# naver-ai/egtr

Hardware: AMD Instinct MI355X
Metric: images/sec end-to-end SGG, 600x1000 input, N=200 queries (higher is better)
Workload: dtype f32; 1 GPU; VG inference: ResNet-50, N=200, 6 enc/6 dec, 150 classes, 50 predicates, 600x1000, bs=1/GPU fp32 (BASELINE configs[1]); hip_graph=True, gemm_tuning=True, miopen_find=True, parallelism=replicas x1 (independent images, no collective)

## Files before the change

### egtr_amd/_lib.py

```python
import ctypes
import os

import torch

_HERE = os.path.dirname(os.path.abspath(__file__))
LIB_PATH = os.environ.get("EGTR_HIP_LIBRARY") or os.path.join(_HERE, "libegtr_hip.so")

_P = ctypes.c_void_p
_I = ctypes.c_int
ABI_VERSION = 5

SIGNATURES = {
    "egtr_abi_version": [],
    "egtr_status_string": [_I],
    "egtr_last_hip_error": [],
    "egtr_msda_forward_f32": [_P, _P, _P, _P, _P, _P, _I, _I, _I, _I, _I, _I, _I, _P],
    "egtr_msda_forward_fused_vbias_f32": [_P, _P, _P, _P, _P, _P, _P, _I, _I, _I, _I, _I, _I, _I, _P, _P, _I, _I, _P, _P,
                                          _P],
    "egtr_msda_forward_fused_box_f32": [_P, _P, _P, _P, _P, _P, _P, _I, _I, _I, _I, _I, _I, _I, _P, _P, _I, _I, _P, _P,
                                        _P],
    "egtr_msda_backward_f32": [_P, _P, _P, _P, _P, _P, _P, _I, _I, _I, _I, _I, _I, _I, _P, _P, _P],
    "egtr_msda_backward_out_f32": [_P, _P, _P, _P, _P, _P, _P, _I, _I, _I, _I, _I, _I, _I, _P, _P, _P],
    "egtr_msda_forward_f64": [_P, _P, _P, _P, _P, _P, _I, _I, _I, _I, _I, _I, _I, _P],
    "egtr_msda_backward_f64": [_P, _P, _P, _P, _P, _P, _P, _I, _I, _I, _I, _I, _I, _I, _P, _P, _P],
    "egtr_msda_backward_bf16": [_P, _P, _P, _P, _P, _P, _P, _I, _I, _I, _I, _I, _I, _I, _P, _P, _P, _P],
    "egtr_msda_backward_bf16_workspace_floats": [_I, _I, _I, _I, _I, _I, _I],
    "egtr_msda_forward_bf16": [_P, _P, _P, _P, _P, _P, _I, _I, _I, _I, _I, _I, _I, _P],
    "egtr_msda_forward_fused_bf16": [_P, _P, _P, _P, _P, _P, _P, _I, _I, _I, _I, _I, _I, _I, _P, _I, _I, _P, _P],
    "egtr_self_attn_forward_f32": [_P, _P, _P, _P, _I, _I, _I, _I, _P, _P, _P, _P],
    "egtr_self_attn_forward_bf16": [_P, _P, _P, _P, _I, _I, _I, _I, _P, _P, _P],
    "egtr_self_attn_backward_f32": [_P, _P, _P, _P, _P, _P, _P, _I, _I, _I, _I, _P, _P, _P],
    "egtr_self_attn_backward_acc_f32": [_P, _P, _P, _P, _P, _P, _P, _I, _I, _I, _I, _P, _P, _P, _P, _P],
    "egtr_linear_f32": [_P, _P, _P, _P, _P, _I, _I, _I, ctypes.c_float, _I],
    "egtr_linear_grouped_f32": [_P, _I, _P, _P, _P, _P, _P, _P, _P, _P, _P, _P, _I],
    "egtr_linear_grouped_ln_f32": [_P, _I, _P, _P, _P, _P, _P, _P, _P, _P, _P, _P, _I, _P, _P, _P, _P, _P, _P, _P],
    "egtr_add_layernorm_pos_f32": [_P, _P, _P, _P, _P, _P, _I, _I, ctypes.c_float, _P, _I, _P],
    "egtr_bias_mask_rows_f32": [_P, _P, _P, _P, _I, _I, _I],
    "egtr_bias_relu_maxpool3x3s2_f32": [_P, _P, _P, _P, _I, _I, _I, _I],
    "egtr_box_decode_argmax_f32": [_P, _P, _P, _P, _I, _I, _I, _I, ctypes.c_float, _P, _P, _I, _P],
    "egtr_scale_rows_multi_f32": [_P, _I, _P, _P, _P, _P, _P],
    "egtr_bias_act_nchw_f32": [_P, _P, _P, _P, _P, _I, _I, _I, _I],
    "egtr_bias_act_nchw_bf16": [_P, _P, _P, _P, _P, _I, _I, _I, _I],
    "egtr_bias_act_nhwc_bf16": [_P, _P, _P, _P, _P, ctypes.c_longlong, _I, _I],
    "egtr_bias_act_nhwc_f32": [_P, _P, _P, _P, _P, ctypes.c_longlong, _I, _I],
    "egtr_add_layernorm_bf16": [_P, _P, _P, _P, _P, _P, _I, _I, ctypes.c_float],
    "egtr_add_layernorm_pos_bf16": [_P, _P, _P, _P, _P, _P, _I, _I, ctypes.c_float, _P, _I, _P],
    "egtr_add_layernorm_f32": [_P, _P, _P, _P, _P, _P, _I, _I, ctypes.c_float],
    "egtr_sine_pos_embed_f32": [_P, _P, _P, _P, _P, _I, _I, _I, _I, ctypes.c_float, ctypes.c_float],
    "egtr_level_geometry_f32": [_P, _P, _I, _P, _P, _P, _I, _I, _I, _I, _I, ctypes.c_float, ctypes.c_float, _P, _P, _P,
                                _P, _P],
    "egtr_level_geometry_bf16": [_P, _P, _I, _P, _P, _P, _I, _I, _I, _I, _I, ctypes.c_float, ctypes.c_float, _P, _P, _P,
                                 _P, _P],
    "egtr_input_proj_groupnorm_flatten_f32": [_P, _I, _P, _P, _P, _P, _P, _I, _I, _I, ctypes.c_float, _P, _P],
    "egtr_input_proj_groupnorm_flatten_bf16": [_P, _I, _P, _P, _P, _P, _P, _I, _I, _I, ctypes.c_float, _P, _P],
    "egtr_input_proj_groupnorm_tokens_bf16": [_P, _I, _P, _P, _P, _P, _P, _I, _I, _I, ctypes.c_float, _P, _P],
    "egtr_input_proj_groupnorm_tokens_f32": [_P, _I, _P, _P, _P, _P, _P, _I, _I, _I, ctypes.c_float, _P, _P],
    "egtr_input_proj_groupnorm_tokens_workspace_floats": [_I, _P, _I],
    "egtr_bbox_overlaps_f64": [_P, _P, _P, _I, _I, _I, _P],
    "egtr_sgg_eval_width": [_I, _I],
    "egtr_sgg_eval_f32": [_P, _P, _I, _P, _P, _P, _I, _I, _I, _I, _P, _P, ctypes.c_longlong, _P, _P, _P, ctypes.c_longlong,
                          _P, _I, ctypes.c_double, _P, _P, _P],
    "egtr_sgg_zero_shot_f64": [_P, _P, _P, _P, ctypes.c_longlong, _P, _P, ctypes.c_longlong, _I, _I, _I, _I, _P, _P, _I, _P,
                               _P],
    "egtr_sgg_eval_phrdet_f32": [_P, _P, _I, _P, _P, _P, _I, _I, _I, _I, _P, _P, ctypes.c_longlong, _P, _P, _P,
                                 ctypes.c_longlong, _P, _I, ctypes.c_double, _P, _P, _P],
    "egtr_sgg_eval_preddet_f32": [_P, _P, _P, _I, _I, _I, _P, _P, ctypes.c_longlong, _P, ctypes.c_longlong, _P, _I, _P, _P,
                                  _P, _P, _P],
    "egtr_matched_topk_workspace_bytes": [_I, _I, _I],
    "egtr_matched_topk_f32": [_P, _P, _P, _P, _P, _I, _I, _I, _I, _I, _I, _P, _P, _P, _P, _P],
    "egtr_rel_stats_i64": [_P, _P, _P, ctypes.c_longlong, _P, _P, ctypes.c_longlong, _I, _I, _I, _P, _P],
    "egtr_rel_seen_bits_i64": [_P, _P, ctypes.c_longlong, _P],
    "egtr_oi_eval_width": [_I, _I],
    "egtr_oi_select_workspace_bytes": [_I, _I, _I, _I],
    "egtr_oi_select_f32": [_P, _P, ctypes.c_longlong, ctypes.c_longlong, _P, _P, ctypes.c_longlong, _I, _I, _I, _I, _I,
                           _I, _P, _P, _P, _P],
    "egtr_oi_match_f32": [_P, _P, _P, _I, _I, _P, _P, _I, _I, _P, _P, ctypes.c_longlong, _P, _P, _P, ctypes.c_longlong,
                          _P, _I, _P, _P, _P],
    "egtr_oi_ap_f64": [_P, _P, _P, _P, ctypes.c_longlong, _I, _P, _P],
    "egtr_coco_match_f32": [_P, _P, _P, _P, _I, _I, _I, _P, _P, _P, _P, _P, ctypes.c_longlong, _P, _P, _I, _P, _P, _P,
                            _P, _P],
    "egtr_coco_accumulate_f64": [_P, _P, _P, _P, _P, ctypes.c_longlong, _I, _P, _P, _P, _P],
    "egtr_hungarian_match_f32": [_P, _P, _P, _P, _P, _P, _P, _I, _I, _I, _I, ctypes.c_float, ctypes.c_float,
                                 ctypes.c_float, _I, ctypes.c_float, ctypes.c_float, _P, _P, _P, _P, _P, _P, _P],
    "egtr_hungarian_match_scratch_doubles": [_I, _I, ctypes.c_longlong],
    "egtr_add_layernorm_backward_f32": [_P, _P, _P, _P, _P, _P, _P, _P, _I, _I, ctypes.c_float],
    "egtr_add_layernorm_backward_workspace_floats": [_I],
    "egtr_msda_geometry_forward_f32": [_P, _P, ctypes.c_longlong, _P, ctypes.c_longlong, _P, _I, _P, _P, _P, ctypes.c_longlong, _I, _I, _I],
    "egtr_msda_geometry_backward_f32": [_P, _P, _P, _P, _P, ctypes.c_longlong, _P, _I, _P, _P, ctypes.c_longlong, _P, ctypes.c_longlong, _P, ctypes.c_longlong, _I, _I, _I],
    "egtr_linear_backward_f32": [_P, _P, _P, _P, _P, ctypes.c_float, _P, _P, _P, _I, _I, _I],
    "egtr_linear_backward_acc_f32": [_P, _P, _P, _P, _P, ctypes.c_float, _P, _P, _P, _I, _I, _I, _P, _P],
    "egtr_weighted_column_sum_f32": [_P, _P, _P, _P, _P, _I, _I],
    "egtr_column_sum_f32": [_P, _P, _P, _P, _P, _P, _I, _I],
    "egtr_column_sum_workspace_floats": [_I, _I],
    "egtr_any_nonfinite_f32": [_P, _P, ctypes.c_longlong, _P],
    "egtr_clamp_if_flag_f32": [_P, _P, _P, ctypes.c_longlong, _P, ctypes.c_float, _I],
    "egtr_detection_loss_f32": [_P, _P, _P, _P, _P, _P, _P, _P, _P, _I, _I, _I, ctypes.c_float, ctypes.c_float, _P, _P,
                                _P, _P],
    "egtr_relation_loss_f32": [_P, _P, _P, _P, _P, _P, _P, _P, _I, _I, _I, ctypes.c_float, _I, _I, _P, _P, _P, _P],
    "egtr_relation_loss_workspace_bytes": [_I, _I],
    "egtr_relation_loss_bits_f32": [_P, _P, _P, _P, _P, _P, _P, _P, _I, _I, _I, ctypes.c_float, _I, _I, _P, _P, _P, _P],
    "egtr_pack_relations_u64": [_P, _P, _P, _I, _I, _I, _I, _P],
    "egtr_rel_head_forward_bf16w": [_P] * 16 + [_I] * 6 + [_P] * 3,
    "egtr_ffn_layernorm_bf16": [_P] * 7 + [ctypes.c_float, _P, _I, _P, _P, _I, _I, _I],
    "egtr_ffn_pack_weights_bf16": [_P, _P, _P, _I, _I, _P],
    "egtr_ffn_packed_weights_bytes": [_I],
    "egtr_linear_bf16": [_P, _P, _I, _P, _P, _P, _I, _I, _I, _I, _I, ctypes.c_float],
    "egtr_rel_head_forward_bf16p": [_P] * 16 + [_I] * 6 + [_P] * 3,
    "egtr_rel_head_pack_tables_bf16": [_P, _P, _I, _I, _I, _P],
    "egtr_linear_split_bf16_f32": [_P, _P, _I, _P, _P, _P, _I, _I, _I, _I, _I],
    "egtr_linear_split_bf16_wgrad_f32": [_P, _P, _I, _P, _I, _P, _P, _I, _I, _I],
    "egtr_linear_split_bf16_wgrad_workspace_floats": [_I, _I, _I],
    "egtr_gemm_split_tile_weights_f32": [_P, _P, _I, _I, _I, _I, _P],
    "egtr_gemm_split_tile_weights_pair_f32": [_P, _P, _I, _I, _I, _P],
    "egtr_gemm_split_tile_weights_multi_f32": [_P, _I, _P, _P, _P, _P, _P, _P, _P, _P],
    "egtr_linear_split_bf16_grouped_pos_f32": [_P, _I, _P, _P, _P, _P, _P, _P, _P, _P, _I, _I, _P, _P],
    "egtr_linear_split_bf16_ex_f32": [_P, _I, _P, _P, _P, _P, _P, _P, _P, _P, _I, _I, _P, _P, _P, _P, _P, _P, _P, _P, _P],
    "egtr_linear_split_bf16_wgrad_ex_f32": [_P, _P, _I, _P, _I, _P, _P, _I, _I, _I, _P, _I, _P],
    "egtr_dropout_add_layernorm_f32": [_P, _P, _P, _P, ctypes.c_float, _P, _P, _P, _I, _I, ctypes.c_float, _P],
    "egtr_dropout_add_layernorm_backward_workspace_floats": [_I],
    "egtr_dropout_add_layernorm_backward_f32": [_P, _P, _P, _P, ctypes.c_float, _P, _P, _P, _P, ctypes.c_float, _P, _P, _P,
                                                _P, _I, _I, ctypes.c_float],
    "egtr_pad_batch_f32": [_P, _P, _P, _I, _I, _I, _I, _P, _P],
    "egtr_preprocess_f32": [_P, _P, _I, _P, _P, _I, _I, _I, _I, _P, _P, _P],
    "egtr_preprocess_bf16": [_P, _P, _I, _P, _P, _I, _I, _I, _I, _P, _P, _P],
    "egtr_preprocess_augment_f32": [_P, _P, _P, _I, _P, _P, _I, _I, _I, _I, _I, _I, _I, _I, _P, _P, _P],
    "egtr_preprocess_augment_bf16": [_P, _P, _P, _I, _P, _P, _I, _I, _I, _I, _I, _I, _I, _I, _P, _P, _P],
    "egtr_conv1x1_tail_x6_f32": [_P, _P, _I, _P, _I, _P, _P, _P, _I, _I, _P, _I, _I, _I, _I, _I, _I],
    "egtr_stem_conv7x7_pool_bf16": [_P, _P, _P, _P, _P, _I, _I, _I],
    "egtr_stem_conv7x7_pool_x6_f32": [_P, _P, _P, _P, _P, _I, _I, _I],
    "egtr_conv1x1_strided_x6_f32": [_P, _P, _P, _P, _I, _I, _I, _I, _I, _I],
    "egtr_conv3x3_phase_channels": [_I, _I, _I, _I],
    "egtr_conv3x3_x6_f32": [_P, _P, _P, _P, _I, _I, _I, _I, _I, _I, _I],
    "egtr_conv3x3_x6_shift_f32": [_P, _P, _P, _P, _P, _I, _I, _I, _I, _I, _I, _I],
    "egtr_conv1x1_tail_pack_weights_bf16": [_P, _P, _I, _I, _I, _P],
    "egtr_conv1x1_tail_bf16": [_P, _P, _I, _P, _I, _P, _P, _P, _I, _I, _P, _I, _I, _I, _I],
    "egtr_ffn_x6_f32": [_P, _P, _I, _P, _P, _P, _P, _P, _P, ctypes.c_float, _P, _I, _P, _P, _I, _I, _I],
    "egtr_encoder_tail_x6_f32": [_P, _P, _I, _P, _I, _P, _P, _P, _P, ctypes.c_float, _P, _P, _P, _P, _P, _P, ctypes.c_float,
                                 _P, _I, _P, _P, _I, _I, _I],
    "egtr_proj_ln_x6_f32": [_P, _P, _I, _P, _P, _P, _I, _P, _P, ctypes.c_float, _P, _I, _P, _P, _I, _I],
    "egtr_proj_multi_x6_f32": [_P, _P, _I, _P, _P, _P, _I, _I, _I],
    "egtr_xs_bytes": [_I, _I],
    "egtr_xs_split_f32": [_P, _P, _I, _P, _I, _I, _I, _P, _P, _I],
    "egtr_rel_head_forward_bf16x6_f32": [_P] * 16 + [_I] * 6 + [_P] * 3 + [_I],
    "egtr_rel_head_forward_bf16x6_save_f32": [_P] * 16 + [_I] * 6 + [_P] * 5,
    "egtr_rel_head_streams_f32": [_P] * 4 + [_I] * 2 + [_P] * 3,
    "egtr_rel_head_forward_save_f32": [_P] * 16 + [_I] * 6 + [_P] * 5,
    "egtr_rel_head_backward_pairs_f32": [_P] * 6 + [_I] * 4 + [_P] * 5,
    "egtr_decoder_layer_f32": [_P, _P],
    "egtr_decoder_layer_workspace": [_I, _I, _P, _P, _P],
}
_RESTYPES = {"egtr_status_string": ctypes.c_char_p, "egtr_last_hip_error": ctypes.c_char_p,
             "egtr_ffn_packed_weights_bytes": ctypes.c_longlong,
             "egtr_input_proj_groupnorm_tokens_workspace_floats": ctypes.c_longlong,
             "egtr_msda_backward_bf16_workspace_floats": ctypes.c_longlong,
             "egtr_hungarian_match_scratch_doubles": ctypes.c_longlong,
             "egtr_relation_loss_workspace_bytes": ctypes.c_longlong,
             "egtr_column_sum_workspace_floats": ctypes.c_longlong,
             "egtr_add_layernorm_backward_workspace_floats": ctypes.c_longlong,
             "egtr_linear_split_bf16_wgrad_workspace_floats": ctypes.c_longlong,
             "egtr_dropout_add_layernorm_backward_workspace_floats": ctypes.c_longlong,
             "egtr_xs_bytes": ctypes.c_longlong, "egtr_sgg_eval_width": ctypes.c_longlong,
             "egtr_oi_eval_width": ctypes.c_longlong, "egtr_matched_topk_workspace_bytes": ctypes.c_longlong, "egtr_oi_select_workspace_bytes": ctypes.c_longlong}

_lib = None


class EgtrHipError(RuntimeError):
    pass


def lib():
    global _lib
    if _lib is None:
        if not os.path.exists(LIB_PATH):
            raise EgtrHipError(
                f"{LIB_PATH} not found: the HIP extension has not been built "
                "(run `make -C egtr_amd/csrc` or __graft_entry__.build()). There is no CPU fallback.")
        handle = ctypes.CDLL(LIB_PATH)
        handle.egtr_abi_version.restype = ctypes.c_int
        got = handle.egtr_abi_version()
        if got != ABI_VERSION:
            raise EgtrHipError(f"{LIB_PATH} has ABI version {got}, this package was written against {ABI_VERSION}: "
                               "rebuild it (make -C egtr_amd/csrc)")
        if os.environ.get("EGTR_HIP_LIBRARY"):
            import sys
            print(f"egtr_amd: EGTR_HIP_LIBRARY is set -- using {LIB_PATH} instead of the in-tree build", file=sys.stderr)
        for name, argtypes in SIGNATURES.items():
            fn = getattr(handle, name)
            fn.argtypes = argtypes
            fn.restype = _RESTYPES.get(name, ctypes.c_int)
        _lib = handle
    return _lib


def check(status, what):
    if status != 0:
        h = lib()
        msg = h.egtr_status_string(status).decode()
        if status == -2:
            msg += ": " + h.egtr_last_hip_error().decode()
        raise EgtrHipError(f"{what} failed: {msg} (status {status})")


def _chk(t, name, dtype=None):
    if not t.is_cuda:
        raise RuntimeError(f"{name} must be a CUDA/HIP tensor")
    if not t.is_contiguous():
        raise RuntimeError(f"{name} tensor has to be contiguous")
    if dtype is not None and t.dtype != dtype:
        raise RuntimeError(f"{name} must be {dtype}, got {t.dtype}")
    if t.data_ptr() % 16 != 0:
        raise RuntimeError(f"{name} must be 16-byte aligned")
    return t


_RAW_STREAM = getattr(torch._C, "_cuda_getCurrentRawStream", None)


def _stream():
    if _RAW_STREAM is not None:
        return _RAW_STREAM(torch.cuda.current_device())
    return torch.cuda.current_stream().cuda_stream


def launch(name, *args, what=None):
    st = getattr(lib(), name)(_stream(), *args)
    if st != 0:
        check(st, what or name)


def ptr(t):
    return None if t is None else t.data_ptr()


def row_view(t, K):
    t2 = t.reshape(-1, K)
    if t2.stride(1) != 1 or t2.stride(0) % 4 or t2.data_ptr() % 16:
        t2 = t2.contiguous()
    return t2
```

### egtr_amd/csrc/elementwise.hip

```cpp
#include <hip/hip_runtime.h>
#include <stdint.h>

#include "common.h"

namespace {

__global__ __launch_bounds__(256) void bias_act_nchw_vec4(const float* __restrict__ x, const float* __restrict__ bias,
                                                          const float* __restrict__ res, float* __restrict__ y,
                                                          long long n4, int C, int HW4, int relu) {
  for (long long i = blockIdx.x * (long long)blockDim.x + threadIdx.x; i < n4; i += (long long)gridDim.x * blockDim.x) {
    const int c = (int)((i / HW4) % C);
    const float b = bias[c];
    float4 v = reinterpret_cast<const float4*>(x)[i];
    v.x += b; v.y += b; v.z += b; v.w += b;
    if (res != nullptr) {
      const float4 r = reinterpret_cast<const float4*>(res)[i];
      v.x += r.x; v.y += r.y; v.z += r.z; v.w += r.w;
    }
    if (relu) { v.x = egtr_relu(v.x); v.y = egtr_relu(v.y); v.z = egtr_relu(v.z); v.w = egtr_relu(v.w); }
    reinterpret_cast<float4*>(y)[i] = v;
  }
}

__global__ __launch_bounds__(256) void bias_act_nchw_flat4(const float* __restrict__ x, const float* __restrict__ bias,
// ... 238 lines not shown
    }
    if (relu) {
#pragma unroll
      for (int k = 0; k < 8; ++k) v[k] = egtr_relu(v[k]);
    }
    unsigned w[4];
#pragma unroll
    for (int k = 0; k < 4; ++k) {
      bf16x2 pr;
      pr[0] = (__bf16)v[2 * k];
      pr[1] = (__bf16)v[2 * k + 1];
      w[k] = __builtin_bit_cast(unsigned, pr);
    }
    reinterpret_cast<uint4*>(y)[i] = make_uint4(w[0], w[1], w[2], w[3]);
  }
}

__global__ __launch_bounds__(256) void bias_act_nchw_scalar_bf16(const unsigned short* __restrict__ x,
                                                                 const float* __restrict__ bias,
                                                                 const unsigned short* __restrict__ res,
                                                                 unsigned short* __restrict__ y, long long n, int C,
                                                                 int HW, int relu) {
  for (long long i = blockIdx.x * (long long)blockDim.x + threadIdx.x; i < n; i += (long long)gridDim.x * blockDim.x) {
    const int c = (int)((i / HW) % C);
    float v = bf2f(x[i]) + bias[c];
    if (res != nullptr) v += bf2f(res[i]);
    if (relu) v = egtr_relu(v);
    y[i] = f2bf(v);
  }
}

__global__ __launch_bounds__(256) void bias_mask_rows(float* __restrict__ y, const float* __restrict__ bias,
                                                      const unsigned char* __restrict__ keep, long long n4, int R,
                                                      int C4) {
  for (long long i = blockIdx.x * (long long)blockDim.x + threadIdx.x; i < n4; i += (long long)gridDim.x * blockDim.x) {
    const int c4 = (int)(i % C4);
    const long long gr = i / C4;
    const int r = (int)(gr % R);
    const int g = (int)(gr / R);
    float4 v = reinterpret_cast<float4*>(y)[i];
    const float4 b = reinterpret_cast<const float4*>(bias)[(size_t)g * C4 + c4];
    const bool k = keep == nullptr || keep[r] != 0;
    v = k ? make_float4(v.x + b.x, v.y + b.y, v.z + b.z, v.w + b.w) : make_float4(0.f, 0.f, 0.f, 0.f);
    reinterpret_cast<float4*>(y)[i] = v;
  }
}

__global__ __launch_bounds__(256) void bias_relu_maxpool3x3s2(const float* __restrict__ x, const float* __restrict__ bias,
                                                              float* __restrict__ y, int C, int H, int W, int Ho,
                                                              int Wo, long long planes) {
  const int ox = blockIdx.x * 64 + (threadIdx.x & 63);
  const int oy = blockIdx.y * 4 + (threadIdx.x >> 6);
  const long long plane = blockIdx.z;
  if (ox >= Wo || oy >= Ho) return;
  const float* xp = x + plane * H * W;
  const int iy0 = 2 * oy - 1, ix0 = 2 * ox - 1;
  float m = -INFINITY;
#pragma unroll
  for (int dy = 0; dy < 3; ++dy) {
    const int iy = iy0 + dy;
    if (iy < 0 || iy >= H) continue;
    const float* row = xp + (size_t)iy * W;
#pragma unroll
    for (int dx = 0; dx < 3; ++dx) {
      const int ix = ix0 + dx;
      if (ix >= 0 && ix < W) {
        const float v = row[ix];
        m = (v > m || v != v) ? v : m;
      }
    }
  }
  const float r = m + bias[(int)(plane % C)];
  y[(plane * Ho + oy) * Wo + ox] = (r != r) ? r : fmaxf(r, 0.f);
}

__global__ __launch_bounds__(256) void box_decode(const float* __restrict__ delta, const float* __restrict__ init_ref,
                                                  const float* __restrict__ inter_ref, int B, int Ld, int N, int RD,
                                                  float eps, float* __restrict__ out,
                                                  const float* __restrict__ logits_all, int C,
                                                  long long* __restrict__ node_cls) {
  const int nb_decode = (B * Ld * N + 255) / 256;
  if ((int)blockIdx.x >= nb_decode) {
    const int row = ((int)blockIdx.x - nb_decode) * 4 + (threadIdx.x >> 6), lane = threadIdx.x & 63;
    if (row >= B * N) return;
    const int b = row / N, n = row - b * N;
    const float* lg = logits_all + (((size_t)b * Ld + (Ld - 1)) * N + n) * C;
    float best = lane < C ? lg[lane] : 0.f;
    int arg = lane < C ? lane : 0x7fffffff;
    for (int c = lane + 64; c < C; c += 64) {
      const float v = lg[c];
      if (v > best || (v != v && best == best)) { best = v; arg = c; }
    }
#pragma unroll
    for (int o = 1; o < 64; o <<= 1) {
      const float v = __shfl_xor(best, o);
      const int a = __shfl_xor(arg, o);
      const bool vn = v != v, bn = best != best;
      const bool take = a != 0x7fffffff && (arg == 0x7fffffff || (vn && !bn) || (!bn && v > best) || ((vn == bn) && (vn || v == best) && a < arg));
      if (take) { best = v; arg = a; }
    }
    if (lane == 0) node_cls[row] = arg;
    return;
  }
  const int i = blockIdx.x * 256 + threadIdx.x;
  if (i >= B * Ld * N) return;
  const int n = i % N, l = (i / N) % Ld, b = i / (N * Ld);
  const float* rp = (l == 0 || inter_ref == nullptr) ? init_ref + ((size_t)b * N + n) * RD
                                                      : inter_ref + (((size_t)b * Ld + (l - 1)) * N + n) * RD;
  const float4 d = reinterpret_cast<const float4*>(delta)[i];
  float v[4] = {d.x, d.y, d.z, d.w};
  for (int k = 0; k < RD; ++k) {
    float x = rp[k];
    x = fminf(fmaxf(x, 0.f), 1.f);
    if (rp[k] != rp[k]) x = rp[k];
    const float x1 = (x != x) ? x : fmaxf(x, eps), x2 = (x != x) ? x : fmaxf(1.f - x, eps);
    v[k] += logf(x1 / x2);
  }
  float4 o;
  o.x = 1.f / (1.f + expf(-v[0]));
  o.y = 1.f / (1.f + expf(-v[1]));
  o.z = 1.f / (1.f + expf(-v[2]));
  o.w = 1.f / (1.f + expf(-v[3]));
  reinterpret_cast<float4*>(out)[i] = o;
}

__global__ __launch_bounds__(256) void sine_pos_embed(const float* __restrict__ y_embed, const float* __restrict__ x_embed,
                                                      const float* __restrict__ dim_t, float* __restrict__ out, int B,
                                                      int H, int Wd, int E, float scale, float eps) {
  const long long n = (long long)B * E * H * Wd;
  for (long long i = blockIdx.x * (long long)blockDim.x + threadIdx.x; i < n; i += (long long)gridDim.x * blockDim.x) {
    const int x = (int)(i % Wd);
    long long t = i / Wd;
    const int y = (int)(t % H);
    t /= H;
    const int slot = (int)(t % E);
    const int b = (int)(t / E);
    const int axis = slot >= E / 2;
    const int pair = axis ? slot - E / 2 : slot;
    const size_t pix = ((size_t)b * H + y) * Wd + x;
    float e, last;
    if (axis == 0) {
      e = y_embed[pix];
      last = y_embed[((size_t)b * H + (H - 1)) * Wd + x];
    } else {
      e = x_embed[pix];
      last = x_embed[((size_t)b * H + y) * Wd + (Wd - 1)];
    }
    const float v = (e - 0.5f) / (last + eps) * scale;
    const float a0 = v / dim_t[2 * pair], a1 = v / dim_t[2 * pair + 1];
    const size_t plane = (size_t)H * Wd;
    float* o = out + ((size_t)b * 2 * E + (size_t)axis * E + 2 * pair) * plane + (size_t)y * Wd + x;
    o[0] = sinf(a0);
    o[plane] = cosf(a1);
  }
}


struct LevelDims {
  int H[4], W[4], start[4];
};

template <typename MaskT>
__global__ __launch_bounds__(256) void level_mask_resize(const MaskT* __restrict__ pixel_mask, LevelDims ld, int L, int S,
                                                         int Hin, int Win, unsigned char* __restrict__ mask_flat,
                                                         unsigned* __restrict__ mask_bits) {
  const int b = blockIdx.y;
  const int s = blockIdx.x * 256 + threadIdx.x;
  int m = 0;
  if (s < S) {
    int l = 0;
    while (l + 1 < L && s >= ld.start[l + 1]) ++l;
    const int rel = s - ld.start[l];
    const int y = rel / ld.W[l], x = rel - y * ld.W[l];
    const float sh = (float)Hin / (float)ld.H[l], sw = (float)Win / (float)ld.W[l];
    const int sy = min((int)floorf((float)y * sh), Hin - 1), sx = min((int)floorf((float)x * sw), Win - 1);
    m = pixel_mask[((size_t)b * Hin + sy) * Win + sx] != 0 ? 1 : 0;
    mask_flat[(size_t)b * S + s] = (unsigned char)m;
  }
  if (mask_bits != nullptr) {
    const unsigned long long bal = __ballot(m != 0);
    const int lane = threadIdx.x & 63, s64 = s - lane;
    const int nwords = (S + 31) >> 5;
    if (lane < 2 && s64 + 32 * lane < S && (s64 >> 5) + lane < nwords)
      mask_bits[(size_t)b * nwords + (s64 >> 5) + lane] = (unsigned)(bal >> (32 * lane));
  }
}

template <typename PosT>
__global__ __launch_bounds__(256) void level_geometry(const unsigned char* __restrict__ mask_all,
                                                      const float* __restrict__ dim_t,
                                                      const float* __restrict__ level_embed, LevelDims ld, int L, int S,
                                                      int E, float scale, float eps, PosT* __restrict__ pos_flat,
                                                      float* __restrict__ valid_ratios, float* __restrict__ ref_points) {
  constexpr int TP = 8;
  __shared__ int s_cnt[8];
  __shared__ float s_vr[8];
  __shared__ int s_pix[TP][5];
  const int tid = threadIdx.x;
  const int b = blockIdx.y;
  const int s0 = blockIdx.x * TP;
  const unsigned char* mk = mask_all + (size_t)b * S;
  if (tid < 8) s_cnt[tid] = 0;
  __syncthreads();
  for (int l = 0; l < L; ++l) {
    const unsigned char* ml = mk + ld.start[l];
    int cw = 0, ch = 0;
    for (int x = tid; x < ld.W[l]; x += 256) cw += ml[x];
    for (int y = tid; y < ld.H[l]; y += 256) ch += ml[(size_t)y * ld.W[l]];
#pragma unroll
    for (int o = 1; o < 64; o <<= 1) {
      cw += __shfl_xor(cw, o);
      ch += __shfl_xor(ch, o);
    }
    if ((tid & 63) == 0) {
      if (cw) atomicAdd(&s_cnt[2 * l], cw);
      if (ch) atomicAdd(&s_cnt[2 * l + 1], ch);
    }
  }
  {
    const int p = tid >> 5, part = tid & 31;
    const int s = s0 + p;
    int l = 0, cy = 0, toty = 0, cx = 0, totx = 0;
    if (s < S) {
      while (l + 1 < L && s >= ld.start[l + 1]) ++l;
      const unsigned char* ml = mk + ld.start[l];
      const int rel = s - ld.start[l];
      const int Wl = ld.W[l], Hl = ld.H[l];
      const int y = rel / Wl, x = rel - y * Wl;
      for (int yy = part; yy < Hl; yy += 32) {
        const int v = ml[yy * Wl + x];
        toty += v;
        cy += (yy <= y) ? v : 0;
      }
      for (int xx = part; xx < Wl; xx += 32) {
        const int v = ml[y * Wl + xx];
        totx += v;
        cx += (xx <= x) ? v : 0;
      }
    }
#pragma unroll
    for (int o = 1; o < 32; o <<= 1) {
      cy += __shfl_xor(cy, o);
      toty += __shfl_xor(toty, o);
      cx += __shfl_xor(cx, o);
      totx += __shfl_xor(totx, o);
    }
    if (part == 0) {
      s_pix[p][0] = l;
      s_pix[p][1] = cy;
      s_pix[p][2] = toty;
      s_pix[p][3] = cx;
      s_pix[p][4] = totx;
    }
  }
  __syncthreads();
  if (tid < 2 * L) {
    const int l = tid >> 1;
    const float vr = (float)s_cnt[tid] / (float)((tid & 1) ? ld.H[l] : ld.W[l]);
    s_vr[tid] = vr;
    if (blockIdx.x == 0) valid_ratios[(size_t)b * L * 2 + tid] = vr;
  }
  __syncthreads();
  if (tid < 8 * TP) {
    const int p = tid >> 3, k = tid & 7, s = s0 + p;
    if (s < S && k < 2 * L) {
      const int l = s_pix[p][0];
      const int rel = s - ld.start[l];
      const int y = rel / ld.W[l], x = rel - y * ld.W[l];
      const int lt = k >> 1, ax = k & 1;
      const float base = ax ? ((float)y + 0.5f) / (s_vr[2 * l + 1] * (float)ld.H[l])
                            : ((float)x + 0.5f) / (s_vr[2 * l] * (float)ld.W[l]);
      ref_points[(((size_t)b * S + s) * L + lt) * 2 + ax] = base * s_vr[2 * lt + ax];
    }
  }
  {
    const int npair = E;
    const int per = 256 / npair > 0 ? 256 / npair : 1;
    for (int k = tid % npair; k < npair; k += 256) {
      const int c = 2 * k;
      const int axis = c >= E, i = axis ? c - E : c;
      const float dt = dim_t[i];
      for (int p = (npair <= 256 ? tid / npair : 0); p < TP; p += per) {
        const int s = s0 + p;
        if (s >= S) break;
        const int l = s_pix[p][0];
        const float e = (float)(axis ? s_pix[p][3] : s_pix[p][1]), last = (float)(axis ? s_pix[p][4] : s_pix[p][2]);
        const float v = (e - 0.5f) / (last + eps) * scale;
        const float a = v / dt;
        float sn, cs;
        sincosf(a, &sn, &cs);
        const float2 le = *reinterpret_cast<const float2*>(level_embed + l * 2 * E + c);
        if constexpr (sizeof(PosT) == 4) {
          *reinterpret_cast<float2*>(pos_flat + ((size_t)b * S + s) * (2 * E) + c) = make_float2(sn + le.x, cs + le.y);
        } else {
          const unsigned lo = f2bf(bf2f(f2bf(sn)) + le.x), hi = f2bf(bf2f(f2bf(cs)) + le.y);
          *reinterpret_cast<unsigned*>(pos_flat + ((size_t)b * S + s) * (2 * E) + c) = lo | (hi << 16);
        }
      }
    }
  }
}


struct GnLevels {
  const void* x[4];
  const float* conv_bias[4];
  const float* gamma[4];
  const float* beta[4];
  int hw[4], start[4], tile0[4];
};

__device__ __forceinline__ float gn_load(const float* p) { return *p; }
__device__ __forceinline__ float gn_load(const unsigned short* p) { return bf2f(*p); }

template <typename T>
__global__ __launch_bounds__(1024) void gn_stats_levels(GnLevels P, int C, int G, float eps, float2* __restrict__ stats) {
  __shared__ double s_red[2][16];
  const int g = blockIdx.x, b = blockIdx.y, l = blockIdx.z;
  const int cpg = C / G, hw = P.hw[l];
  const T* x = static_cast<const T*>(P.x[l]) + ((size_t)b * C + (size_t)g * cpg) * hw;
  float s1 = 0.f, s2 = 0.f;
  for (int c = 0; c < cpg; ++c) {
    const float cb = P.conv_bias[l][g * cpg + c];
    const T* xc = x + (size_t)c * hw;
    for (int i0 = threadIdx.x; i0 < hw; i0 += 8 * 1024) {
      float v[8];
#pragma unroll
      for (int u = 0; u < 8; ++u) {
        const int i = i0 + 1024 * u;
        v[u] = i < hw ? gn_load(xc + i) : 0.f;
      }
#pragma unroll
      for (int u = 0; u < 8; ++u) {
        if (i0 + 1024 * u < hw) {
          const float t = v[u] + cb;
          s1 += t;
          s2 += t * t;
        }
      }
    }
  }
  double d1 = (double)s1, d2 = (double)s2;
#pragma unroll
  for (int o = 1; o < 64; o <<= 1) {
    d1 += __shfl_xor(d1, o);
    d2 += __shfl_xor(d2, o);
  }
  if ((threadIdx.x & 63) == 0) {
    s_red[0][threadIdx.x >> 6] = d1;
    s_red[1][threadIdx.x >> 6] = d2;
  }
  __syncthreads();
  if (threadIdx.x == 0) {
    double t1 = 0.0, t2 = 0.0;
    for (int w = 0; w < 16; ++w) {
      t1 += s_red[0][w];
      t2 += s_red[1][w];
    }
    const double n = (double)cpg * hw, mean = t1 / n;
    const double var = fmax(t2 / n - mean * mean, 0.0);
    stats[((size_t)l * gridDim.y + b) * G + g] = make_float2((float)mean, (float)(1.0 / sqrt(var + (double)eps)));
  }
}

template <typename T>
__global__ __launch_bounds__(256) void gn_apply_flatten(GnLevels P, int L, int C, int G, int S, const float2* __restrict__ stats,
                                                        T* __restrict__ out) {
  __shared__ float s_t[32][257];
  const int b = blockIdx.y;
  int l = 0;
  while (l + 1 < L && (int)blockIdx.x >= P.tile0[l + 1]) ++l;
  const int p0 = ((int)blockIdx.x - P.tile0[l]) * 32, hw = P.hw[l];
  const int cpg = C / G;
  const int px = threadIdx.x & 31, cs = threadIdx.x >> 5;
  const T* x = static_cast<const T*>(P.x[l]) + (size_t)b * C * hw;
  float xv[32];
  const bool inside = p0 + px < hw;
#pragma unroll
  for (int k = 0; k < 32; ++k) xv[k] = inside ? gn_load(x + (size_t)(cs + 8 * k) * hw + p0 + px) : 0.f;
#pragma unroll
  for (int k = 0; k < 32; ++k) {
    const int c = cs + 8 * k;
    const float2 st = stats[((size_t)l * gridDim.y + b) * G + c / cpg];
    const float v = (xv[k] + P.conv_bias[l][c] - st.x) * st.y * P.gamma[l][c] + P.beta[l][c];
    s_t[px][c] = inside ? v : 0.f;
  }
  __syncthreads();
  for (int p = 0; p < 32; ++p) {
    if (p0 + p >= hw) break;
    if constexpr (sizeof(T) == 4) out[((size_t)b * S + P.start[l] + p0 + p) * C + threadIdx.x] = s_t[p][threadIdx.x];
    else out[((size_t)b * S + P.start[l] + p0 + p) * C + threadIdx.x] = f2bf(s_t[p][threadIdx.x]);
  }
}

}

extern "C" int egtr_sine_pos_embed_f32(egtr_stream_t stream, const float* y_embed, const float* x_embed,
                                       const float* dim_t, float* out, int B, int H, int W, int E, float scale,
                                       float eps) {
  if (!y_embed || !x_embed || !dim_t || !out) return EGTR_E_ARG;
  if (B <= 0 || H <= 0 || W <= 0 || E <= 0 || (E & 1)) return EGTR_E_ARG;
  const long long n = (long long)B * E * H * W;
  const int blocks = (int)std::min<long long>((n + 255) / 256, 256 * 16);
  hipLaunchKernelGGL(sine_pos_embed, dim3(blocks), dim3(256), 0, static_cast<hipStream_t>(stream), y_embed, x_embed,
                     dim_t, out, B, H, W, E, scale, eps);
  return egtr_check_launch();
}

static int level_geometry_launch(egtr_stream_t stream, const void* pixel_mask, int mask_elem_size, const float* dim_t,
                                 const float* level_embed, const int* level_hw, int num_levels, int batch, int height,
                                 int width, int embed_dim, float scale, float eps, unsigned char* mask_flat,
                                 void* pos_flat, bool pos_bf16, float* valid_ratios, float* ref_points,
                                 unsigned* mask_bits) {
  if (!pixel_mask || !dim_t || !level_embed || !level_hw || !mask_flat || !pos_flat || !valid_ratios || !ref_points)
    return EGTR_E_ARG;
  if (num_levels < 1 || num_levels > 4 || batch <= 0 || height <= 0 || width <= 0 || embed_dim <= 0)
    return EGTR_E_ARG;
  if (mask_elem_size != 1 && mask_elem_size != 8) return EGTR_E_UNSUPPORTED;
  if (embed_dim & 1) return EGTR_E_UNSUPPORTED;
  LevelDims ld;
  int S = 0;
  for (int l = 0; l < 4; ++l) {
    const bool on = l < num_levels;
    ld.H[l] = on ? level_hw[2 * l] : 1;
    ld.W[l] = on ? level_hw[2 * l + 1] : 1;
    ld.start[l] = S;
    if (on) {
      if (ld.H[l] <= 0 || ld.W[l] <= 0) return EGTR_E_ARG;
      S += ld.H[l] * ld.W[l];
    }
  }
  hipStream_t st = static_cast<hipStream_t>(stream);
  const dim3 grid1((unsigned)((S + 255) / 256), (unsigned)batch);
  if (mask_elem_size == 8)
    hipLaunchKernelGGL(level_mask_resize<long long>, grid1, dim3(256), 0, st, static_cast<const long long*>(pixel_mask),
                       ld, num_levels, S, height, width, mask_flat, mask_bits);
  else
    hipLaunchKernelGGL(level_mask_resize<unsigned char>, grid1, dim3(256), 0, st,
                       static_cast<const unsigned char*>(pixel_mask), ld, num_levels, S, height, width, mask_flat,
                       mask_bits);
  const dim3 grid((unsigned)((S + 7) / 8), (unsigned)batch);
  if (pos_bf16)
    hipLaunchKernelGGL(level_geometry<unsigned short>, grid, dim3(256), 0, st, mask_flat, dim_t, level_embed, ld,
                       num_levels, S, embed_dim, scale, eps, static_cast<unsigned short*>(pos_flat), valid_ratios,
                       ref_points);
  else
    hipLaunchKernelGGL(level_geometry<float>, grid, dim3(256), 0, st, mask_flat, dim_t, level_embed, ld, num_levels, S,
                       embed_dim, scale, eps, static_cast<float*>(pos_flat), valid_ratios, ref_points);
  return egtr_check_launch();
}

extern "C" int egtr_level_geometry_f32(egtr_stream_t stream, const void* pixel_mask, int mask_elem_size,
                                       const float* dim_t, const float* level_embed, const int* level_hw,
                                       int num_levels, int batch, int height, int width, int embed_dim, float scale,
                                       float eps, unsigned char* mask_flat, float* pos_flat, float* valid_ratios,
                                       float* ref_points, unsigned* mask_bits) {
  return level_geometry_launch(stream, pixel_mask, mask_elem_size, dim_t, level_embed, level_hw, num_levels, batch, height,
                               width, embed_dim, scale, eps, mask_flat, pos_flat, false, valid_ratios, ref_points,
                               mask_bits);
}

extern "C" int egtr_level_geometry_bf16(egtr_stream_t stream, const void* pixel_mask, int mask_elem_size,
                                        const float* dim_t, const float* level_embed, const int* level_hw,
                                        int num_levels, int batch, int height, int width, int embed_dim, float scale,
                                        float eps, unsigned char* mask_flat, uint16_t* pos_flat, float* valid_ratios,
                                        float* ref_points, unsigned* mask_bits) {
  return level_geometry_launch(stream, pixel_mask, mask_elem_size, dim_t, level_embed, level_hw, num_levels, batch, height,
                               width, embed_dim, scale, eps, mask_flat, pos_flat, true, valid_ratios, ref_points,
                               mask_bits);
}

static int groupnorm_flatten_launch(egtr_stream_t stream, int num_levels, const void* const* x,
                                    const float* const* conv_bias, const float* const* gamma, const float* const* beta,
                                    const int* level_hw, int batch, int channels, int num_groups, float eps, float* stats,
                                    void* out, bool bf16) {
  if (!x || !conv_bias || !gamma || !beta || !level_hw || !stats || !out) return EGTR_E_ARG;
  if (num_levels < 1 || num_levels > 4 || batch <= 0 || num_groups <= 0) return EGTR_E_ARG;
  if (channels != 256 || channels % num_groups != 0) return EGTR_E_UNSUPPORTED;
  GnLevels P;
  int S = 0, tiles = 0;
  for (int l = 0; l < 4; ++l) {
    const int s = l < num_levels ? l : 0;
    if (!x[s] || !conv_bias[s] || !gamma[s] || !beta[s] || level_hw[2 * s] <= 0 || level_hw[2 * s + 1] <= 0)
      return EGTR_E_ARG;
    P.x[l] = x[s];
    P.conv_bias[l] = conv_bias[s];
    P.gamma[l] = gamma[s];
    P.beta[l] = beta[s];
    P.hw[l] = level_hw[2 * s] * level_hw[2 * s + 1];
    P.start[l] = S;
    P.tile0[l] = tiles;
    if (l < num_levels) {
      S += P.hw[l];
      tiles += (P.hw[l] + 31) / 32;
    }
  }
  hipStream_t st = static_cast<hipStream_t>(stream);
  if (bf16) {
    hipLaunchKernelGGL(gn_stats_levels<unsigned short>, dim3(num_groups, batch, num_levels), dim3(1024), 0, st, P, channels,
                       num_groups, eps, reinterpret_cast<float2*>(stats));
    hipLaunchKernelGGL(gn_apply_flatten<unsigned short>, dim3(tiles, batch), dim3(256), 0, st, P, num_levels, channels,
                       num_groups, S, reinterpret_cast<const float2*>(stats), static_cast<unsigned short*>(out));
  } else {
    hipLaunchKernelGGL(gn_stats_levels<float>, dim3(num_groups, batch, num_levels), dim3(1024), 0, st, P, channels,
                       num_groups, eps, reinterpret_cast<float2*>(stats));
    hipLaunchKernelGGL(gn_apply_flatten<float>, dim3(tiles, batch), dim3(256), 0, st, P, num_levels, channels, num_groups,
                       S, reinterpret_cast<const float2*>(stats), static_cast<float*>(out));
  }
  return egtr_check_launch();
}

struct GnTokLevels {
  const void* x[4];
  const float* conv_bias[4];
  const float* gamma[4];
  const float* beta[4];
  int hw[4], start[4];
  long long chunk0[5];
  int cchunk0[5];
};

namespace {
__device__ __forceinline__ void load_group8(const unsigned short* x, size_t idx, float (&f)[8]) {
  unpack8(reinterpret_cast<const uint4*>(x)[idx], f);
}
__device__ __forceinline__ void load_group8(const float* x, size_t idx, float (&f)[8]) {
  const float4 a = reinterpret_cast<const float4*>(x)[2 * idx], b = reinterpret_cast<const float4*>(x)[2 * idx + 1];
  f[0] = a.x; f[1] = a.y; f[2] = a.z; f[3] = a.w; f[4] = b.x; f[5] = b.y; f[6] = b.z; f[7] = b.w;
}
constexpr int kGnTokChunk = 256;
template <typename T>
__global__ __launch_bounds__(256) void gn_partial_tokens(GnTokLevels P, int L, int chunks_total, double2* __restrict__ partial) {
  __shared__ double s_red[2][32][9];
  const int b = blockIdx.y;
  int l = 0;
  while (l + 1 < L && (int)blockIdx.x >= P.cchunk0[l + 1]) ++l;
  const int t_begin = ((int)blockIdx.x - P.cchunk0[l]) * kGnTokChunk, hw = P.hw[l];
  const int g = threadIdx.x & 31, ph = threadIdx.x >> 5;
  const T* x = static_cast<const T*>(P.x[l]) + (size_t)b * hw * 256;
  const float4 ba = *reinterpret_cast<const float4*>(P.conv_bias[l] + 8 * g), bb = *reinterpret_cast<const float4*>(P.conv_bias[l] + 8 * g + 4);
  const float cb[8] = {ba.x, ba.y, ba.z, ba.w, bb.x, bb.y, bb.z, bb.w};
  float s1 = 0.f, s2 = 0.f;
#pragma unroll
  for (int u0 = 0; u0 < kGnTokChunk / 8; u0 += 8) {
    float f[8][8];
#pragma unroll
    for (int u = 0; u < 8; ++u) {
      const int t = t_begin + ph + 8 * (u0 + u);
      if (t < hw) load_group8(x, (size_t)t * 32 + g, f[u]);
    }
#pragma unroll
    for (int u = 0; u < 8; ++u) {
      const int t = t_begin + ph + 8 * (u0 + u);
      if (t < hw) {
#pragma unroll
        for (int k = 0; k < 8; ++k) {
          const float v = f[u][k] + cb[k];
          s1 += v;
          s2 += v * v;
        }
      }
    }
  }
  s_red[0][g][ph] = (double)s1;
  s_red[1][g][ph] = (double)s2;
  __syncthreads();
  if (threadIdx.x < 32) {
    double t1 = 0.0, t2 = 0.0;
    for (int w = 0; w < 8; ++w) {
      t1 += s_red[0][threadIdx.x][w];
      t2 += s_red[1][threadIdx.x][w];
    }
    partial[((size_t)b * chunks_total + blockIdx.x) * 32 + threadIdx.x] = make_double2(t1, t2);
  }
}

__global__ __launch_bounds__(256) void gn_finalize_tokens(GnTokLevels P, int chunks_total, float eps,
                                                          const double2* __restrict__ partial, float2* __restrict__ stats) {
  __shared__ double2 s_part[8][32];
  const int b = blockIdx.x, l = blockIdx.y, B = gridDim.x, g = threadIdx.x & 31, part = threadIdx.x >> 5;
  double t1 = 0.0, t2 = 0.0;
  for (int c = P.cchunk0[l] + part; c < P.cchunk0[l + 1]; c += 8) {
    const double2 p = partial[((size_t)b * chunks_total + c) * 32 + g];
    t1 += p.x;
    t2 += p.y;
  }
  s_part[part][g] = make_double2(t1, t2);
  __syncthreads();
  if (part != 0) return;
  t1 = 0.0;
  t2 = 0.0;
#pragma unroll
  for (int k = 0; k < 8; ++k) {
    t1 += s_part[k][g].x;
    t2 += s_part[k][g].y;
  }
  const double n = 8.0 * P.hw[l], mean = t1 / n;
  const double var = fmax(t2 / n - mean * mean, 0.0);
  stats[((size_t)l * B + b) * 32 + g] = make_float2((float)mean, (float)(1.0 / sqrt(var + (double)eps)));
}

template <typename T>
__global__ __launch_bounds__(256) void gn_apply_tokens(GnTokLevels P, int L, int S, const float2* __restrict__ stats,
                                                       T* __restrict__ out) {
  typedef __bf16 bf16x2 __attribute__((ext_vector_type(2)));
  const int b = blockIdx.y, B = gridDim.y;
  const long long i = (long long)blockIdx.x * 256 + threadIdx.x;
  if (i >= (long long)S * 32) return;
  int l = 0;
  while (l + 1 < L && i >= P.chunk0[l + 1]) ++l;
  const long long rel = i - P.chunk0[l];
  const int g = (int)(rel & 31);
  const float2 st = stats[((size_t)l * B + b) * 32 + g];
  float f[8];
  load_group8(static_cast<const T*>(P.x[l]) + (size_t)b * P.hw[l] * 256, (size_t)rel, f);
  const float4 ca = *reinterpret_cast<const float4*>(P.conv_bias[l] + 8 * g), cb = *reinterpret_cast<const float4*>(P.conv_bias[l] + 8 * g + 4);
  const float4 ga = *reinterpret_cast<const float4*>(P.gamma[l] + 8 * g), gb = *reinterpret_cast<const float4*>(P.gamma[l] + 8 * g + 4);
  const float4 ea = *reinterpret_cast<const float4*>(P.beta[l] + 8 * g), eb = *reinterpret_cast<const float4*>(P.beta[l] + 8 * g + 4);
  const float c8[8] = {ca.x, ca.y, ca.z, ca.w, cb.x, cb.y, cb.z, cb.w};
  const float g8[8] = {ga.x, ga.y, ga.z, ga.w, gb.x, gb.y, gb.z, gb.w};
  const float e8[8] = {ea.x, ea.y, ea.z, ea.w, eb.x, eb.y, eb.z, eb.w};
  float o[8];
#pragma unroll
  for (int k = 0; k < 8; ++k) o[k] = (f[k] + c8[k] - st.x) * st.y * g8[k] + e8[k];
  T* dst = out + ((size_t)b * S + P.start[l]) * 256;
  if constexpr (sizeof(T) == 2) {
    unsigned w[4];
#pragma unroll
    for (int k = 0; k < 4; ++k) {
      bf16x2 pr;
      pr[0] = (__bf16)o[2 * k];
      pr[1] = (__bf16)o[2 * k + 1];
      w[k] = __builtin_bit_cast(unsigned, pr);
    }
    reinterpret_cast<uint4*>(dst)[rel] = make_uint4(w[0], w[1], w[2], w[3]);
  } else {
    reinterpret_cast<float4*>(dst)[2 * rel] = make_float4(o[0], o[1], o[2], o[3]);
    reinterpret_cast<float4*>(dst)[2 * rel + 1] = make_float4(o[4], o[5], o[6], o[7]);
  }
}
}

static int gn_tokens_chunks(int num_levels, const int* level_tokens) {
  int c = 0;
  for (int l = 0; l < num_levels; ++l) c += (level_tokens[l] + kGnTokChunk - 1) / kGnTokChunk;
  return c;
}

extern "C" long long egtr_input_proj_groupnorm_tokens_workspace_floats(int num_levels, const int* level_tokens, int batch) {
  if (!level_tokens || num_levels < 1 || num_levels > 4 || batch <= 0) return 0;
  return (long long)num_levels * batch * 64 + (long long)batch * gn_tokens_chunks(num_levels, level_tokens) * 128;
}

static int groupnorm_tokens_launch(egtr_stream_t stream, int num_levels, const void* const* x, const float* const* conv_bias,
                                   const float* const* gamma, const float* const* beta, const int* level_tokens, int batch,
                                   int channels, int num_groups, float eps, float* stats, void* out, bool bf16) {
  if (!x || !conv_bias || !gamma || !beta || !level_tokens || !stats || !out) return EGTR_E_ARG;
  if (num_levels < 1 || num_levels > 4 || batch <= 0) return EGTR_E_ARG;
  if (channels != 256 || num_groups != 32) return EGTR_E_UNSUPPORTED;
  GnTokLevels P;
  int S = 0, cc = 0;
  for (int l = 0; l < 4; ++l) {
    const int s = l < num_levels ? l : 0;
    if (!x[s] || !conv_bias[s] || !gamma[s] || !beta[s] || level_tokens[s] <= 0) return EGTR_E_ARG;
    if (reinterpret_cast<uintptr_t>(x[s]) & 15) return EGTR_E_UNSUPPORTED;
    P.x[l] = x[s];
    P.conv_bias[l] = conv_bias[s];
    P.gamma[l] = gamma[s];
    P.beta[l] = beta[s];
    P.hw[l] = level_tokens[s];
    P.start[l] = S;
    P.chunk0[l] = (long long)S * 32;
    P.cchunk0[l] = cc;
    if (l < num_levels) {
      S += P.hw[l];
      cc += (P.hw[l] + kGnTokChunk - 1) / kGnTokChunk;
    }
  }
  P.chunk0[4] = (long long)S * 32;
  P.cchunk0[4] = cc;
  for (int l = num_levels; l < 4; ++l) {
    P.chunk0[l] = (long long)S * 32;
    P.cchunk0[l] = cc;
  }
  if ((reinterpret_cast<uintptr_t>(out) | reinterpret_cast<uintptr_t>(stats)) & 15) return EGTR_E_UNSUPPORTED;
  hipStream_t st = static_cast<hipStream_t>(stream);
  float2* st2 = reinterpret_cast<float2*>(stats);
  double2* partial = reinterpret_cast<double2*>(stats + (size_t)num_levels * batch * 64);
  const long long chunks = (long long)S * 32;
  const dim3 agrid((unsigned)((chunks + 255) / 256), batch);
  if (bf16) {
    hipLaunchKernelGGL(gn_partial_tokens<unsigned short>, dim3(cc, batch), dim3(256), 0, st, P, num_levels, cc, partial);
    hipLaunchKernelGGL(gn_finalize_tokens, dim3(batch, num_levels), dim3(256), 0, st, P, cc, eps, partial, st2);
    hipLaunchKernelGGL(gn_apply_tokens<unsigned short>, agrid, dim3(256), 0, st, P, num_levels, S, st2,
                       static_cast<unsigned short*>(out));
  } else {
    hipLaunchKernelGGL(gn_partial_tokens<float>, dim3(cc, batch), dim3(256), 0, st, P, num_levels, cc, partial);
    hipLaunchKernelGGL(gn_finalize_tokens, dim3(batch, num_levels), dim3(256), 0, st, P, cc, eps, partial, st2);
    hipLaunchKernelGGL(gn_apply_tokens<float>, agrid, dim3(256), 0, st, P, num_levels, S, st2, static_cast<float*>(out));
  }
  return egtr_check_launch();
}

extern "C" int egtr_input_proj_groupnorm_tokens_bf16(egtr_stream_t stream, int num_levels, const uint16_t* const* x,
                                                     const float* const* conv_bias, const float* const* gamma,
                                                     const float* const* beta, const int* level_tokens, int batch,
                                                     int channels, int num_groups, float eps, float* stats, uint16_t* out) {
  return groupnorm_tokens_launch(stream, num_levels, reinterpret_cast<const void* const*>(x), conv_bias, gamma, beta,
                                 level_tokens, batch, channels, num_groups, eps, stats, out, true);
}

extern "C" int egtr_input_proj_groupnorm_tokens_f32(egtr_stream_t stream, int num_levels, const float* const* x,
                                                    const float* const* conv_bias, const float* const* gamma,
                                                    const float* const* beta, const int* level_tokens, int batch,
                                                    int channels, int num_groups, float eps, float* stats, float* out) {
  return groupnorm_tokens_launch(stream, num_levels, reinterpret_cast<const void* const*>(x), conv_bias, gamma, beta,
                                 level_tokens, batch, channels, num_groups, eps, stats, out, false);
}

extern "C" int egtr_input_proj_groupnorm_flatten_f32(egtr_stream_t stream, int num_levels, const float* const* x,
                                                     const float* const* conv_bias, const float* const* gamma,
                                                     const float* const* beta, const int* level_hw, int batch,
                                                     int channels, int num_groups, float eps, float* stats,
                                                     float* out) {
  return groupnorm_flatten_launch(stream, num_levels, reinterpret_cast<const void* const*>(x), conv_bias, gamma, beta,
                                  level_hw, batch, channels, num_groups, eps, stats, out, false);
}

extern "C" int egtr_input_proj_groupnorm_flatten_bf16(egtr_stream_t stream, int num_levels, const uint16_t* const* x,
                                                      const float* const* conv_bias, const float* const* gamma,
                                                      const float* const* beta, const int* level_hw, int batch,
                                                      int channels, int num_groups, float eps, float* stats,
                                                      uint16_t* out) {
  return groupnorm_flatten_launch(stream, num_levels, reinterpret_cast<const void* const*>(x), conv_bias, gamma, beta,
                                  level_hw, batch, channels, num_groups, eps, stats, out, true);
}

struct ScaleRowsArgs {
  const float* w[64];
  const float* scale[64];
  float* out[64];
  int rows[64], cols[64], blk0[65];
  int n;
};

namespace {
__global__ __launch_bounds__(256) void scale_rows_multi(ScaleRowsArgs A) {
  int t = 0;
  while (t + 1 < A.n && (int)blockIdx.x >= A.blk0[t + 1]) ++t;
  const int cols = A.cols[t];
  const long long n4 = (long long)A.rows[t] * cols / 4;
  const float4* w = reinterpret_cast<const float4*>(A.w[t]);
  float4* o = reinterpret_cast<float4*>(A.out[t]);
  const float* sc = A.scale[t];
  const long long base = (long long)((int)blockIdx.x - A.blk0[t]) * 1024;
#pragma unroll
  for (int u = 0; u < 4; ++u) {
    const long long i = base + u * 256 + threadIdx.x;
    if (i < n4) {
      const float s = sc[(i * 4) / cols];
      const float4 v = w[i];
      o[i] = make_float4(v.x * s, v.y * s, v.z * s, v.w * s);
    }
  }
}
}

extern "C" int egtr_scale_rows_multi_f32(egtr_stream_t stream, int n, const float* const* w, const float* const* scale,
                                         float* const* out, const int* rows, const int* cols) {
  if (!w || !scale || !out || !rows || !cols) return EGTR_E_ARG;
  if (n <= 0 || n > 64) return EGTR_E_UNSUPPORTED;
  ScaleRowsArgs A;
  int blocks = 0;
  for (int t = 0; t < n; ++t) {
    if (!w[t] || !scale[t] || !out[t] || rows[t] <= 0 || cols[t] <= 0) return EGTR_E_ARG;
    if (cols[t] % 4 != 0) return EGTR_E_UNSUPPORTED;
    if ((reinterpret_cast<uintptr_t>(w[t]) | reinterpret_cast<uintptr_t>(out[t])) & 15) return EGTR_E_UNSUPPORTED;
    A.w[t] = w[t];
    A.scale[t] = scale[t];
    A.out[t] = out[t];
    A.rows[t] = rows[t];
    A.cols[t] = cols[t];
    A.blk0[t] = blocks;
    const long long n4 = (long long)rows[t] * cols[t] / 4;
    blocks += (int)((n4 + 1023) / 1024);
  }
  A.blk0[n] = blocks;
  A.n = n;
  hipLaunchKernelGGL(scale_rows_multi, dim3(blocks), dim3(256), 0, static_cast<hipStream_t>(stream), A);
  return egtr_check_launch();
}

extern "C" int egtr_bias_act_nchw_f32(egtr_stream_t stream, const float* x, const float* bias, const float* residual,
                                      float* y, int N, int C, int HW, int relu) {
  if (!x || !bias || !y) return EGTR_E_ARG;
  if (N <= 0 || C <= 0 || HW <= 0) return EGTR_E_ARG;
  hipStream_t st = static_cast<hipStream_t>(stream);
  const long long n = (long long)N * C * HW;
  const bool aligned = ((reinterpret_cast<uintptr_t>(x) | reinterpret_cast<uintptr_t>(y) |
                         reinterpret_cast<uintptr_t>(residual)) & 15) == 0;
  const long long cap = 256 * 8;
  if (HW % 4 == 0 && aligned) {
    const long long n4 = n / 4;
    const int blocks = (int)std::min<long long>((n4 + 255) / 256, cap);
    hipLaunchKernelGGL(bias_act_nchw_vec4, dim3(blocks), dim3(256), 0, st, x, bias, residual, y, n4, C, HW / 4, relu);
  } else if (n % 4 == 0 && aligned && HW >= 4 && n < (1ll << 25)) {
    const long long n4 = n / 4;
    const int blocks = (int)std::min<long long>((n4 + 255) / 256, cap);
    hipLaunchKernelGGL(bias_act_nchw_flat4, dim3(blocks), dim3(256), 0, st, x, bias, residual, y, n4, C, HW, relu);
  } else {
    const int blocks = (int)std::min<long long>((n + 255) / 256, cap);
    hipLaunchKernelGGL(bias_act_nchw_scalar, dim3(blocks), dim3(256), 0, st, x, bias, residual, y, n, C, HW, relu);
  }
  return egtr_check_launch();
}

extern "C" int egtr_add_layernorm_f32(egtr_stream_t stream, const float* x, const float* residual, const float* gamma,
                                      const float* beta, float* y, int rows, int dim, float eps) {
  if (!x || !gamma || !beta || !y) return EGTR_E_ARG;
  if (rows <= 0) return EGTR_E_ARG;
  if (dim != 256) return EGTR_E_UNSUPPORTED;
  hipLaunchKernelGGL(add_layernorm_256, dim3((rows + 3) / 4), dim3(256), 0, static_cast<hipStream_t>(stream), x,
                     residual, gamma, beta, y, rows, eps, (const float*)nullptr, 1, (float*)nullptr);
  return egtr_check_launch();
}

extern "C" int egtr_add_layernorm_pos_f32(egtr_stream_t stream, const float* x, const float* residual,
                                          const float* gamma, const float* beta, float* y, int rows, int dim,
                                          float eps, const float* pos, int pos_rows, float* y_plus_pos) {
  if (!x || !gamma || !beta || !y || !pos || !y_plus_pos) return EGTR_E_ARG;
  if (rows <= 0 || pos_rows <= 0) return EGTR_E_ARG;
  if (dim != 256) return EGTR_E_UNSUPPORTED;
  hipLaunchKernelGGL(add_layernorm_256, dim3((rows + 3) / 4), dim3(256), 0, static_cast<hipStream_t>(stream), x,
                     residual, gamma, beta, y, rows, eps, pos, pos_rows, y_plus_pos);
  return egtr_check_launch();
}

extern "C" int egtr_bias_relu_maxpool3x3s2_f32(egtr_stream_t stream, const float* x, const float* bias, float* y, int N,
                                               int C, int H, int W) {
  if (!x || !bias || !y) return EGTR_E_ARG;
  if (N <= 0 || C <= 0 || H <= 0 || W <= 0) return EGTR_E_ARG;
  const int Ho = (H - 1) / 2 + 1, Wo = (W - 1) / 2 + 1;
  const long long planes = (long long)N * C;
  if (planes > 65535 || (Ho + 3) / 4 > 65535) return EGTR_E_UNSUPPORTED;
  const dim3 grid((unsigned)((Wo + 63) / 64), (unsigned)((Ho + 3) / 4), (unsigned)planes);
  hipLaunchKernelGGL(bias_relu_maxpool3x3s2, grid, dim3(256), 0, static_cast<hipStream_t>(stream), x, bias, y, C, H, W, Ho,
                     Wo, planes);
  return egtr_check_launch();
}

extern "C" int egtr_box_decode_argmax_f32(egtr_stream_t stream, const float* delta, const float* init_reference,
                                          const float* inter_references, int batch, int num_levels, int num_query,
                                          int ref_dim, float eps, float* boxes, const float* logits_all,
                                          int num_classes, int64_t* node_cls) {
  if (!delta || !init_reference || !boxes) return EGTR_E_ARG;
  if (batch <= 0 || num_levels <= 0 || num_query <= 0) return EGTR_E_ARG;
  if (logits_all && (!node_cls || num_classes <= 0)) return EGTR_E_ARG;
  if (ref_dim != 2 && ref_dim != 4) return EGTR_E_UNSUPPORTED;
  const long long n = (long long)batch * num_levels * num_query;
  if (n >= (1ll << 31)) return EGTR_E_UNSUPPORTED;
  const long long blocks = (n + 255) / 256 + (logits_all ? ((long long)batch * num_query + 3) / 4 : 0);
  hipLaunchKernelGGL(box_decode, dim3((unsigned)blocks), dim3(256), 0, static_cast<hipStream_t>(stream), delta,
                     init_reference, inter_references, batch, num_levels, num_query, ref_dim, eps, boxes, logits_all,
                     num_classes, reinterpret_cast<long long*>(node_cls));
  return egtr_check_launch();
}

extern "C" int egtr_bias_mask_rows_f32(egtr_stream_t stream, float* y, const float* bias, const unsigned char* keep,
                                       int groups, int rows, int cols) {
  if (!y || !bias) return EGTR_E_ARG;
  if (groups <= 0 || rows <= 0 || cols <= 0) return EGTR_E_ARG;
  if (cols % 4 != 0) return EGTR_E_UNSUPPORTED;
  const long long n4 = (long long)groups * rows * (cols / 4);
  const int blocks = (int)std::min<long long>((n4 + 255) / 256, 256 * 16);
  hipLaunchKernelGGL(bias_mask_rows, dim3(blocks), dim3(256), 0, static_cast<hipStream_t>(stream), y, bias, keep, n4,
                     rows, cols / 4);
  return egtr_check_launch();
}

extern "C" int egtr_bias_act_nchw_bf16(egtr_stream_t stream, const uint16_t* x, const float* bias,
                                       const uint16_t* residual, uint16_t* y, int N, int C, int HW, int relu) {
  if (!x || !bias || !y) return EGTR_E_ARG;
  if (N <= 0 || C <= 0 || HW <= 0) return EGTR_E_ARG;
  hipStream_t st = static_cast<hipStream_t>(stream);
  const long long n = (long long)N * C * HW;
  const bool aligned = ((reinterpret_cast<uintptr_t>(x) | reinterpret_cast<uintptr_t>(y) |
                         reinterpret_cast<uintptr_t>(residual)) & 15) == 0;
  if (n % 8 == 0 && aligned && HW >= 8) {
    const long long n8 = n / 8;
    const int blocks = (int)std::min<long long>((n8 + 255) / 256, 256 * 16);
    hipLaunchKernelGGL(bias_act_nchw_flat8_bf16, dim3(blocks), dim3(256), 0, st, x, bias, residual, y, n8, C, HW, relu);
  } else {
    const int blocks = (int)std::min<long long>((n + 255) / 256, 256 * 16);
    hipLaunchKernelGGL(bias_act_nchw_scalar_bf16, dim3(blocks), dim3(256), 0, st, x, bias, residual, y, n, C, HW, relu);
  }
  return egtr_check_launch();
}

namespace {
__global__ __launch_bounds__(256) void bias_act_nhwc_flat4_f32(const float* __restrict__ x, const float* __restrict__ bias,
                                                               const float* __restrict__ res, float* __restrict__ y,
                                                               long long n4, int C, int relu) {
  for (long long i = blockIdx.x * (long long)blockDim.x + threadIdx.x; i < n4; i += (long long)gridDim.x * blockDim.x) {
    const float4 b = *reinterpret_cast<const float4*>(bias + (int)((i * 4) % C));
    float4 v = reinterpret_cast<const float4*>(x)[i];
    v.x += b.x; v.y += b.y; v.z += b.z; v.w += b.w;
    if (res != nullptr) {
      const float4 r = reinterpret_cast<const float4*>(res)[i];
      v.x += r.x; v.y += r.y; v.z += r.z; v.w += r.w;
    }
    if (relu) v = make_float4(egtr_relu(v.x), egtr_relu(v.y), egtr_relu(v.z), egtr_relu(v.w));
    reinterpret_cast<float4*>(y)[i] = v;
  }
}
}

extern "C" int egtr_bias_act_nhwc_f32(egtr_stream_t stream, const float* x, const float* bias, const float* residual, float* y,
                                      long long rows, int C, int relu) {
  if (!x || !bias || !y) return EGTR_E_ARG;
  if (rows <= 0 || C <= 0) return EGTR_E_ARG;
  if (C % 4 != 0 || ((reinterpret_cast<uintptr_t>(x) | reinterpret_cast<uintptr_t>(y) | reinterpret_cast<uintptr_t>(residual) |
                      reinterpret_cast<uintptr_t>(bias)) & 15))
    return EGTR_E_UNSUPPORTED;
  const long long n4 = rows * C / 4;
  const int blocks = (int)std::min<long long>((n4 + 255) / 256, 256 * 16);
  hipLaunchKernelGGL(bias_act_nhwc_flat4_f32, dim3(blocks), dim3(256), 0, static_cast<hipStream_t>(stream), x, bias, residual, y,
                     n4, C, relu);
  return egtr_check_launch();
}

extern "C" int egtr_bias_act_nhwc_bf16(egtr_stream_t stream, const uint16_t* x, const float* bias, const uint16_t* residual,
                                       uint16_t* y, long long rows, int C, int relu) {
  if (!x || !bias || !y) return EGTR_E_ARG;
  if (rows <= 0 || C <= 0) return EGTR_E_ARG;
  if (C % 8 != 0 || ((reinterpret_cast<uintptr_t>(x) | reinterpret_cast<uintptr_t>(y) | reinterpret_cast<uintptr_t>(residual) |
                      reinterpret_cast<uintptr_t>(bias)) & 15))
    return EGTR_E_UNSUPPORTED;
  const long long n8 = rows * C / 8;
  const int blocks = (int)std::min<long long>((n8 + 255) / 256, 256 * 16);
  hipLaunchKernelGGL(bias_act_nhwc_flat8_bf16, dim3(blocks), dim3(256), 0, static_cast<hipStream_t>(stream), x, bias, residual,
                     y, n8, C, relu);
  return egtr_check_launch();
}

extern "C" int egtr_add_layernorm_bf16(egtr_stream_t stream, const uint16_t* x, const uint16_t* residual,
                                       const uint16_t* gamma, const uint16_t* beta, uint16_t* y, int rows, int dim,
                                       float eps) {
  if (!x || !gamma || !beta || !y) return EGTR_E_ARG;
  if (rows <= 0) return EGTR_E_ARG;
  if (dim != 256) return EGTR_E_UNSUPPORTED;
  hipLaunchKernelGGL(add_layernorm_256_bf16, dim3((rows + 7) / 8), dim3(256), 0, static_cast<hipStream_t>(stream), x,
                     residual, gamma, beta, y, rows, eps, static_cast<const uint16_t*>(nullptr), 1,
                     static_cast<uint16_t*>(nullptr));
  return egtr_check_launch();
}

extern "C" int egtr_add_layernorm_pos_bf16(egtr_stream_t stream, const uint16_t* x, const uint16_t* residual,
                                           const uint16_t* gamma, const uint16_t* beta, uint16_t* y, int rows, int dim,
                                           float eps, const uint16_t* pos, int pos_rows, uint16_t* y_pos) {
  if (!x || !gamma || !beta || !y || !pos || !y_pos) return EGTR_E_ARG;
  if (rows <= 0 || pos_rows <= 0 || rows % pos_rows != 0) return EGTR_E_ARG;
  if (dim != 256) return EGTR_E_UNSUPPORTED;
  hipLaunchKernelGGL(add_layernorm_256_bf16, dim3((rows + 7) / 8), dim3(256), 0, static_cast<hipStream_t>(stream), x,
                     residual, gamma, beta, y, rows, eps, pos, pos_rows, y_pos);
  return egtr_check_launch();
}


namespace {

__global__ __launch_bounds__(256) void any_nonfinite_f32(const float* __restrict__ x, long long n4, long long n,
                                                         int* __restrict__ flag) {
  bool bad = false;
  for (long long i = blockIdx.x * (long long)blockDim.x + threadIdx.x; i < n4; i += (long long)gridDim.x * blockDim.x) {
    const float4 v = reinterpret_cast<const float4*>(x)[i];
    bad |= (__float_as_uint(v.x) & 0x7f800000u) == 0x7f800000u || (__float_as_uint(v.y) & 0x7f800000u) == 0x7f800000u ||
           (__float_as_uint(v.z) & 0x7f800000u) == 0x7f800000u || (__float_as_uint(v.w) & 0x7f800000u) == 0x7f800000u;
  }
  if (blockIdx.x == 0)
    for (long long i = 4 * n4 + threadIdx.x; i < n; i += blockDim.x)
      bad |= (__float_as_uint(x[i]) & 0x7f800000u) == 0x7f800000u;
  if (__any(bad) && (threadIdx.x & 63) == 0) atomicOr(flag, 1);
}

template <bool MASK>
__global__ __launch_bounds__(256) void clamp_if_flag_f32(float* __restrict__ t, const float* __restrict__ x, long long n,
                                                         const int* __restrict__ flag, float c) {
  if (*flag == 0) return;
  for (long long i = blockIdx.x * (long long)blockDim.x + threadIdx.x; i < n; i += (long long)gridDim.x * blockDim.x) {
    if (MASK) {
      const float v = x[i];
      if (!(fabsf(v) < c)) t[i] = 0.f;
    } else {
      const float v = t[i];
      t[i] = v != v ? v : fminf(fmaxf(v, -c), c);
    }
  }
}

}

extern "C" int egtr_any_nonfinite_f32(egtr_stream_t stream, const float* x, long long n, int* flag) {
  if (!x || !flag || n <= 0) return EGTR_E_ARG;
  if (reinterpret_cast<uintptr_t>(x) & 15) return EGTR_E_UNSUPPORTED;
  const long long n4 = n / 4;
  const int blocks = (int)std::min<long long>((n4 + 255) / 256 + 1, 2048);
  hipLaunchKernelGGL(any_nonfinite_f32, dim3(blocks), dim3(256), 0, static_cast<hipStream_t>(stream), x, n4, n, flag);
  return egtr_check_launch();
}

extern "C" int egtr_clamp_if_flag_f32(egtr_stream_t stream, float* t, const float* x, long long n, const int* flag,
                                      float clamp_value, int mask_gradient) {
  if (!t || !flag || n <= 0 || (mask_gradient && !x)) return EGTR_E_ARG;
  const int blocks = (int)std::min<long long>((n + 255) / 256, 4096);
  hipStream_t st = static_cast<hipStream_t>(stream);
  if (mask_gradient)
    hipLaunchKernelGGL(clamp_if_flag_f32<true>, dim3(blocks), dim3(256), 0, st, t, x, n, flag, clamp_value);
  else
    hipLaunchKernelGGL(clamp_if_flag_f32<false>, dim3(blocks), dim3(256), 0, st, t, x, n, flag, clamp_value);
  return egtr_check_launch();
// ... 214 lines not shown
```

### egtr_amd/kernels/elementwise.py

```python
import torch

from .. import _lib
from .._lib import _chk
from .derived import cached_weights

__all__ = ["dropout_add_layernorm", "dropout_add_layernorm_backward", "add_layer_norm_into", "box_decode", "bias_mask_rows_",
           "add_layer_norm_pos", "scale_rows_multi", "sine_position_embedding", "input_proj_groupnorm_flatten",
           "input_proj_groupnorm_tokens", "level_geometry"]


def dropout_add_layernorm(x, residual, keep, scale, weight, bias, eps, flag=None):
    rows = x.shape[0]
    y = torch.empty_like(x)
    _lib.launch("egtr_dropout_add_layernorm_f32", x.data_ptr(), residual.data_ptr(), _lib.ptr(keep), float(scale),
                weight.data_ptr(), bias.data_ptr(), y.data_ptr(), rows, 256, float(eps), _lib.ptr(flag))
    return y


def dropout_add_layernorm_backward(x, residual, keep, scale, weight, eps, grad_y, flag=None, y_out=None, clamp_value=0.0):
    lib = _lib.lib()
    rows = x.shape[0]
    gs = torch.empty_like(x)
    gx = torch.empty_like(x) if keep is not None else None
    ws = torch.empty(int(lib.egtr_dropout_add_layernorm_backward_workspace_floats(rows)), dtype=torch.float32, device=x.device)
    out = torch.empty(768, dtype=torch.float32, device=x.device)
    _lib.launch("egtr_dropout_add_layernorm_backward_f32", x.data_ptr(), residual.data_ptr(), _lib.ptr(keep), float(scale),
                weight.data_ptr(), grad_y.data_ptr(), _lib.ptr(flag),
                y_out.data_ptr() if (flag is not None and y_out is not None) else None, float(clamp_value), gs.data_ptr(),
                _lib.ptr(gx), ws.data_ptr(), out.data_ptr(), rows, 256, float(eps))
    return gs, (gx if gx is not None else gs), out


def add_layer_norm_into(x, residual, ln, out):
    x2 = _chk(x.contiguous(), "x", torch.float32)
    r2 = _chk(residual.contiguous(), "residual", torch.float32)
    _chk(out, "out", torch.float32)
    if out.shape != x2.shape or x2.shape[-1] != 256:
        raise ValueError("add_layer_norm_into: out must have the shape of x, 256 channels")
    _lib.launch("egtr_add_layernorm_f32", x2.data_ptr(), r2.data_ptr(), ln.weight.data_ptr(), ln.bias.data_ptr(),
                out.data_ptr(), x2.numel() // 256, 256, float(ln.eps))
    return out


def box_decode(delta, init_reference, inter_references, eps=1e-5, logits_all=None):
    B, Ld, N, four = delta.shape
    if four != 4:
        raise ValueError(f"delta must be [B, Ld, N, 4], got {tuple(delta.shape)}")
    d = _chk(delta.contiguous(), "delta", torch.float32)
    r0 = _chk(init_reference.contiguous(), "init_reference", torch.float32)
    RD = r0.shape[-1]
    same = (inter_references.dim() == 4 and Ld > 1 and inter_references.stride(1) == 0
            and inter_references.data_ptr() == init_reference.data_ptr()
            and inter_references.stride(0) == init_reference.stride(0)
            and tuple(inter_references.stride()[2:]) == tuple(init_reference.stride()[1:]))
    r1 = None if same else _chk(inter_references.contiguous(), "inter_references", torch.float32)
    if tuple(r0.shape) != (B, N, RD) or tuple(inter_references.shape) != (B, Ld, N, RD):
        raise ValueError(f"reference shapes {tuple(r0.shape)} / {tuple(inter_references.shape)} do not match delta "
                         f"{tuple(delta.shape)}")
    if RD not in (2, 4):
        raise ValueError(f"reference.shape[-1] should be 4 or 2, but got {RD}")
    out = torch.empty_like(d)
    lg, node, C = None, None, 0
    if logits_all is not None:
        lg = _chk(logits_all.contiguous(), "logits_all", torch.float32)
        C = lg.shape[-1]
        if tuple(lg.shape[:3]) != (B, Ld, N):
            raise ValueError("logits_all must be [B, Ld, N, C]")
        node = torch.empty(B, N, dtype=torch.int64, device=d.device)
    _lib.launch("egtr_box_decode_argmax_f32", d.data_ptr(), r0.data_ptr(), _lib.ptr(r1), B, Ld, N, RD, float(eps),
                out.data_ptr(), _lib.ptr(lg), C, _lib.ptr(node))
    return out if logits_all is None else (out, node)


def bias_mask_rows_(y, bias, keep):
    G, R, C = y.shape
    _chk(y, "y", torch.float32)
    b2 = _chk(bias.detach().contiguous(), "bias", torch.float32)
    k2 = None
    if keep is not None:
        k2 = keep.reshape(-1).contiguous()
        k2 = k2.view(torch.uint8) if k2.dtype == torch.bool else k2.to(torch.uint8)
        _chk(k2, "keep")
    _lib.launch("egtr_bias_mask_rows_f32", y.data_ptr(), b2.data_ptr(), _lib.ptr(k2), G, R, C)
    return y


def add_layer_norm_pos(x, residual, ln, pos, out=None):
    if x.dtype == torch.bfloat16:
        x2 = _chk(x.contiguous(), "x", torch.bfloat16)
        r2 = _chk(residual.contiguous(), "residual", torch.bfloat16)
        p2 = _chk(pos.contiguous(), "pos", torch.bfloat16)
        _chk(ln.weight, "ln.weight", torch.bfloat16)
        rows, prow = x2.numel() // 256, p2.numel() // 256
        if x2.shape[-1] != 256 or rows % prow != 0 or out is not None:
            raise ValueError("add_layer_norm_pos (bf16): d_model must be 256, pos must tile the rows, no `out`")
        y, yp = torch.empty_like(x2), torch.empty_like(x2)
        _lib.launch("egtr_add_layernorm_pos_bf16", x2.data_ptr(), r2.data_ptr(), ln.weight.data_ptr(), ln.bias.data_ptr(),
                    y.data_ptr(), rows, 256, float(ln.eps), p2.data_ptr(), prow, yp.data_ptr())
        return y, yp
    x2 = _chk(x.contiguous(), "x", torch.float32)
    r2 = _chk(residual.contiguous(), "residual", torch.float32)
    p2 = _chk(pos.contiguous(), "pos", torch.float32)
    rows = x2.numel() // 256
    prow = p2.numel() // 256
    if x2.shape[-1] != 256 or rows % prow != 0:
        raise ValueError("add_layer_norm_pos: d_model must be 256 and pos must tile the rows")
    y = torch.empty_like(x2) if out is None else _chk(out, "out", torch.float32)
    if y.shape != x2.shape:
        raise ValueError("add_layer_norm_pos: out must have the shape of x")
    yp = torch.empty_like(x2)
    _lib.launch("egtr_add_layernorm_pos_f32", x2.data_ptr(), r2.data_ptr(), ln.weight.data_ptr(), ln.bias.data_ptr(),
                y.data_ptr(), rows, 256, float(ln.eps), p2.data_ptr(), prow, yp.data_ptr())
    return y, yp


def scale_rows_multi(tensors, scales):
    import ctypes
    out = [None] * len(tensors)
    todo = []
    for i, (t, s) in enumerate(zip(tensors, scales)):
        rows = t.shape[0]
        cols = t.numel() // rows if rows else 0
        if (t.is_cuda and t.dtype == torch.float32 and s.dtype == torch.float32 and s.numel() == rows and cols > 0
                and cols % 4 == 0):
            tc = t.contiguous()
            if tc.data_ptr() % 16 == 0:
                todo.append((i, tc, s.reshape(-1).contiguous(), rows, cols))
                continue
        out[i] = t * s
    for c0 in range(0, len(todo), 64):
        grp = todo[c0:c0 + 64]
        n = len(grp)
        res = [torch.empty_like(g[1]) for g in grp]
        PA, IA = ctypes.c_void_p * n, ctypes.c_int * n
        _lib.launch("egtr_scale_rows_multi_f32", n, PA(*[g[1].data_ptr() for g in grp]), PA(*[g[2].data_ptr() for g in grp]),
                    PA(*[r.data_ptr() for r in res]), IA(*[g[3] for g in grp]), IA(*[g[4] for g in grp]))
        for g, r in zip(grp, res):
            out[g[0]] = r
    return out


def sine_position_embedding(pixel_mask, embedding_dim, temperature, scale, eps=1e-6):
    y_embed = pixel_mask.cumsum(1, dtype=torch.float32).contiguous()
    x_embed = pixel_mask.cumsum(2, dtype=torch.float32).contiguous()
    dim_t = torch.arange(embedding_dim, dtype=torch.float32, device=pixel_mask.device)
    dim_t = temperature ** (2 * torch.div(dim_t, 2, rounding_mode="trunc") / embedding_dim)
    B, H, W_ = pixel_mask.shape
    out = torch.empty(B, 2 * embedding_dim, H, W_, dtype=torch.float32, device=pixel_mask.device)
    _lib.launch("egtr_sine_pos_embed_f32", y_embed.data_ptr(), x_embed.data_ptr(), dim_t.data_ptr(), out.data_ptr(), B, H, W_,
                embedding_dim, float(scale), float(eps))
    return out


def input_proj_groupnorm_flatten(conv_outputs, input_projs):
    import ctypes
    L = len(conv_outputs)
    B, C = conv_outputs[0].shape[:2]
    gn0 = input_projs[0][1]
    dt = conv_outputs[0].dtype
    if dt not in (torch.float32, torch.bfloat16):
        raise TypeError("input_proj_groupnorm_flatten: fp32 or bf16 convolution outputs")
    xs = [_chk(x.contiguous(), "conv output", dt) for x in conv_outputs]
    for proj in input_projs[:L]:
        conv, gn = proj[0], proj[1]
        if gn.num_groups != gn0.num_groups or gn.eps != gn0.eps or conv.bias is None:
            raise ValueError("input_proj_groupnorm_flatten: levels must share the GroupNorm configuration")
    srcs = [t for proj in input_projs[:L] for t in (proj[0].bias, proj[1].weight, proj[1].bias)]
    if dt == torch.float32:
        keep = [tuple(_chk(t.detach().contiguous(), "input_proj parameter", torch.float32) for t in srcs[3 * l:3 * l + 3])
                for l in range(L)]
    else:
        flat = cached_weights(input_projs, "gn_params_f32", srcs,
                              lambda: [t.detach().float().contiguous() for t in srcs])
        keep = [tuple(flat[3 * l:3 * l + 3]) for l in range(L)]
    hw = [int(v) for x in xs for v in x.shape[-2:]]
    S = sum(h * w for h, w in zip(hw[0::2], hw[1::2]))
    out = torch.empty(B, S, C, dtype=dt, device=xs[0].device)
    stats = torch.empty(L * B * gn0.num_groups * 2, dtype=torch.float32, device=xs[0].device)
    PA, IA = ctypes.c_void_p * L, ctypes.c_int * (2 * L)
    entry = "egtr_input_proj_groupnorm_flatten_f32" if dt == torch.float32 else "egtr_input_proj_groupnorm_flatten_bf16"
    _lib.launch(entry, L, PA(*[x.data_ptr() for x in xs]), PA(*[k[0].data_ptr() for k in keep]),
                PA(*[k[1].data_ptr() for k in keep]), PA(*[k[2].data_ptr() for k in keep]), IA(*hw), B, C, gn0.num_groups,
                float(gn0.eps), stats.data_ptr(), out.data_ptr())
    return out


def input_proj_groupnorm_tokens(token_outputs, input_projs):
    import ctypes
    lib = _lib.lib()
    L = len(token_outputs)
    B = token_outputs[0].shape[0]
    gn0 = input_projs[0][1]
    dt = token_outputs[0].dtype
    if dt not in (torch.bfloat16, torch.float32):
        raise TypeError("input_proj_groupnorm_tokens: bf16 or fp32 projections")
    xs = [_chk(x.contiguous(), "token-major projection", dt) for x in token_outputs]
    for proj, x in zip(input_projs[:L], xs):
        conv, gn = proj[0], proj[1]
        if gn.num_groups != 32 or gn.eps != gn0.eps or conv.bias is None or x.shape[-1] != 256 or x.shape[0] != B:
            raise ValueError("input_proj_groupnorm_tokens: 256 channels in 32 groups, one GroupNorm configuration")
    srcs = [t for proj in input_projs[:L] for t in (proj[0].bias, proj[1].weight, proj[1].bias)]
    flat = cached_weights(input_projs, "gn_params_f32", srcs, lambda: [t.detach().float().contiguous() for t in srcs])
    keep = [tuple(flat[3 * l:3 * l + 3]) for l in range(L)]
    toks = [int(x.shape[1]) for x in xs]
    S = sum(toks)
    out = torch.empty(B, S, 256, dtype=dt, device=xs[0].device)
    PA, IA = ctypes.c_void_p * L, ctypes.c_int * L
    stats = torch.empty(int(lib.egtr_input_proj_groupnorm_tokens_workspace_floats(L, IA(*toks), B)), dtype=torch.float32,
                        device=xs[0].device)
    entry = "egtr_input_proj_groupnorm_tokens_bf16" if dt == torch.bfloat16 else "egtr_input_proj_groupnorm_tokens_f32"
    _lib.launch(entry, L, PA(*[x.data_ptr() for x in xs]), PA(*[k[0].data_ptr() for k in keep]),
                PA(*[k[1].data_ptr() for k in keep]), PA(*[k[2].data_ptr() for k in keep]), IA(*toks), B, 256, 32,
                float(gn0.eps), stats.data_ptr(), out.data_ptr())
    return out


_DIM_T = {}


def level_geometry(pixel_mask, spatial_shapes_list, level_embed, embedding_dim, temperature, scale, eps=1e-6):
    import ctypes
    dev = pixel_mask.device
    key = (embedding_dim, float(temperature), str(dev))
    dim_t = _DIM_T.get(key)
    if dim_t is None:
        dim_t = torch.arange(embedding_dim, dtype=torch.float32, device=dev)
        dim_t = temperature ** (2 * torch.div(dim_t, 2, rounding_mode="trunc") / embedding_dim)
        _DIM_T[key] = dim_t
    if pixel_mask.dtype not in (torch.int64, torch.uint8, torch.bool):
        pixel_mask = (pixel_mask != 0).to(torch.uint8)
    pm = pixel_mask.contiguous()
    _chk(pm, "pixel_mask")
    pos_dtype = level_embed.dtype
    if pos_dtype == torch.bfloat16:
        le = level_embed.detach().float().contiguous()
    else:
        le = _chk(level_embed.detach().contiguous(), "level_embed", torch.float32)
    B, H, W_ = pm.shape
    L = len(spatial_shapes_list)
    S = sum(h * w for h, w in spatial_shapes_list)
    hw = (ctypes.c_int * (2 * L))(*[int(v) for hw_ in spatial_shapes_list for v in hw_])
    mask_u8 = torch.empty(B, S, dtype=torch.uint8, device=dev)
    bits = torch.empty(B, (S + 31) // 32, dtype=torch.int32, device=dev)
    pos = torch.empty(B, S, 2 * embedding_dim, dtype=pos_dtype, device=dev)
    vr = torch.empty(B, L, 2, dtype=torch.float32, device=dev)
    ref = torch.empty(B, S, L, 2, dtype=torch.float32, device=dev)
    entry = "egtr_level_geometry_bf16" if pos_dtype == torch.bfloat16 else "egtr_level_geometry_f32"
    _lib.launch(entry, pm.data_ptr(), pm.element_size(), dim_t.data_ptr(), le.data_ptr(), hw, L, B, H, W_, embedding_dim,
                float(scale), float(eps), mask_u8.data_ptr(), pos.data_ptr(), vr.data_ptr(), ref.data_ptr(), bits.data_ptr())
    return mask_u8.view(torch.bool), pos, vr, ref, bits
```

### egtr_amd/ops.py

```python
import os

import torch
from torch.autograd import Function
from torch.autograd.function import once_differentiable

from . import _lib
from . import targets as rel_targets
from ._lib import _chk, _stream
from .kernels.backbone import *
from .kernels.derived import *
from .kernels.elementwise import *
from .kernels.elementwise import _DIM_T
from .kernels.heads import *
from .kernels.linear import *
from .kernels.linear import _c16, _host_array, _skinny_bwd, _skinny_fwd, _split3_bf16, _wgrad_ex
from .kernels.protocols import *
from .kernels.statistics import *
from .kernels.vrd import *
from .load_custom import load_hip_kernels

_MSDA = None


def _msda():
# ... 560 lines not shown

def encoder_layer_train(layer, x, attention_mask, pos, ref, spatial_shapes, level_start_index, masks=None):
    sa = layer.self_attn
    return EncoderLayerTrainFunction.apply(
        x, pos, ref, attention_mask, spatial_shapes, level_start_index, layer.dropout, masks,
        (layer.self_attn_layer_norm.eps, layer.final_layer_norm.eps), sa.sampling_offsets.weight, sa.sampling_offsets.bias, sa.attention_weights.weight, sa.attention_weights.bias,
        sa.value_proj.weight, sa.value_proj.bias, sa.output_proj.weight, sa.output_proj.bias,
        layer.self_attn_layer_norm.weight, layer.self_attn_layer_norm.bias, layer.fc1.weight, layer.fc1.bias,
        layer.fc2.weight, layer.fc2.bias, layer.final_layer_norm.weight, layer.final_layer_norm.bias)


DECODER_TRAIN_FUSED = True


class DecoderLayerTrainFunction(Function):

    @staticmethod
    def forward(ctx, x, pos, ref, value, shapes, lsi, p_drop, masks, eps3, scaling, wq, bq, wk, bk, wv, bv, wo, bo, ln1w, ln1b,
                wso, bso, waw, baw, wop, bop, ln2w, ln2b, w1, b1, w2, b2, ln3w, ln3b):
        B, N, D = x.shape
        M = B * N
        dev = x.device
        x2 = _rows256(x.detach())
        pos3 = pos.detach()
        heads = 8
        d = [t.detach() for t in (wq, bq, wk, bk, wv, bv, wo, bo, ln1w, ln1b, wso, bso, waw, baw, wop, bop, ln2w, ln2b, w1, b1,
                                  w2, b2, ln3w, ln3b)]
        (wq_, bq_, wk_, bk_, wv_, bv_, wo_, bo_, g1, be1, wso_, bso_, waw_, baw_, wop_, bop_, g2, be2, w1_, b1_, w2_, b2_, g3,
         be3) = [t if t.is_contiguous() else t.contiguous() for t in d]
        p = float(p_drop)
        scale = 1.0 / (1.0 - p) if p > 0.0 else 1.0
        if masks is not None:
            m1, m2, m3 = masks[0], masks[1], masks[2]
        elif p > 0.0:
            mm = torch.empty(3, M, D, dtype=torch.uint8, device=dev).bernoulli_(1.0 - p)
            m1, m2, m3 = mm[0], mm[1], mm[2]
        else:
            m1 = m2 = m3 = None
        e1, e2, e3 = (float(v) for v in eps3)
        xp = _rows256(x2.view(B, N, D) + pos3)
        q = _skinny_fwd(xp, wq_, bq_, alpha=scaling)
        k = _skinny_fwd(xp, wk_, bk_)
        v = _skinny_fwd(x2, wv_, bv_)
        sa = torch.empty(M, D, dtype=torch.float32, device=dev)
        lse = torch.empty(B, heads, N, dtype=torch.float32, device=dev)
        _lib.launch("egtr_self_attn_forward_f32", q.data_ptr(), k.data_ptr(), v.data_ptr(), B, N, heads, D // heads,
                    sa.data_ptr(), None, None, lse.data_ptr())
        a = _skinny_fwd(sa, wo_, bo_)
        y1 = dropout_add_layernorm(a, x2, m1, scale, g1, be1, e1)
        y1p = _rows256(y1.view(B, N, D) + pos3)
        off = _skinny_fwd(y1p, wso_, bso_)
        lg = _skinny_fwd(y1p, waw_, baw_)
        L = shapes.shape[0]
        P_ = wso_.shape[0] // (heads * L * 2)
        refc = _chk(ref.detach().contiguous(), "reference_points", torch.float32)
        shp = _chk(shapes.contiguous(), "spatial_shapes", torch.int64)
        loc = torch.empty(B, N, heads, L, P_, 2, dtype=torch.float32, device=dev)
        attn = torch.empty(B, N, heads, L, P_, dtype=torch.float32, device=dev)
        _lib.launch("egtr_msda_geometry_forward_f32", off.data_ptr(), off.stride(0), lg.data_ptr(), lg.stride(0),
                    refc.data_ptr(), refc.shape[-1], shp.data_ptr(), loc.data_ptr(), attn.data_ptr(), M, heads, L, P_)
        val = value.detach()
        S = val.shape[1]
        val4 = (val if val.is_contiguous() else val.contiguous()).view(B, S, heads, D // heads)
        ca = _msda().ms_deform_attn_forward(val4, shp, lsi, loc, attn, 64).view(M, D)
        c = _skinny_fwd(ca, wop_, bop_)
        y2 = dropout_add_layernorm(c, y1, m2, scale, g2, be2, e2)
        h = _skinny_fwd(y2, w1_, b1_, relu=True)
        f = _skinny_fwd(h, w2_, b2_)
        y3 = dropout_add_layernorm(f, y2, m3, scale, g3, be3, e3)
        ctx.save_for_backward(x2, xp, q, k, v, sa, lse, a, m1, y1, y1p, off, refc, shp, lsi, loc, attn, val4, ca, c, m2, y2, h,
                              f, m3, wq_, wk_, wv_, wo_, g1, wso_, waw_, wop_, g2, w1_, w2_, g3)
        ctx.dims = (B, N, D, heads, L, P_, scale, e1, e2, e3, float(scaling))
        ctx.pos_shape = tuple(pos.shape)
        ctx.value_shape = tuple(value.shape)
        ctx.ref_needs_grad = bool(ref.requires_grad)
        return y3.view(B, N, D), q.view(B, N, D), k.view(B, N, D)

    @staticmethod
    @once_differentiable
    def backward(ctx, g_y3, g_q_ext, g_k_ext):
        (x2, xp, q, k, v, sa, lse, a, m1, y1, y1p, off, refc, shp, lsi, loc, attn, val4, ca, c, m2, y2, h, f, m3, wq_, wk_, wv_,
         wo_, g1, wso_, waw_, wop_, g2, w1_, w2_, g3) = ctx.saved_tensors
        B, N, D, heads, L, P_, scale, e1, e2, e3, scaling = ctx.dims
        M = B * N
        dev = x2.device
        g3y = _rows256(g_y3)
        gs3, gf, gbb3 = dropout_add_layernorm_backward(f, y2, m3, scale, g3, e3, g3y)
        g_h, d_w2, _ = _skinny_bwd(gf, h, w2_, want_gb=False)
        g_y2, d_w1, d_b1 = _skinny_bwd(g_h, y2, w1_, relu_out=h, add1=gs3)
        gs2, gc, gbb2 = dropout_add_layernorm_backward(c, y1, m2, scale, g2, e2, g_y2)
        g_ca, d_wop, _ = _skinny_bwd(gc, ca, wop_, want_gb=False)
        g_value, g_loc, g_attn = _msda().ms_deform_attn_backward(val4, shp, lsi, loc, attn, g_ca.view(B, N, D), 64)
        g_off = torch.empty(M, off.shape[1], dtype=torch.float32, device=dev)
        g_lg = torch.empty(M, attn.numel() // M, dtype=torch.float32, device=dev)
        g_ref = torch.empty_like(refc) if ctx.ref_needs_grad else None
        _lib.launch("egtr_msda_geometry_backward_f32", g_loc.data_ptr(), g_attn.data_ptr(), attn.data_ptr(), off.data_ptr(),
                    off.stride(0), refc.data_ptr(), refc.shape[-1], shp.data_ptr(), g_off.data_ptr(), g_off.shape[1],
                    g_lg.data_ptr(), g_lg.shape[1], _lib.ptr(g_ref), M, heads, L, P_)
        t_so, d_wso, d_bso = _skinny_bwd(g_off, y1p, wso_)
        g_y1p, d_waw, d_baw = _skinny_bwd(g_lg, y1p, waw_, add1=t_so, out=t_so)
        g_y1 = gs2.add_(g_y1p)
        gs1, ga, gbb1 = dropout_add_layernorm_backward(a, x2, m1, scale, g1, e1, g_y1)
        g_sa, d_wo, _ = _skinny_bwd(ga, sa, wo_, want_gb=False)
        gq, gk, gv = torch.empty_like(q), torch.empty_like(k), torch.empty_like(v)
        gqe = _rows256(g_q_ext) if g_q_ext is not None else None
        gke = _rows256(g_k_ext) if g_k_ext is not None else None
        _lib.launch("egtr_self_attn_backward_acc_f32", q.data_ptr(), k.data_ptr(), v.data_ptr(), sa.data_ptr(), lse.data_ptr(),
                    g_sa.data_ptr(), B, N, heads, D // heads, gq.data_ptr(), gk.data_ptr(), gv.data_ptr(), _lib.ptr(gqe),
                    _lib.ptr(gke))
        u_q, d_wq, d_bq = _skinny_bwd(gq, xp, wq_, alpha=scaling)
        g_xp, d_wk, d_bk = _skinny_bwd(gk, xp, wk_, add1=u_q, out=u_q)
        g_x, d_wv, d_bv = _skinny_bwd(gv, x2, wv_, add1=g_xp, add2=gs1, out=gs1)
        g_pos = (g_y1p + g_xp).view(B, N, D)
        if ctx.pos_shape != (B, N, D):
            g_pos = g_pos.sum_to_size(ctx.pos_shape)
        g_val = g_value.view(ctx.value_shape)
        return (g_x.view(B, N, D), g_pos, g_ref, g_val, None, None, None, None, None, None,
                d_wq, d_bq, d_wk, d_bk, d_wv, d_bv, d_wo, gbb1[512:768], gbb1[0:256], gbb1[256:512],
                d_wso, d_bso, d_waw, d_baw, d_wop, gbb2[512:768], gbb2[0:256], gbb2[256:512],
                d_w1, d_b1, d_w2, gbb3[512:768], gbb3[0:256], gbb3[256:512])


def decoder_layer_train_supported(layer, x, pos, ref, value, attention_mask, output_attentions):
    sa, ca = layer.self_attn, layer.encoder_attn
    eligible = (DECODER_TRAIN_FUSED and ENCODER_TRAIN_FUSED and SKINNY_BACKWARD_FUSED and torch.is_grad_enabled()
                and layer.training and not output_attentions and attention_mask is None and torch.is_tensor(x) and x.is_cuda
                and x.dtype == torch.float32 and x.dim() == 3 and x.shape[0] * x.shape[1] <= SKINNY_MAX_ROWS
                and torch.is_tensor(value))
    ok = (eligible and x.shape[-1] == 256 and pos is not None and pos.dtype == torch.float32 and pos.shape[-1] == 256
          and ref is not None and ref.dim() == 4 and ref.shape[-1] == 2 and ref.shape[2] == 4
          and value.dim() == 3 and value.shape[-1] == 256 and value.dtype == torch.float32
          and sa.num_heads == 8 and sa.embed_dim == 256 and sa.dropout == 0.0 and sa.q_proj.bias is not None
          and ca.n_heads == 8 and ca.n_levels == 4 and ca.n_points == 4 and ca.d_model == 256
          and layer.activation_fn is torch.nn.functional.relu and layer.activation_dropout == 0.0
          and layer.fc1.weight.shape[0] % 64 == 0 and tuple(layer.fc2.weight.shape) == (256, layer.fc1.weight.shape[0])
          and x.shape[1] <= 640 and 0.0 <= layer.dropout < 1.0)
    return _gate("decoder_layer_train", eligible, ok,
                 lambda: f"states {tuple(x.shape)}: the training node serves d_model 256, 8 heads, 4 x 4 sampling points, ReLU, "
                         "2-d reference points, <= 640 queries, no attention dropout")


def decoder_layer_train(layer, x, pos, ref, value, spatial_shapes, level_start_index, masks=None):
    sa, ca = layer.self_attn, layer.encoder_attn
    return DecoderLayerTrainFunction.apply(
        x, pos, ref, value, spatial_shapes, level_start_index, layer.dropout, masks,
        (layer.self_attn_layer_norm.eps, layer.encoder_attn_layer_norm.eps, layer.final_layer_norm.eps), float(sa.scaling),
        sa.q_proj.weight, sa.q_proj.bias, sa.k_proj.weight, sa.k_proj.bias, sa.v_proj.weight, sa.v_proj.bias,
        sa.out_proj.weight, sa.out_proj.bias, layer.self_attn_layer_norm.weight, layer.self_attn_layer_norm.bias,
        ca.sampling_offsets.weight, ca.sampling_offsets.bias, ca.attention_weights.weight, ca.attention_weights.bias,
        ca.output_proj.weight, ca.output_proj.bias, layer.encoder_attn_layer_norm.weight, layer.encoder_attn_layer_norm.bias,
        layer.fc1.weight, layer.fc1.bias, layer.fc2.weight, layer.fc2.bias, layer.final_layer_norm.weight,
        layer.final_layer_norm.bias)


ENV_ROUTE_SWITCHES = ("EGTR_DECODER_CLUSTER", "EGTR_GEMM_SPLIT_BF16", "EGTR_REL_HEAD_SPLIT_BF16", "EGTR_FFN_FUSED",
                      "EGTR_BACKBONE_NHWC", "EGTR_ENCODER_TRAIN_FUSED", "EGTR_TOKEN_LINEAR")

FALLBACKS = {}
STRICT_FAST_PATH = os.environ.get("EGTR_STRICT_FAST_PATH", "0") == "1"


class FastPathError(RuntimeError):
    pass


def note_fallback(name, why=""):
    n = FALLBACKS.get(name, 0)
    FALLBACKS[name] = n + 1
    if STRICT_FAST_PATH:
        raise FastPathError(f"left the HIP fast path '{name}': {why}")
    if n == 0:
        import warnings
        warnings.warn(f"egtr_amd: leaving the HIP fast path '{name}' ({why}); counted in egtr_amd.ops.FALLBACKS",
                      RuntimeWarning, stacklevel=3)


def _gate(name, eligible, ok, why):
    if eligible and not ok:
        note_fallback(name, why() if callable(why) else why)
    return bool(ok)


def inference_fast_path(x):
    return x.is_cuda and x.dtype == torch.float32 and not torch.is_grad_enabled()


DEFER_LAYERNORM = True

GEMM_SPLIT_BF16 = os.environ.get("EGTR_GEMM_SPLIT_BF16", "1") != "0"
LAZY_POS = True
GEMM_SPLIT_MIN_ROWS = 4096
GEMM_SPLIT_WGRAD = True


def gemm_split_supported(x, N, K):
    rows = x.numel() // x.shape[-1]
    eligible = (GEMM_SPLIT_BF16 and x.is_cuda and x.dtype == torch.float32 and not torch.is_grad_enabled()
                and rows >= GEMM_SPLIT_MIN_ROWS)
    return _gate("gemm_split", eligible, eligible and K % 32 == 0 and N % 128 == 0,
                 lambda: f"{rows} x {K} -> {N}: K must be a multiple of 32 and N of 128 (vendor GEMM instead)")


def conv1x1_tail_supported(a, N):
    return (a.is_cuda and a.dtype == torch.float32 and a.dim() == 2 and a.stride(1) == 1 and a.stride(0) % 4 == 0
            and a.data_ptr() % 16 == 0 and a.shape[1] in (64, 128, 256, 512) and N % 64 == 0)


def stem_fused_bf16_supported(x, w):
    return (x.is_cuda and x.dtype == torch.bfloat16 and x.dim() == 4 and x.shape[1] == 3 and x.is_contiguous()
            and tuple(w.shape) == (64, 3, 7, 7) and w.dtype == torch.bfloat16)


def stem_fused_supported(x, w):
    return (x.is_cuda and x.dtype == torch.float32 and x.dim() == 4 and x.shape[1] == 3 and x.is_contiguous()
            and tuple(w.shape) == (64, 3, 7, 7))


def conv3x3_supported(x, N, stride=1, variant=0):
    return (x.is_cuda and x.dtype == torch.float32 and x.dim() == 4 and x.is_contiguous(memory_format=torch.channels_last)
            and x.data_ptr() % 16 == 0
            and int(_lib.lib().egtr_conv3x3_phase_channels(int(x.shape[1]), int(N), int(stride), int(variant))) > 0)


def conv1x1_strided_supported(x, N, stride):
    return (x.is_cuda and x.dtype == torch.float32 and x.dim() == 4 and x.is_contiguous(memory_format=torch.channels_last)
            and x.data_ptr() % 16 == 0 and x.shape[1] in (256, 512, 1024) and N % 128 == 0 and stride in (1, 2))


def conv1x1_tail_bf16_supported(a, N):
    return (a.is_cuda and a.dtype == torch.bfloat16 and a.dim() == 2 and a.stride(1) == 1 and a.stride(0) % 8 == 0
            and a.data_ptr() % 16 == 0 and a.shape[1] in (64, 128, 256, 512) and N % 256 == 0)


FFN_FUSED = os.environ.get("EGTR_FFN_FUSED", "1") != "0"


def ffn_fused_supported(x, fc1, fc2, ln):
    rows = x.numel() // x.shape[-1]
    eligible = FFN_FUSED and GEMM_SPLIT_BF16 and inference_fast_path(x) and rows >= GEMM_SPLIT_MIN_ROWS
    ok = (eligible and x.shape[-1] == 256 and tuple(fc1.weight.shape)[1] == 256 and fc1.weight.shape[0] % 64 == 0
          and tuple(fc2.weight.shape) == (256, fc1.weight.shape[0]) and fc1.bias is not None and fc2.bias is not None
          and ln.weight.shape[0] == 256 and fc1.weight.dtype == torch.float32)
    return _gate("ffn_fused", eligible, ok,
                 lambda: f"d_model {x.shape[-1]}, fc1 {tuple(fc1.weight.shape)}: the row-panel kernel serves d_model 256, "
                         "a hidden width that is a multiple of 64, biases present")


ENCODER_TAIL_FUSED = True


def encoder_tail_fused_supported(context, out_proj, ln1, fc1, fc2, ln2):
    return (ENCODER_TAIL_FUSED and proj_ln_fused_supported(context, out_proj, ln1)
            and ffn_fused_supported(context, fc1, fc2, ln2))


def proj_ln_fused_supported(x, lin, ln):
    rows = x.numel() // x.shape[-1]
    eligible = FFN_FUSED and GEMM_SPLIT_BF16 and inference_fast_path(x) and rows >= GEMM_SPLIT_MIN_ROWS
    ok = (eligible and x.shape[-1] == 256 and tuple(lin.weight.shape) == (256, 256) and lin.bias is not None
          and ln.weight.shape[0] == 256 and lin.weight.dtype == torch.float32)
    return _gate("proj_ln_fused", eligible, ok, lambda: f"projection {tuple(lin.weight.shape)}: the kernel serves 256 -> 256 with a bias")


def proj_multi_fused_supported(x):
    rows = x.numel() // x.shape[-1]
    eligible = FFN_FUSED and GEMM_SPLIT_BF16 and inference_fast_path(x) and rows >= GEMM_SPLIT_MIN_ROWS
    return _gate("proj_multi_fused", eligible, eligible and x.shape[-1] == 256, lambda: f"d_model {x.shape[-1]} (256 served)")


def module_linear(mod, x, alpha=1.0, relu=False):
    w = mod.weight
    if alpha == 1.0 and gemm_split_supported(x, w.shape[0], w.shape[1]):
        wt = cached_weights(mod, "gemm_split_bf16", [w], lambda: gemm_split_weights(w))
        return linear_split_bf16(x, wt, mod.bias, w.shape[0], relu)
    return linear(x, mod.weight, mod.bias, alpha, relu)


class BiasActFunction(Function):

    @staticmethod
    def forward(ctx, x, bias, residual):
        x = _chk(x.contiguous(), "x", torch.float32)
        _chk(bias, "bias", torch.float32)
        r = _chk(residual.contiguous(), "residual", torch.float32) if residual is not None else None
        N, C, H, W_ = x.shape
        y = torch.empty_like(x)
        _lib.launch("egtr_bias_act_nchw_f32", x.data_ptr(), bias.data_ptr(), _lib.ptr(r), y.data_ptr(), N, C, H * W_, 1)
        ctx.save_for_backward(y)
        ctx.has_residual = residual is not None
        return y

    @staticmethod
    @once_differentiable
    def backward(ctx, g):
        (y,) = ctx.saved_tensors
        gm = torch.ops.aten.threshold_backward(g.contiguous(), y, 0.0)
        return gm, None, gm if ctx.has_residual else None


def bias_act(x, bias, residual=None):
    return BiasActFunction.apply(x, bias, residual)


class LevelGeometryTrainFunction(Function):

    @staticmethod
    def forward(ctx, level_embed, pixel_mask, spatial_shapes_list, embedding_dim, temperature, scale):
        mask, pos, vr, ref, _ = level_geometry(pixel_mask, spatial_shapes_list, level_embed, embedding_dim, temperature, scale)
        ctx.shapes = (tuple(spatial_shapes_list), pos.shape[0])
        ctx.mark_non_differentiable(mask, vr, ref)
        return pos, mask, vr, ref

    @staticmethod
    @once_differentiable
    def backward(ctx, g_pos, g_mask, g_vr, g_ref):
        shapes, B = ctx.shapes
        g2 = _rows256(g_pos)
        return torch.stack([weighted_column_sum(g2, wl) for wl in _level_row_weights(shapes, B, g2.device)]), \
            None, None, None, None, None


_LEVEL_ROW_WEIGHTS = {}
_LEVEL_ROW_WEIGHTS_MAX = 4


def _level_row_weights(shapes, B, device):
    key = (shapes, B, str(device))
    w = _LEVEL_ROW_WEIGHTS.pop(key, None)
    if w is None:
        sizes = [h * w_ for h, w_ in shapes]
        S = sum(sizes)
        tok = torch.arange(B * S, device=device, dtype=torch.int32) % S
        w, start = [], 0
        for n in sizes:
            w.append(((tok >= start) & (tok < start + n)).to(torch.float32))
            start += n
        while len(_LEVEL_ROW_WEIGHTS) >= _LEVEL_ROW_WEIGHTS_MAX:
            _LEVEL_ROW_WEIGHTS.pop(next(iter(_LEVEL_ROW_WEIGHTS)))
    _LEVEL_ROW_WEIGHTS[key] = w
    return w


def level_geometry_train(pixel_mask, spatial_shapes_list, level_embed, embedding_dim, temperature, scale):
    pos, mask, vr, ref = LevelGeometryTrainFunction.apply(level_embed, pixel_mask, list(spatial_shapes_list), embedding_dim,
                                                          temperature, scale)
    return mask, pos, vr, ref


class AddLayerNormFunction(Function):

    @staticmethod
    def forward(ctx, x, residual, weight, bias, eps):
        x2 = _chk(x.contiguous(), "x", torch.float32)
        r2 = _chk(residual.contiguous(), "residual", torch.float32)
        y = torch.empty_like(x2)
        _lib.launch("egtr_add_layernorm_f32", x2.data_ptr(), r2.data_ptr(), weight.data_ptr(), bias.data_ptr(), y.data_ptr(),
                    x2.numel() // x2.shape[-1], x2.shape[-1], float(eps))
        ctx.eps = eps
        ctx.save_for_backward(x2, r2, weight, bias)
        return y

    @staticmethod
    @once_differentiable
    def backward(ctx, gy):
        lib = _lib.lib()
        x, r, w, b = ctx.saved_tensors
        g = _chk(gy.contiguous(), "grad", torch.float32)
        rows = x.numel() // x.shape[-1]
        gs = torch.empty_like(x)
        ws = torch.empty(int(lib.egtr_add_layernorm_backward_workspace_floats(rows)), dtype=torch.float32, device=x.device)
        gwb = torch.empty(2, x.shape[-1], dtype=torch.float32, device=x.device)
        _lib.launch("egtr_add_layernorm_backward_f32", x.data_ptr(), r.data_ptr(), w.data_ptr(), g.data_ptr(), gs.data_ptr(),
                    ws.data_ptr(), gwb.data_ptr(), rows, x.shape[-1], float(ctx.eps))
        return gs, gs, gwb[0], gwb[1], None


def add_layer_norm(x, residual, ln):
    if x.is_cuda and x.dtype == torch.float32 and x.shape[-1] == 256:
        return AddLayerNormFunction.apply(x, residual, ln.weight, ln.bias, ln.eps)
    if (x.is_cuda and x.dtype == torch.bfloat16 and x.shape[-1] == 256 and not torch.is_grad_enabled()
            and ln.weight.dtype == torch.bfloat16 and residual.dtype == torch.bfloat16):
        lib = _lib.lib()
        x2 = _chk(x.contiguous(), "x", torch.bfloat16)
        r2 = _chk(residual.contiguous(), "residual", torch.bfloat16)
        y = torch.empty_like(x2)
        _lib.launch("egtr_add_layernorm_bf16", x2.data_ptr(), r2.data_ptr(), ln.weight.data_ptr(), ln.bias.data_ptr(),
                    y.data_ptr(), x2.numel() // 256, 256, float(ln.eps))
        return y
    return ln(residual + x)


class RelationHeadFunction(Function):

    @staticmethod
    def forward(ctx, gate_q, gate_k, uq, uk, b1, w2r, b2r, w3r, b3r, w2c, b2c, w3c, b3c, triplet_dist, node_cls,
                want_gate_mean):
        B, N, T = gate_q.shape
        Hd = w2r.shape[1]
        R = w3r.shape[0]
        tens = [gate_q, gate_k, uq, uk, b1, w2r, b2r, w3r, b3r, w2c, b2c, w3c, b3c]
        names = ["gate_q", "gate_k", "uq", "uk", "b1", "w2r", "b2r", "w3r", "b3r", "w2c", "b2c", "w3c", "b3c"]
        tens = [_chk(t.contiguous(), n, torch.float32) for t, n in zip(tens, names)]
        rel = torch.empty(B, N, N, R, dtype=torch.float32, device=gate_q.device)
        conn = torch.empty(B, N, N, dtype=torch.float32, device=gate_q.device)
        gm = torch.zeros(T, dtype=torch.float32, device=gate_q.device) if want_gate_mean else None
        if triplet_dist is not None:
            _chk(triplet_dist, "triplet_dist", torch.float32)
            _chk(node_cls, "node_cls", torch.int64)
            c1 = triplet_dist.shape[0]
        else:
            c1 = 0
        need_grad = any(ctx.needs_input_grad[:13])
        P_ = B * N * N
        h1s = torch.empty(2, P_, Hd, dtype=torch.float32, device=gate_q.device) if need_grad else None
        h2s = torch.empty(2, P_, Hd, dtype=torch.float32, device=gate_q.device) if need_grad else None
        if REL_HEAD_TRAIN_X6 and need_grad and GEMM_SPLIT_BF16 and Hd == 256 and R <= 64 and T in (4, 7):
            gq_, gk_, uq_, uk_, b1_, w2r_, b2r_, w3r_, b3r_, w2c_, b2c_, w3c_, b3c_ = tens
            w2xr, w3x, w2xc = rel_head_streams(w2r_, w3r_, w2c_)
            _lib.launch("egtr_rel_head_forward_bf16x6_save_f32", gq_.data_ptr(), gk_.data_ptr(), uq_.data_ptr(), uk_.data_ptr(),
                        b1_.data_ptr(), w2xr.data_ptr(), b2r_.data_ptr(), w3x.data_ptr(), b3r_.data_ptr(), w2xc.data_ptr(),
                        b2c_.data_ptr(), w3c_.data_ptr(), b3c_.data_ptr(), _lib.ptr(triplet_dist),
                        _lib.ptr(node_cls if triplet_dist is not None else None), B, N, T, Hd, R, c1, rel.data_ptr(),
                        conn.data_ptr(), _lib.ptr(gm), h1s.data_ptr(), h2s.data_ptr())
        else:
            _lib.launch("egtr_rel_head_forward_save_f32", *[t.data_ptr() for t in tens], _lib.ptr(triplet_dist),
                        _lib.ptr(node_cls if triplet_dist is not None else None), B, N, T, Hd, R, c1, rel.data_ptr(),
                        conn.data_ptr(), _lib.ptr(gm), _lib.ptr(h1s), _lib.ptr(h2s))
        if need_grad:
            ctx.save_for_backward(*tens, h1s, h2s)
        return rel, conn.unsqueeze(-1), gm

    @staticmethod
    @once_differentiable
    def backward(ctx, grad_rel, grad_conn, grad_gm):
        (gate_q, gate_k, uq, uk, b1, w2r, b2r, w3r, b3r, w2c, b2c, w3c, b3c, h1s, h2s) = ctx.saved_tensors
        B, N, T = gate_q.shape
        Hd = w2r.shape[1]
        R = w3r.shape[0]
        P_ = B * N * N
        G = grad_rel.reshape(P_, R).contiguous()
        gc = grad_conn.reshape(P_, 1).contiguous()
        dh1 = torch.empty(2, P_, Hd, dtype=torch.float32, device=G.device)
        wgrad = (linear_split_bf16_wgrad if GEMM_SPLIT_BF16 and GEMM_SPLIT_WGRAD and Hd % 128 == 0
                 else (lambda g, h: g.t() @ h))
        dh2, db2r = column_sum(G @ w3r, relu_output=h2s[0], inplace=True)
        dw3r = G.t() @ h2s[0]
        db3r = G.sum(0)
        torch.mm(dh2, w2r, out=dh1[0])
        dw2r = wgrad(dh2, h1s[0])
        dh2, db2c = column_sum(gc * w3c, relu_output=h2s[1], inplace=True)
        dw3c = weighted_column_sum(h2s[1], gc).view(1, -1)
        db3c = gc.sum(0)
        torch.mm(dh2, w2c, out=dh1[1])
        dw2c = wgrad(dh2, h1s[1])
        del dh2
        db1 = torch.cat([column_sum(dh1[i], relu_output=h1s[i], inplace=True)[1] for i in range(2)])
        duq = torch.empty_like(uq)
        duk = torch.empty_like(uk)
        dgq = torch.empty_like(gate_q)
        dgk = torch.empty_like(gate_k)
        dz = torch.empty(P_ * T, dtype=torch.float32, device=G.device)
        _lib.launch("egtr_rel_head_backward_pairs_f32", dh1.data_ptr(), gate_q.data_ptr(), gate_k.data_ptr(), uq.data_ptr(),
                    uk.data_ptr(), B, N, T, Hd, duq.data_ptr(), duk.data_ptr(), dgq.data_ptr(), dgk.data_ptr(), dz.data_ptr())
        return (dgq, dgk, duq, duk, db1, dw2r, db2r, dw3r, db3r, dw2c, db2c, dw3c, db3c, None, None, None)


REL_HEAD_BF16_PACKED = True


def relation_head_bf16w(gate_q, gate_k, uq, uk, b1, w2r, b2r, w3r, b3r, w2c, b2c, w3c, b3c, triplet_dist=None,
                        node_cls=None, want_gate_mean=False):
    B, N, T = gate_q.shape
    Hd = w2r.shape[1]
    R = w3r.shape[0]
    dev = gate_q.device
    packed = REL_HEAD_BF16_PACKED and T <= 10 and Hd == 256 and R <= 64
    tables = []
    for t, n in ((uq, "uq"), (uk, "uk")):
        t = t.detach()
        if packed and t.dtype == torch.bfloat16:
            tables.append(_chk(t.contiguous(), n, torch.bfloat16))
        else:
            tables.append(_chk(t.float().contiguous(), n, torch.float32))
    f32 = [_chk(t.detach().float().contiguous(), n, torch.float32)
           for t, n in ((gate_q, "gate_q"), (gate_k, "gate_k"), (b1, "b1"), (b2r, "b2r"),
                        (b3r, "b3r"), (b2c, "b2c"), (b3c, "b3c"))]
    gq, gk, b1_, b2r_, b3r_, b2c_, b3c_ = f32
    wts = [_chk(t.detach().contiguous(), n, torch.bfloat16)
           for t, n in ((w2r, "w2r"), (w3r, "w3r"), (w2c, "w2c"), (w3c, "w3c"))]
    w2r_, w3r_, w2c_, w3c_ = wts
    rel = torch.empty(B, N, N, R, dtype=torch.float32, device=dev)
    conn = torch.empty(B, N, N, dtype=torch.float32, device=dev)
    gm = torch.zeros(T, dtype=torch.float32, device=dev) if want_gate_mean else None
    td = None
    c1 = 0
    if triplet_dist is not None:
        td = _chk(triplet_dist.detach().float().contiguous(), "triplet_dist", torch.float32)
        _chk(node_cls, "node_cls", torch.int64)
        c1 = td.shape[0]
    if packed:
        if tuple(tables[0].shape) != (B, N, T, 2 * Hd) or tuple(tables[1].shape) != (B, N, T, 2 * Hd):
            raise ValueError("relation_head_bf16w: uq / uk must be [B, N, T, 512]")
        pk = []
        for t in tables:
            out = torch.empty(B * N, 8192, dtype=torch.bfloat16, device=dev)
            _lib.launch("egtr_rel_head_pack_tables_bf16", t.data_ptr(), int(t.dtype == torch.bfloat16), B * N, T,
                        out.data_ptr())
            pk.append(out)
        _lib.launch("egtr_rel_head_forward_bf16p", gq.data_ptr(), gk.data_ptr(), pk[0].data_ptr(), pk[1].data_ptr(),
                    b1_.data_ptr(), w2r_.data_ptr(), b2r_.data_ptr(), w3r_.data_ptr(), b3r_.data_ptr(), w2c_.data_ptr(),
                    b2c_.data_ptr(), w3c_.data_ptr(), b3c_.data_ptr(), _lib.ptr(td),
                    _lib.ptr(node_cls if td is not None else None), B, N, T, Hd, R, c1, rel.data_ptr(), conn.data_ptr(),
                    _lib.ptr(gm))
        return rel, conn.unsqueeze(-1), gm
    uq_, uk_ = tables
    _lib.launch("egtr_rel_head_forward_bf16w", gq.data_ptr(), gk.data_ptr(), uq_.data_ptr(), uk_.data_ptr(), b1_.data_ptr(),
                w2r_.data_ptr(), b2r_.data_ptr(), w3r_.data_ptr(), b3r_.data_ptr(), w2c_.data_ptr(), b2c_.data_ptr(),
                w3c_.data_ptr(), b3c_.data_ptr(), _lib.ptr(td), _lib.ptr(node_cls if td is not None else None), B, N, T, Hd, R,
                c1, rel.data_ptr(), conn.data_ptr(), _lib.ptr(gm))
    return rel, conn.unsqueeze(-1), gm


REL_HEAD_SPLIT_BF16 = os.environ.get("EGTR_REL_HEAD_SPLIT_BF16", "1") != "0"


def relation_head(gate_q, gate_k, uq, uk, b1, w2r, b2r, w3r, b3r, w2c, b2c, w3c, b3c, triplet_dist=None,
                  node_cls=None, want_gate_mean=False, owner=None, sigmoid=False):
    if sigmoid:
        rel, conn, gm = _relation_head(gate_q, gate_k, uq, uk, b1, w2r, b2r, w3r, b3r, w2c, b2c, w3c, b3c, triplet_dist,
                                       node_cls, want_gate_mean, owner, True)
        return rel, conn, gm
    return _relation_head(gate_q, gate_k, uq, uk, b1, w2r, b2r, w3r, b3r, w2c, b2c, w3c, b3c, triplet_dist, node_cls,
                          want_gate_mean, owner, False)


def _relation_head(gate_q, gate_k, uq, uk, b1, w2r, b2r, w3r, b3r, w2c, b2c, w3c, b3c, triplet_dist, node_cls,
                   want_gate_mean, owner, sigmoid):
    if (REL_HEAD_SPLIT_BF16 and owner is not None and gate_q.dtype == torch.float32 and gate_q.is_cuda
            and w2r.shape == (256, 256) and w3r.shape[0] <= 64 and gate_q.shape[-1] <= 9
            and not (torch.is_grad_enabled() and any(
                t.requires_grad for t in (gate_q, gate_k, uq, uk, b1, w2r, b2r, w3r, b3r, w2c, b2c, w3c, b3c)))):
        w2xr, w3xr, w2xc = cached_weights(owner, "rel_head_split_bf16", [w2r, w3r, w2c],
                                          lambda: rel_head_split_weights(w2r, w3r, w2c))
        return relation_head_split_bf16(gate_q, gate_k, uq, uk, b1, w2xr, b2r, w3xr, b3r, w2xc, b2c, w3c, b3c,
                                        w3r.shape[0], triplet_dist, node_cls, want_gate_mean, sigmoid)
    if sigmoid:
        rel, conn, gm = _relation_head(gate_q, gate_k, uq, uk, b1, w2r, b2r, w3r, b3r, w2c, b2c, w3c, b3c, triplet_dist,
                                       node_cls, want_gate_mean, None, False)
        return rel.sigmoid(), conn.sigmoid(), gm
    if gate_q.dtype == torch.bfloat16 and not (torch.is_grad_enabled() and any(
            t.requires_grad for t in (gate_q, gate_k, uq, uk, b1, w2r, b2r, w3r, b3r, w2c, b2c, w3c, b3c))):
        rel, conn, gm = relation_head_bf16w(gate_q, gate_k, uq, uk, b1, w2r, b2r, w3r, b3r, w2c, b2c, w3c, b3c,
                                            triplet_dist, node_cls, want_gate_mean)
        return rel.to(torch.bfloat16), conn.to(torch.bfloat16), gm
    if gate_q.dtype != torch.float32:
        dt = gate_q.dtype
        f = [t.float() for t in (gate_q, gate_k, uq, uk, b1, w2r, b2r, w3r, b3r, w2c, b2c, w3c, b3c)]
        rel, conn, gm = RelationHeadFunction.apply(*f, triplet_dist.float() if triplet_dist is not None else None,
                                                   node_cls, want_gate_mean)
        return rel.to(dt), conn.to(dt), gm
    return RelationHeadFunction.apply(gate_q, gate_k, uq, uk, b1, w2r, b2r, w3r, b3r, w2c, b2c, w3c, b3c,
                                      triplet_dist, node_cls, want_gate_mean)


class RelationLossFunction(Function):

    @staticmethod
    def forward(ctx, pred_rel, pred_conn, target, pred_idx, tgt_idx, match_cost, out_off, nonmatching_cost,
                sample_negatives, sample_nonmatching, packed=False):
        pr = _chk(pred_rel.detach().contiguous(), "pred_rel", torch.float32)
        pc = _chk(pred_conn.detach().contiguous(), "pred_connectivity", torch.float32)
        loss, grad_rel, grad_conn = relation_loss_launch(pr, pc, target, packed, pred_idx, tgt_idx, match_cost, out_off,
                                                         nonmatching_cost, sample_negatives, sample_nonmatching)
        ctx.save_for_backward(grad_rel, grad_conn)
        return loss[0], loss[1]

    @staticmethod
    @once_differentiable
    def backward(ctx, g_rel, g_conn):
        grad_rel, grad_conn = ctx.saved_tensors
        return grad_rel * g_rel, grad_conn * g_conn, None, None, None, None, None, None, None, None, None


class ClampNonFiniteFunction(Function):

    @staticmethod
    def forward(ctx, x):
        _chk(x, "hidden_states", torch.float32)
        flag = torch.zeros(1, dtype=torch.int32, device=x.device)
        cv = torch.finfo(torch.float32).max - 1000
        _lib.launch("egtr_any_nonfinite_f32", x.data_ptr(), x.numel(), flag.data_ptr())
        _lib.launch("egtr_clamp_if_flag_f32", x.data_ptr(), None, x.numel(), flag.data_ptr(), cv, 0)
        ctx.mark_dirty(x)
        ctx.save_for_backward(x, flag)
        ctx.cv = cv
        return x

    @staticmethod
    @once_differentiable
    def backward(ctx, g):
        x, flag = ctx.saved_tensors
        g = g.clone(memory_format=torch.contiguous_format)
        _lib.launch("egtr_clamp_if_flag_f32", g.data_ptr(), x.data_ptr(), g.numel(), flag.data_ptr(), ctx.cv, 1)
        return g


def clamp_nonfinite_(x):
    if x.is_cuda and x.dtype == torch.float32 and x.is_contiguous() and x.data_ptr() % 16 == 0:
        return ClampNonFiniteFunction.apply(x)
    bad = torch.logical_not(torch.isfinite(x).all())
    cv = torch.finfo(x.dtype).max - 1000
# ... 81 lines not shown
```

### include/egtr_hip.h

```cpp
#ifndef EGTR_HIP_H
#define EGTR_HIP_H

#include <stdint.h>

#ifdef __cplusplus
extern "C" {
#endif

typedef void* egtr_stream_t;

enum {
  EGTR_OK = 0,
  EGTR_E_ARG = -1,
  EGTR_E_LAUNCH = -2,
  EGTR_E_UNSUPPORTED = -3
};

#define EGTR_ABI_VERSION 5
int egtr_abi_version(void);
const char* egtr_status_string(int status);
const char* egtr_last_hip_error(void);

int egtr_msda_forward_f32(egtr_stream_t stream, const float* value, const int64_t* spatial_shapes,
                          const int64_t* level_start_index, const float* sampling_loc, const float* attn_weight,
                          int batch, int spatial_size, int num_heads, int channels, int num_levels, int num_query,
                          int num_point, float* out);

int egtr_msda_forward_fused_vbias_f32(egtr_stream_t stream, const float* value, const int64_t* spatial_shapes,
                                      const int64_t* level_start_index, const float* sampling_offsets,
                                      const float* attn_logits, const float* reference_points, int batch,
                                      int spatial_size, int num_heads, int channels, int num_levels, int num_query,
                                      int num_point, float* out, float* attn_weight_out, int ld_offsets, int ld_logits,
                                      const unsigned char* keep_mask, const unsigned* keep_bits,
                                      const float* value_bias);

int egtr_msda_forward_fused_box_f32(egtr_stream_t stream, const float* value, const int64_t* spatial_shapes,
                                    const int64_t* level_start_index, const float* sampling_offsets,
                                    const float* attn_logits, const float* reference_boxes, int batch,
                                    int spatial_size, int num_heads, int channels, int num_levels, int num_query,
                                    int num_point, float* out, float* attn_weight_out, int ld_offsets, int ld_logits,
                                    const unsigned char* keep_mask, const unsigned* keep_bits,
                                    const float* value_bias);

int egtr_msda_backward_f32(egtr_stream_t stream, const float* grad_out, const float* value,
                           const int64_t* spatial_shapes, const int64_t* level_start_index,
                           const float* sampling_loc, const float* attn_weight, int batch, int spatial_size,
                           int num_heads, int channels, int num_levels, int num_query, int num_point,
                           float* grad_value, float* grad_sampling_loc, float* grad_attn_weight);

int egtr_msda_backward_out_f32(egtr_stream_t stream, const float* grad_out, const float* value,
                               const int64_t* spatial_shapes, const int64_t* level_start_index,
                               const float* sampling_loc, const float* attn_weight, int batch, int spatial_size,
                               int num_heads, int channels, int num_levels, int num_query, int num_point,
                               float* grad_value, float* grad_sampling_loc, float* grad_attn_weight);

int egtr_msda_forward_f64(egtr_stream_t stream, const double* value, const int64_t* spatial_shapes,
                          const int64_t* level_start_index, const double* sampling_loc, const double* attn_weight,
                          int batch, int spatial_size, int num_heads, int channels, int num_levels, int num_query,
                          int num_point, double* out);
int egtr_msda_backward_f64(egtr_stream_t stream, const double* grad_out, const double* value,
                           const int64_t* spatial_shapes, const int64_t* level_start_index, const double* sampling_loc,
                           const double* attn_weight, int batch, int spatial_size, int num_heads, int channels,
                           int num_levels, int num_query, int num_point, double* grad_value, double* grad_sampling_loc,
                           double* grad_attn_weight);

long long egtr_msda_backward_bf16_workspace_floats(int batch, int spatial_size, int num_heads, int channels, int num_levels,
                                                   int num_query, int num_point);
int egtr_msda_backward_bf16(egtr_stream_t stream, const uint16_t* grad_out, const uint16_t* value,
                            const int64_t* spatial_shapes, const int64_t* level_start_index, const float* sampling_loc,
                            const float* attn_weight, int batch, int spatial_size, int num_heads, int channels,
                            int num_levels, int num_query, int num_point, float* grad_value, float* grad_sampling_loc,
                            float* grad_attn_weight, float* workspace);

int egtr_msda_forward_bf16(egtr_stream_t stream, const uint16_t* value, const int64_t* spatial_shapes,
                           const int64_t* level_start_index, const float* sampling_loc, const float* attn_weight,
                           int batch, int spatial_size, int num_heads, int channels, int num_levels, int num_query,
                           int num_point, uint16_t* out);

int egtr_msda_forward_fused_bf16(egtr_stream_t stream, const uint16_t* value, const int64_t* spatial_shapes,
                                 const int64_t* level_start_index, const uint16_t* sampling_offsets,
                                 const uint16_t* attn_logits, const uint16_t* reference_points, int batch,
                                 int spatial_size, int num_heads, int channels, int num_levels, int num_query,
                                 int num_point, uint16_t* out, int ld_offsets, int ld_logits,
                                 const unsigned char* keep_mask, const unsigned* keep_bits);

int egtr_self_attn_forward_f32(egtr_stream_t stream, const float* q, const float* k, const float* v, int batch,
                               int num_query, int num_heads, int head_dim, float* out, float* q_heads,
                               float* k_heads, float* lse);

int egtr_self_attn_forward_bf16(egtr_stream_t stream, const uint16_t* q, const uint16_t* k, const uint16_t* v, int batch,
                                int num_query, int num_heads, int head_dim, uint16_t* out, uint16_t* q_heads,
                                uint16_t* k_heads);

int egtr_self_attn_backward_f32(egtr_stream_t stream, const float* q, const float* k, const float* v,
                                const float* out, const float* lse, const float* grad_out, int batch,
                                int num_query, int num_heads, int head_dim, float* grad_q, float* grad_k,
                                float* grad_v);

int egtr_self_attn_backward_acc_f32(egtr_stream_t stream, const float* q, const float* k, const float* v,
                                    const float* out, const float* lse, const float* grad_out, int batch,
                                    int num_query, int num_heads, int head_dim, float* grad_q, float* grad_k,
                                    float* grad_v, const float* grad_q_add, const float* grad_k_add);

int egtr_linear_f32(egtr_stream_t stream, const float* x, const float* w, const float* bias, float* y, int M, int K,
                    int N, float alpha, int relu);

int egtr_linear_backward_f32(egtr_stream_t stream, const float* grad_y, const float* relu_output, const float* x,
                             const float* w, float alpha, float* grad_x, float* grad_w, float* grad_bias, int M, int K,
                             int N);

int egtr_linear_backward_acc_f32(egtr_stream_t stream, const float* grad_y, const float* relu_output, const float* x,
                                 const float* w, float alpha, float* grad_x, float* grad_w, float* grad_bias, int M,
                                 int K, int N, const float* grad_x_add1, const float* grad_x_add2);

int egtr_linear_grouped_f32(egtr_stream_t stream, int num_groups, const float* const* x, const float* const* w,
                            const float* const* bias, float* const* y, const int* M, const int* N, const int* ldy,
                            const float* alpha_x, const float* alpha, const int* relu, int K);

int egtr_linear_grouped_ln_f32(egtr_stream_t stream, int num_groups, const float* const* x, const float* const* w,
                               const float* const* bias, float* const* y, const int* M, const int* N, const int* ldy,
                               const float* alpha_x, const float* alpha, const int* relu, int K,
                               const float* const* ln_residual, const float* const* ln_gamma, const float* const* ln_beta,
                               const float* ln_eps, const float* const* pos, const int* pos_rows, float* const* ln_out);

typedef struct EgtrDecoderLayer {
  const float* x_in;
  const float* pos;
  const float* q;
  const float* k;
  const float* v;
  const float* reference_points;
  const float* valid_ratios;
  const float* value;
  const float* value_bias;
  const unsigned* keep_bits;
  const int64_t* spatial_shapes;
  const int64_t* level_start_index;
  float* x_out;
  float* q_next;
  float* k_next;
  float* v_next;
  const float* w_attn_out;
  const float* b_attn_out;
  const float* ln1_gamma;
  const float* ln1_beta;
  const float* w_off_logit;
  const float* b_off_logit;
  const float* w_cross_out;
  const float* b_cross_out;
  const float* ln2_gamma;
  const float* ln2_beta;
  const float* w_fc1;
  const float* b_fc1;
  const float* w_fc2;
  const float* b_fc2;
  const float* ln3_gamma;
  const float* ln3_beta;
  const float* w_qkv_next;
  const float* b_qkv_next;
  float* partials;
  unsigned* barriers;
  unsigned* status;
  int* xcc_ids;
  float q_scale;
  float ln_eps;
  int batch, num_query, spatial_size, x_rows, pos_rows, qkv_rows, num_clusters;
  int generation;
  int ref_rows;
} EgtrDecoderLayer;
int egtr_decoder_layer_f32(egtr_stream_t stream, const EgtrDecoderLayer* layer);
int egtr_decoder_layer_workspace(int batch, int num_query, long long* partial_floats, int* barrier_words, int* id_words);

int egtr_msda_geometry_forward_f32(egtr_stream_t stream, const float* sampling_offsets, long long ld_offsets,
                                   const float* attention_logits, long long ld_logits, const float* reference_points,
                                   int ref_dim, const int64_t* spatial_shapes, float* sampling_locations,
                                   float* attention_weights, long long rows, int num_heads, int num_levels,
                                   int num_points);
int egtr_msda_geometry_backward_f32(egtr_stream_t stream, const float* grad_locations, const float* grad_weights,
                                    const float* attention_weights, const float* sampling_offsets, long long ld_offsets,
                                    const float* reference_points, int ref_dim, const int64_t* spatial_shapes,
                                    float* grad_offsets, long long ld_grad_offsets, float* grad_logits,
                                    long long ld_grad_logits, float* grad_reference, long long rows, int num_heads,
                                    int num_levels, int num_points);

int egtr_bias_act_nchw_f32(egtr_stream_t stream, const float* x, const float* bias, const float* residual, float* y,
                           int N, int C, int HW, int relu);
int egtr_add_layernorm_f32(egtr_stream_t stream, const float* x, const float* residual, const float* gamma,
                           const float* beta, float* y, int rows, int dim, float eps);
long long egtr_add_layernorm_backward_workspace_floats(int rows);
int egtr_add_layernorm_backward_f32(egtr_stream_t stream, const float* x, const float* residual, const float* gamma,
                                    const float* grad_y, float* grad_sum, float* workspace, float* grad_gamma_beta,
                                    int rows, int dim, float eps);

int egtr_dropout_add_layernorm_f32(egtr_stream_t stream, const float* x, const float* residual, const unsigned char* keep,
                                   float keep_scale, const float* gamma, const float* beta, float* y, int rows, int dim,
                                   float eps, int* nonfinite_flag);
long long egtr_dropout_add_layernorm_backward_workspace_floats(int rows);
int egtr_dropout_add_layernorm_backward_f32(egtr_stream_t stream, const float* x, const float* residual,
                                            const unsigned char* keep, float keep_scale, const float* gamma,
                                            const float* grad_y, const int* clamp_flag, const float* y_out,
                                            float clamp_value, float* grad_sum, float* grad_x, float* workspace,
                                            float* grad_gamma_beta_bias, int rows, int dim, float eps);

int egtr_scale_rows_multi_f32(egtr_stream_t stream, int n, const float* const* w, const float* const* scale,
                              float* const* out, const int* rows, const int* cols);

int egtr_bias_act_nchw_bf16(egtr_stream_t stream, const uint16_t* x, const float* bias, const uint16_t* residual,
                            uint16_t* y, int N, int C, int HW, int relu);
int egtr_add_layernorm_bf16(egtr_stream_t stream, const uint16_t* x, const uint16_t* residual, const uint16_t* gamma,
                            const uint16_t* beta, uint16_t* y, int rows, int dim, float eps);
int egtr_bias_act_nhwc_bf16(egtr_stream_t stream, const uint16_t* x, const float* bias, const uint16_t* residual, uint16_t* y,
                            long long rows, int C, int relu);
int egtr_bias_act_nhwc_f32(egtr_stream_t stream, const float* x, const float* bias, const float* residual, float* y,
                           long long rows, int C, int relu);
int egtr_add_layernorm_pos_bf16(egtr_stream_t stream, const uint16_t* x, const uint16_t* residual, const uint16_t* gamma,
                                const uint16_t* beta, uint16_t* y, int rows, int dim, float eps, const uint16_t* pos,
                                int pos_rows, uint16_t* y_plus_pos);

int egtr_add_layernorm_pos_f32(egtr_stream_t stream, const float* x, const float* residual, const float* gamma,
                               const float* beta, float* y, int rows, int dim, float eps, const float* pos,
                               int pos_rows, float* y_plus_pos);

int egtr_bias_mask_rows_f32(egtr_stream_t stream, float* y, const float* bias, const unsigned char* keep, int groups,
                            int rows, int cols);

int egtr_bias_relu_maxpool3x3s2_f32(egtr_stream_t stream, const float* x, const float* bias, float* y, int N, int C,
                                    int H, int W);

int egtr_box_decode_argmax_f32(egtr_stream_t stream, const float* delta, const float* init_reference,
                               const float* inter_references, int batch, int num_levels, int num_query, int ref_dim,
                               float eps, float* boxes, const float* logits_all, int num_classes, int64_t* node_cls);

int egtr_hungarian_match_f32(egtr_stream_t stream, const float* logits, const float* boxes, const int64_t* tgt_ids,
                             const float* tgt_boxes, const int* tgt_offsets, const int* out_offsets, int batch,
                             int num_query, int num_logits, int max_targets, float class_cost, float bbox_cost,
                             float giou_cost, int smoothing, float cost_min, float inverse_sigmoid_smoothing,
                             int64_t* pred_idx, int64_t* tgt_idx, float* match_cost, float* cost_out,
                             const float* cost_in, int* status, double* scratch);
long long egtr_hungarian_match_scratch_doubles(int num_query, int max_targets, long long total_targets);

int egtr_relation_loss_f32(egtr_stream_t stream, const float* pred_rel, const float* pred_conn,
                           const float* const* target_rel, const int64_t* pred_idx, const int64_t* tgt_idx,
                           const float* match_cost, const int* out_offsets, int batch, int num_query, int num_rel,
                           float nonmatching_cost, int sample_negatives, int sample_nonmatching, float* loss_out,
                           float* grad_rel, float* grad_conn, void* workspace);
long long egtr_relation_loss_workspace_bytes(int batch, int num_query);

int egtr_pack_relations_u64(egtr_stream_t stream, const int64_t* triplets, const int* offsets, int batch, int total,
                            int num_query, int num_rel, uint64_t* rel_bits);
int egtr_relation_loss_bits_f32(egtr_stream_t stream, const float* pred_rel, const float* pred_conn,
                                const uint64_t* rel_bits, const int64_t* pred_idx, const int64_t* tgt_idx,
                                const float* match_cost, const int* out_offsets, int batch, int num_query, int num_rel,
                                float nonmatching_cost, int sample_negatives, int sample_nonmatching, float* loss_out,
                                float* grad_rel, float* grad_conn, void* workspace);

int egtr_bbox_overlaps_f64(egtr_stream_t stream, const double* boxes, const double* query_boxes, int num_boxes,
                           int num_query, int mode, double* out);

long long egtr_sgg_eval_width(int num_rel, int num_k);
int egtr_sgg_eval_f32(egtr_stream_t stream, const int64_t* cand, int cand_cols, const float* rel_scores,
                      const float* pred_boxes, const int64_t* pred_classes, int batch, int num_cand, int num_obj,
                      int num_rel, const int64_t* gt_rels, const int64_t* rel_offsets, long long num_gt_rels,
                      const float* gt_boxes, const int64_t* gt_classes, const int64_t* box_offsets,
                      long long num_gt_boxes, const int* ks, int num_k, double iou_thresh, int* first_rank, double* slab,
                      double* acc);

int egtr_rel_stats_i64(egtr_stream_t stream, const int64_t* rels, const int64_t* rel_offsets, long long num_rels,
                       const int64_t* classes, const int64_t* box_offsets, long long num_boxes, int batch,
                       int num_classes, int num_rel, int64_t* counts, int* status);
int egtr_rel_seen_bits_i64(egtr_stream_t stream, const int64_t* counts, long long num_counts, int64_t* bits);
int egtr_sgg_zero_shot_f64(egtr_stream_t stream, const int* first_rank, const int64_t* gt_rels,
                           const int64_t* rel_offsets, long long num_gt_rels, const int64_t* gt_classes,
                           const int64_t* box_offsets, long long num_gt_boxes, int batch, int num_cand, int num_classes,
                           int num_rel, const int64_t* seen_bits, const int* ks, int num_k, double* slab, double* acc);

int egtr_sgg_eval_phrdet_f32(egtr_stream_t stream, const int64_t* cand, int cand_cols, const float* rel_scores,
                             const float* pred_boxes, const int64_t* pred_classes, int batch, int num_cand, int num_obj,
                             int num_rel, const int64_t* gt_rels, const int64_t* rel_offsets, long long num_gt_rels,
                             const float* gt_boxes, const int64_t* gt_classes, const int64_t* box_offsets,
                             long long num_gt_boxes, const int* ks, int num_k, double iou_thresh, int* first_rank,
                             double* slab, double* acc);
int egtr_sgg_eval_preddet_f32(egtr_stream_t stream, const int64_t* cand, const float* rel_scores, int batch,
                              int num_cand, int num_rel, const int64_t* gt_rels, const int64_t* rel_offsets,
                              long long num_gt_rels, const int64_t* box_offsets, long long num_gt_boxes, const int* ks,
                              int num_k, int* chosen_row, int* first_rank, int* first_rank_pred, double* slab,
                              double* acc);

long long egtr_matched_topk_workspace_bytes(int batch, int num_gt_padded, int num_cand);
int egtr_matched_topk_f32(egtr_stream_t stream, const float* pred_rel, const float* pred_conn, const int* query_of,
                          const float* obj_score, int batch, int num_query, int num_rel, int num_gt_padded, int num_cand,
                          int mode, void* workspace, int64_t* inds, float* rel_scores, float* triplet_scores, int* count);

long long egtr_oi_eval_width(int num_rel, int num_k);
long long egtr_oi_select_workspace_bytes(int num_pairs, int topk, int prd_k, int batch);
int egtr_oi_select_f32(egtr_stream_t stream, const float* pred_scores, long long img_stride, long long row_stride,
                       const float* obj_scores, const int64_t* pairs, long long pair_stride, int batch, int num_pairs,
                       int num_obj, int num_rel, int topk, int prd_k, void* workspace, int* det_sop, float* det_score,
                       int* det_count);
int egtr_oi_match_f32(egtr_stream_t stream, const int* det_sop, const int* det_count, int batch, int topk,
                      const float* pred_boxes, const int64_t* pred_classes, int num_obj, int num_rel,
                      const int64_t* gt_rels, const int64_t* rel_offsets, long long num_gt_rels, const float* gt_boxes,
                      const int64_t* gt_classes, const int64_t* box_offsets, long long num_gt_boxes, const int* ks,
                      int num_k, unsigned char* tp, double* slab, double* acc);
int egtr_oi_ap_f64(egtr_stream_t stream, const unsigned char* tp_sorted, const int64_t* seg_offsets, const double* npos,
                   long long num_records, int num_rel, double* scratch, double* ap);

int egtr_coco_match_f32(egtr_stream_t stream, const float* det_boxes, const float* det_scores, const int64_t* det_labels,
                        int batch, int num_det, int num_classes, const double* gt_boxes, const double* gt_area,
                        const unsigned char* gt_crowd, const int64_t* gt_labels, const int64_t* gt_offsets,
                        long long num_gt, const double* iou_thrs, const double* area_rngs, int max_det, int* rec_label,
                        float* rec_score, int* rec_rank, int64_t* rec_bits, int* npig);
int egtr_coco_accumulate_f64(egtr_stream_t stream, const int* rank_sorted, const int64_t* bits_sorted,
                             const int64_t* seg_offsets, const int* npig, long long num_records, int num_classes,
                             const int* max_dets, const double* rec_thrs, double* precision, double* recall);

int egtr_sine_pos_embed_f32(egtr_stream_t stream, const float* y_embed, const float* x_embed, const float* dim_t,
                            float* out, int B, int H, int W, int E, float scale, float eps);

int egtr_level_geometry_f32(egtr_stream_t stream, const void* pixel_mask, int mask_elem_size, const float* dim_t,
                            const float* level_embed, const int* level_hw, int num_levels, int batch, int height,
                            int width, int embed_dim, float scale, float eps, unsigned char* mask_flat,
                            float* pos_flat, float* valid_ratios, float* ref_points, unsigned* mask_bits);
int egtr_level_geometry_bf16(egtr_stream_t stream, const void* pixel_mask, int mask_elem_size, const float* dim_t,
                             const float* level_embed, const int* level_hw, int num_levels, int batch, int height,
                             int width, int embed_dim, float scale, float eps, unsigned char* mask_flat,
                             uint16_t* pos_flat, float* valid_ratios, float* ref_points, unsigned* mask_bits);

int egtr_input_proj_groupnorm_flatten_f32(egtr_stream_t stream, int num_levels, const float* const* x,
                                          const float* const* conv_bias, const float* const* gamma,
                                          const float* const* beta, const int* level_hw, int batch, int channels,
                                          int num_groups, float eps, float* stats, float* out);
int egtr_input_proj_groupnorm_flatten_bf16(egtr_stream_t stream, int num_levels, const uint16_t* const* x,
                                           const float* const* conv_bias, const float* const* gamma,
                                           const float* const* beta, const int* level_hw, int batch, int channels,
                                           int num_groups, float eps, float* stats, uint16_t* out);

long long egtr_input_proj_groupnorm_tokens_workspace_floats(int num_levels, const int* level_tokens, int batch);
int egtr_input_proj_groupnorm_tokens_bf16(egtr_stream_t stream, int num_levels, const uint16_t* const* x,
                                          const float* const* conv_bias, const float* const* gamma,
                                          const float* const* beta, const int* level_tokens, int batch, int channels,
                                          int num_groups, float eps, float* stats, uint16_t* out);
int egtr_input_proj_groupnorm_tokens_f32(egtr_stream_t stream, int num_levels, const float* const* x,
                                         const float* const* conv_bias, const float* const* gamma, const float* const* beta,
                                         const int* level_tokens, int batch, int channels, int num_groups, float eps,
                                         float* stats, float* out);

int egtr_rel_head_forward_save_f32(egtr_stream_t stream, const float* gate_q, const float* gate_k, const float* uq,
                                   const float* uk, const float* b1, const float* w2r, const float* b2r,
                                   const float* w3r, const float* b3r, const float* w2c, const float* b2c,
                                   const float* w3c, const float* b3c, const float* triplet_dist,
                                   const int64_t* node_cls, int batch, int num_query, int num_slots, int hidden,
                                   int num_rel, int num_cls_plus1, float* rel_logits, float* conn_logits,
                                   float* gate_mean, float* h1_save, float* h2_save);

int egtr_rel_head_forward_bf16w(egtr_stream_t stream, const float* gate_q, const float* gate_k, const float* uq,
                                const float* uk, const float* b1, const uint16_t* w2r, const float* b2r,
                                const uint16_t* w3r, const float* b3r, const uint16_t* w2c, const float* b2c,
                                const uint16_t* w3c, const float* b3c, const float* triplet_dist,
                                const int64_t* node_cls, int batch, int num_query, int num_slots, int hidden,
                                int num_rel, int num_cls_plus1, float* rel_logits, float* conn_logits,
                                float* gate_mean);

int egtr_rel_head_pack_tables_bf16(egtr_stream_t stream, const void* u ,
                                   int u_is_bf16, int rows, int num_slots, uint16_t* packed);
int egtr_rel_head_forward_bf16p(egtr_stream_t stream, const float* gate_q, const float* gate_k,
                                const uint16_t* uq_packed, const uint16_t* uk_packed, const float* b1,
                                const uint16_t* w2r, const float* b2r, const uint16_t* w3r, const float* b3r,
                                const uint16_t* w2c, const float* b2c, const uint16_t* w3c, const float* b3c,
                                const float* triplet_dist, const int64_t* node_cls, int batch, int num_query,
                                int num_slots, int hidden, int num_rel, int num_cls_plus1, float* rel_logits,
                                float* conn_logits, float* gate_mean);

int egtr_linear_bf16(egtr_stream_t stream, const uint16_t* x, int ldx, const uint16_t* weight, const uint16_t* bias,
                     uint16_t* y, int ldy, int M, int N, int K, int relu, float alpha);

int egtr_linear_split_bf16_f32(egtr_stream_t stream, const float* x, int ldx, const uint16_t* w_tiled,
                               const float* bias, float* y, int ldy, int M, int K, int N, int relu);

int egtr_gemm_split_tile_weights_f32(egtr_stream_t stream, const float* w, int ldw, int transposed, int N, int K,
                                     uint16_t* w_tiled);
int egtr_gemm_split_tile_weights_pair_f32(egtr_stream_t stream, const float* w, int ldw, int N, int K,
                                          uint16_t* w_tiled_pair);
int egtr_gemm_split_tile_weights_multi_f32(egtr_stream_t stream, int num_weights, const float* const* w, const int* ldw,
                                           const float* const* w2, const int* ldw2, const int* split_rows, const int* N,
                                           const int* K, uint16_t* const* w_tiled_pair);

long long egtr_linear_split_bf16_wgrad_workspace_floats(int M, int N, int K);
int egtr_linear_split_bf16_wgrad_f32(egtr_stream_t stream, const float* g, int ldg, const float* x, int ldx,
                                     float* grad_weight, float* workspace, int M, int N, int K);

int egtr_linear_split_bf16_grouped_pos_f32(egtr_stream_t stream, int num_problems, const float* const* x, const int* ldx,
                                           const uint16_t* const* w_tiled, const float* const* bias, float* const* y,
                                           const int* ldy, const int* N, const int* relu, int M, int K,
                                           const float* const* pos, const int* pos_rows);

int egtr_linear_split_bf16_ex_f32(egtr_stream_t stream, int num_problems, const float* const* x, const int* ldx,
                                  const uint16_t* const* w_tiled, const float* const* bias, float* const* y,
                                  const int* ldy, const int* N, const int* relu, int M, int K, const float* const* pos,
                                  const int* pos_rows, const unsigned char* const* row_keep, const float* const* relu_ref,
                                  const int* ldref, const float* const* add1, const float* const* add2, const int* ldadd,
                                  float* const* colpart);
int egtr_linear_split_bf16_wgrad_ex_f32(egtr_stream_t stream, const float* g, int ldg, const float* x, int ldx,
                                        float* grad_weight, float* workspace, int M, int N, int K, const float* x_pos,
                                        int pos_rows, const unsigned char* row_keep);

long long egtr_xs_bytes(int rows, int K);
int egtr_xs_split_f32(egtr_stream_t stream, const float* x, int ldx, const float* pos, int pos_rows, int rows, int K,
                      void* xs_out, void* xs_pos_out, int round_to_nearest);

int egtr_conv1x1_tail_x6_f32(egtr_stream_t stream, const float* a, int lda, const float* a_shift, int relu_in,
                             const void* w_xs, const float* bias, const float* shortcut, int ld_shortcut, int relu_out,
                             float* y, int ldy, int M, int K, int N, int tile_rows, int tile_cols);

int egtr_stem_conv7x7_pool_x6_f32(egtr_stream_t stream, const float* x, const void* w_xs, const float* bias, float* y, int B,
                                  int H, int W);

int egtr_stem_conv7x7_pool_bf16(egtr_stream_t stream, const uint16_t* x, const uint16_t* w_packed, const float* bias, uint16_t* y,
                                int B, int H, int W);

int egtr_conv3x3_phase_channels(int C, int N, int stride, int variant);
int egtr_conv3x3_x6_f32(egtr_stream_t stream, const float* x, const void* w_xs, float* y, int B, int H, int W, int C, int N,
                        int stride, int variant);
int egtr_conv3x3_x6_shift_f32(egtr_stream_t stream, const float* x, const float* in_shift, const void* w_xs, float* y, int B, int H,
                              int W, int C, int N, int stride, int variant);

int egtr_conv1x1_strided_x6_f32(egtr_stream_t stream, const float* x, const void* w_xs, float* y, int B, int H, int W, int C, int N,
                                int stride);

int egtr_conv1x1_tail_pack_weights_bf16(egtr_stream_t stream, const uint16_t* w, int ldw, int N, int K, uint16_t* w_packed);
int egtr_conv1x1_tail_bf16(egtr_stream_t stream, const uint16_t* a, int lda, const float* a_shift, int relu_in,
                           const uint16_t* w_packed, const float* bias, const uint16_t* shortcut, int ld_shortcut, int relu_out,
                           uint16_t* y, int ldy, int M, int K, int N);

int egtr_ffn_x6_f32(egtr_stream_t stream, const float* x, int ldx, const void* w1_xs, const float* b1, const void* w2_xs,
                    const float* b2, const float* ln_gamma, const float* ln_beta, float eps, const float* pos,
                    int pos_rows, float* out, float* out_pos, int M, int d_model, int ffn_dim);

long long egtr_ffn_packed_weights_bytes(int ffn_dim);
int egtr_ffn_pack_weights_bf16(egtr_stream_t stream, const uint16_t* w1, const uint16_t* w2, int d_model, int ffn_dim,
                               uint16_t* packed);
int egtr_ffn_layernorm_bf16(egtr_stream_t stream, const uint16_t* x, const uint16_t* w_packed, const uint16_t* b1,
                            const uint16_t* b2, const uint16_t* gamma, const uint16_t* beta, float eps, const uint16_t* pos,
                            int pos_rows, uint16_t* y, uint16_t* y_pos, int M, int d_model, int ffn_dim);

int egtr_encoder_tail_x6_f32(egtr_stream_t stream, const float* context, int ldc, const float* hidden, int ldh,
                             const void* wp_xs, const float* bp, const float* ln1_gamma, const float* ln1_beta, float eps1,
                             const void* w1_xs, const float* b1, const void* w2_xs, const float* b2, const float* ln2_gamma,
                             const float* ln2_beta, float eps2, const float* pos, int pos_rows, float* out, float* out_pos,
                             int M, int d_model, int ffn_dim);

int egtr_proj_ln_x6_f32(egtr_stream_t stream, const float* x, int ldx, const void* w_xs, const float* bias,
                        const float* residual, int ldr, const float* ln_gamma, const float* ln_beta, float eps,
                        const float* pos, int pos_rows, float* out, float* out_pos, int M, int d_model);

int egtr_proj_multi_x6_f32(egtr_stream_t stream, const float* x, int ldx, const void* w_xs, const float* bias, float* out,
                           int M, int d_model, int num_weights);

int egtr_rel_head_forward_bf16x6_f32(egtr_stream_t stream, const float* gate_q, const float* gate_k, const float* uq,
                                     const float* uk, const float* b1, const uint16_t* w2x_rel, const float* b2r,
                                     const uint16_t* w3x_rel, const float* b3r, const uint16_t* w2x_conn,
                                     const float* b2c, const float* w3c, const float* b3c, const float* triplet_dist,
                                     const int64_t* node_cls, int batch, int num_query, int num_slots, int hidden,
                                     int num_rel, int num_cls_plus1, float* rel_logits, float* conn_logits,
                                     float* gate_mean, int apply_sigmoid);

int egtr_rel_head_forward_bf16x6_save_f32(egtr_stream_t stream, const float* gate_q, const float* gate_k, const float* uq,
                                          const float* uk, const float* b1, const uint16_t* w2x_rel, const float* b2r,
                                          const uint16_t* w3x_rel, const float* b3r, const uint16_t* w2x_conn,
                                          const float* b2c, const float* w3c, const float* b3c,
                                          const float* triplet_dist, const int64_t* node_cls, int batch, int num_query,
                                          int num_slots, int hidden, int num_rel, int num_cls_plus1, float* rel_logits,
                                          float* conn_logits, float* gate_mean, float* h1_save, float* h2_save);

int egtr_rel_head_streams_f32(egtr_stream_t stream, const float* w2_rel, const float* w2_conn, const float* w3_rel,
                              int hidden, int num_rel, uint16_t* w2x_rel, uint16_t* w2x_conn, uint16_t* w3x_rel);


int egtr_rel_head_backward_pairs_f32(egtr_stream_t stream, const float* dh1, const float* gate_q, const float* gate_k,
                                     const float* uq, const float* uk, int batch, int num_query, int num_slots,
                                     int hidden, float* grad_uq, float* grad_uk, float* grad_gate_q,
                                     float* grad_gate_k, float* dz_workspace);

int egtr_detection_loss_f32(egtr_stream_t stream, const float* logits, const float* pred_boxes, const int64_t* pred_idx,
                            const int64_t* tgt_idx, const int* match_offsets, const int64_t* target_labels,
                            const float* target_boxes, const int* target_offsets, int batch, int num_query,
                            int num_classes, float focal_alpha, float num_boxes, float* grad_logits,
                            float* grad_boxes_l1, float* grad_boxes_giou, float* out);

int egtr_any_nonfinite_f32(egtr_stream_t stream, const float* x, long long n, int* flag);
int egtr_clamp_if_flag_f32(egtr_stream_t stream, float* t, const float* x, long long n, const int* flag,
                           float clamp_value, int mask_gradient);

long long egtr_column_sum_workspace_floats(int M, int N);
int egtr_column_sum_f32(egtr_stream_t stream, const float* g, const float* relu_output, float* g_masked,
                        float* workspace, float* out, int M, int N);
int egtr_weighted_column_sum_f32(egtr_stream_t stream, const float* g, const float* row_weight, float* workspace,
                                 float* out, int M, int N);

int egtr_pad_batch_f32(egtr_stream_t stream, const float* const* images, const int* heights_widths, int batch,
                       int channels, int H, int W, float* pixel_values, int64_t* pixel_mask);

#define EGTR_PREPROCESS_TILE_W 128
#define EGTR_PREPROCESS_STAGE_BYTES 16354
int egtr_preprocess_f32(egtr_stream_t stream, const int64_t* desc, int batch, const int32_t* coeffs, const float* lut,
                        int H, int W, int prepass_rows, int prepass_cols, uint8_t* workspace, float* pixel_values,
                        int64_t* pixel_mask);
int egtr_preprocess_bf16(egtr_stream_t stream, const int64_t* desc, int batch, const int32_t* coeffs, const float* lut,
                         int H, int W, int prepass_rows, int prepass_cols, uint8_t* workspace, uint16_t* pixel_values,
                         int64_t* pixel_mask);

#define EGTR_AUGMENT_DESC_WORDS 17
#define EGTR_AUGMENT_MIRROR 1
#define EGTR_AUGMENT_SRC_WORKSPACE 2
#define EGTR_AUGMENT_PREPASS 4
int egtr_preprocess_augment_f32(egtr_stream_t stream, const int64_t* first_desc, const int64_t* final_desc, int batch,
                                const int32_t* coeffs, const float* lut, int H, int W, int first_rows, int first_cols,
                                int pre1_rows, int pre1_cols, int pre2_rows, int pre2_cols, uint8_t* workspace,
                                float* pixel_values, int64_t* pixel_mask);
int egtr_preprocess_augment_bf16(egtr_stream_t stream, const int64_t* first_desc, const int64_t* final_desc, int batch,
                                 const int32_t* coeffs, const float* lut, int H, int W, int first_rows, int first_cols,
                                 int pre1_rows, int pre1_cols, int pre2_rows, int pre2_cols, uint8_t* workspace,
                                 uint16_t* pixel_values, int64_t* pixel_mask);

#ifdef __cplusplus
}
#endif
#endif
```

Baseline: 389.7 images/sec.

## Fuse level geometry into one kernel and add fused token GroupNorm path

Adds a single-launch level_geometry_fused kernel. It computes the resized mask, cumulative-sum sine positional embeddings, valid ratios, reference points and mask bits per 32-pixel run, replacing the previous multi-kernel sequence. It also adds a fused GroupNorm-over-tokens variant with smaller chunks that normalizes and stores in the same pass. Both are enabled by default at inference when grad is off. The cost is redundant mask resampling in every block and a row-width limit of 2048.

```diff
diff --git a/egtr_amd/_lib.py b/egtr_amd/_lib.py
--- a/egtr_amd/_lib.py
+++ b/egtr_amd/_lib.py
@@ -51,11 +51,18 @@
                                 _P, _P],
     "egtr_level_geometry_bf16": [_P, _P, _I, _P, _P, _P, _I, _I, _I, _I, _I, ctypes.c_float, ctypes.c_float, _P, _P, _P,
                                  _P, _P],
+    "egtr_level_geometry_fused_f32": [_P, _P, _I, _P, _P, _P, _I, _I, _I, _I, _I, ctypes.c_float, ctypes.c_float, _P, _P,
+                                      _P, _P, _P],
+    "egtr_level_geometry_fused_bf16": [_P, _P, _I, _P, _P, _P, _I, _I, _I, _I, _I, ctypes.c_float, ctypes.c_float, _P, _P,
+                                       _P, _P, _P],
     "egtr_input_proj_groupnorm_flatten_f32": [_P, _I, _P, _P, _P, _P, _P, _I, _I, _I, ctypes.c_float, _P, _P],
     "egtr_input_proj_groupnorm_flatten_bf16": [_P, _I, _P, _P, _P, _P, _P, _I, _I, _I, ctypes.c_float, _P, _P],
     "egtr_input_proj_groupnorm_tokens_bf16": [_P, _I, _P, _P, _P, _P, _P, _I, _I, _I, ctypes.c_float, _P, _P],
     "egtr_input_proj_groupnorm_tokens_f32": [_P, _I, _P, _P, _P, _P, _P, _I, _I, _I, ctypes.c_float, _P, _P],
     "egtr_input_proj_groupnorm_tokens_workspace_floats": [_I, _P, _I],
+    "egtr_input_proj_groupnorm_tokens_fused_bf16": [_P, _I, _P, _P, _P, _P, _P, _I, _I, _I, ctypes.c_float, _P, _P],
+    "egtr_input_proj_groupnorm_tokens_fused_f32": [_P, _I, _P, _P, _P, _P, _P, _I, _I, _I, ctypes.c_float, _P, _P],
+    "egtr_input_proj_groupnorm_tokens_fused_workspace_floats": [_I, _P, _I],
     "egtr_bbox_overlaps_f64": [_P, _P, _P, _I, _I, _I, _P],
     "egtr_sgg_eval_width": [_I, _I],
     "egtr_sgg_eval_f32": [_P, _P, _I, _P, _P, _P, _I, _I, _I, _I, _P, _P, ctypes.c_longlong, _P, _P, _P, ctypes.c_longlong,
@@ -152,6 +159,7 @@
 _RESTYPES = {"egtr_status_string": ctypes.c_char_p, "egtr_last_hip_error": ctypes.c_char_p,
              "egtr_ffn_packed_weights_bytes": ctypes.c_longlong,
              "egtr_input_proj_groupnorm_tokens_workspace_floats": ctypes.c_longlong,
+             "egtr_input_proj_groupnorm_tokens_fused_workspace_floats": ctypes.c_longlong,
              "egtr_msda_backward_bf16_workspace_floats": ctypes.c_longlong,
              "egtr_hungarian_match_scratch_doubles": ctypes.c_longlong,
              "egtr_relation_loss_workspace_bytes": ctypes.c_longlong,
diff --git a/egtr_amd/csrc/elementwise.hip b/egtr_amd/csrc/elementwise.hip
--- a/egtr_amd/csrc/elementwise.hip
+++ b/egtr_amd/csrc/elementwise.hip
@@ -564,6 +564,193 @@
 }
 
 
+constexpr int kGeoRun = 32;
+constexpr int kGeoMaxW = 2048;
+struct LevelRuns {
+  int block0[5];
+  int runs[4];
+};
+
+template <typename MaskT>
+__device__ __forceinline__ int resized_mask(const MaskT* __restrict__ pm, int Hin, int Win, int Hl, int Wl, int y, int x) {
+  const float sh = (float)Hin / (float)Hl, sw = (float)Win / (float)Wl;
+  const int sy = min((int)floorf((float)y * sh), Hin - 1), sx = min((int)floorf((float)x * sw), Win - 1);
+  return pm[(size_t)sy * Win + sx] != 0 ? 1 : 0;
+}
+
+template <typename MaskT, typename PosT>
+__global__ __launch_bounds__(256) void level_geometry_fused(const MaskT* __restrict__ pixel_mask,
+                                                            const float* __restrict__ dim_t,
+                                                            const float* __restrict__ level_embed, LevelDims ld,
+                                                            LevelRuns lr, int L, int S, int Hin, int Win, int E,
+                                                            float scale, float eps, unsigned char* __restrict__ mask_flat,
+                                                            unsigned* __restrict__ mask_bits, PosT* __restrict__ pos_flat,
+                                                            float* __restrict__ valid_ratios,
+                                                            float* __restrict__ ref_points) {
+  constexpr int TP = kGeoRun;
+  __shared__ int s_cnt[8];
+  __shared__ float s_vr[8];
+  __shared__ int s_pix[TP][4];
+  __shared__ unsigned char s_row[kGeoMaxW];
+  const int tid = threadIdx.x;
+  const int b = blockIdx.y;
+  const MaskT* pm = pixel_mask + (size_t)b * Hin * Win;
+  int l = 0;
+  while (l + 1 < L && (int)blockIdx.x >= lr.block0[l + 1]) ++l;
+  const int Hl = ld.H[l], Wl = ld.W[l];
+  const int blk = (int)blockIdx.x - lr.block0[l];
+  const int y = blk / lr.runs[l], x0 = (blk - y * lr.runs[l]) * TP;
+  const int n = min(TP, Wl - x0);
+  const int s0 = ld.start[l] + y * Wl + x0;
+  if (tid < 8) s_cnt[tid] = 0;
+  __syncthreads();
+  const int p = tid >> 3, part = tid & 7;
+  const int xcol = x0 + min(p, n - 1);
+  int vr_total = 0;
+  for (int k = 0; k < L; ++k) vr_total += ld.W[k] + ld.H[k];
+  const int nwords = (S + 31) >> 5;
+  const int rowv = resized_mask(pm, Hin, Win, Hl, Wl, y, min(tid, Wl - 1));
+  int colv[8];
+#pragma unroll
+  for (int u = 0; u < 8; ++u) colv[u] = resized_mask(pm, Hin, Win, Hl, Wl, min(part + 8 * u, Hl - 1), xcol);
+  int vrv[2], vrs[2];
+#pragma unroll
+  for (int u = 0; u < 2; ++u) {
+    int i = min(tid + 256 * u, vr_total - 1), k = 0;
+    while (k + 1 < L && i >= ld.W[k] + ld.H[k]) {
+      i -= ld.W[k] + ld.H[k];
+      ++k;
+    }
+    const int col = i >= ld.W[k];
+    vrs[u] = 2 * k + col;
+    vrv[u] = resized_mask(pm, Hin, Win, ld.H[k], ld.W[k], col ? i - ld.W[k] : 0, col ? 0 : i);
+  }
+  int bitv = 0;
+  if (mask_bits != nullptr && tid < 64 && (int)blockIdx.x < nwords) {
+    const int s = 32 * (int)blockIdx.x + tid;
+    if (tid < 32 && s < S) {
+      int k = 0;
+      while (k + 1 < L && s >= ld.start[k + 1]) ++k;
+      const int rel = s - ld.start[k];
+      const int ty = rel / ld.W[k];
+      bitv = resized_mask(pm, Hin, Win, ld.H[k], ld.W[k], ty, rel - ty * ld.W[k]);
+    }
+  }
+  if (tid < Wl) s_row[tid] = (unsigned char)rowv;
+  for (int x = tid + 256; x < Wl; x += 256) s_row[x] = (unsigned char)resized_mask(pm, Hin, Win, Hl, Wl, y, x);
+  int cy = 0, toty = 0;
+#pragma unroll
+  for (int u = 0; u < 8; ++u) {
+    const int yy = part + 8 * u, v = yy < Hl ? colv[u] : 0;
+    toty += v;
+    cy += (yy <= y) ? v : 0;
+  }
+  for (int yy = part + 64; yy < Hl; yy += 8) {
+    const int v = resized_mask(pm, Hin, Win, Hl, Wl, yy, xcol);
+    toty += v;
+    cy += (yy <= y) ? v : 0;
+  }
+#pragma unroll
+  for (int u = 0; u < 2; ++u)
+    if (tid + 256 * u < vr_total && vrv[u]) atomicAdd(&s_cnt[vrs[u]], 1);
+  for (int i0 = tid + 512; i0 < vr_total; i0 += 256) {
+    int i = i0, k = 0;
+    while (k + 1 < L && i >= ld.W[k] + ld.H[k]) {
+      i -= ld.W[k] + ld.H[k];
+      ++k;
+    }
+    const int col = i >= ld.W[k];
+    if (resized_mask(pm, Hin, Win, ld.H[k], ld.W[k], col ? i - ld.W[k] : 0, col ? 0 : i)) atomicAdd(&s_cnt[2 * k + col], 1);
+  }
+  if (mask_bits != nullptr && tid < 64) {
+    if ((int)blockIdx.x < nwords) {
+      const unsigned long long bal = __ballot(bitv != 0);
+      if (tid == 0) mask_bits[(size_t)b * nwords + blockIdx.x] = (unsigned)bal;
+    }
+    for (int w = blockIdx.x + gridDim.x; w < nwords; w += gridDim.x) {
+      const int s = 32 * w + tid;
+      int m = 0;
+      if (tid < 32 && s < S) {
+        int k = 0;
+        while (k + 1 < L && s >= ld.start[k + 1]) ++k;
+        const int rel = s - ld.start[k];
+        const int ty = rel / ld.W[k];
+        m = resized_mask(pm, Hin, Win, ld.H[k], ld.W[k], ty, rel - ty * ld.W[k]);
+      }
+      const unsigned long long bal = __ballot(m != 0);
+      if (tid == 0) mask_bits[(size_t)b * nwords + w] = (unsigned)bal;
+    }
+  }
+  __syncthreads();
+  {
+    int cx = 0, totx = 0;
+    if (p < n) {
+      for (int xx = part; xx < Wl; xx += 8) {
+        const int v = s_row[xx];
+        totx += v;
+        cx += (xx <= xcol) ? v : 0;
+      }
+    }
+#pragma unroll
+    for (int o = 1; o < 8; o <<= 1) {
+      cy += __shfl_xor(cy, o);
+      toty += __shfl_xor(toty, o);
+      cx += __shfl_xor(cx, o);
+      totx += __shfl_xor(totx, o);
+    }
+    if (part == 0) {
+      s_pix[p][0] = cy;
+      s_pix[p][1] = toty;
+      s_pix[p][2] = cx;
+      s_pix[p][3] = totx;
+    }
+  }
+  if (tid < n) mask_flat[(size_t)b * S + s0 + tid] = s_row[x0 + tid];
+  __syncthreads();
+  if (tid < 2 * L) {
+    const int k = tid >> 1;
+    const float vr = (float)s_cnt[tid] / (float)((tid & 1) ? ld.H[k] : ld.W[k]);
+    s_vr[tid] = vr;
+    if (blockIdx.x == 0) valid_ratios[(size_t)b * L * 2 + tid] = vr;
+  }
+  __syncthreads();
+  {
+    const int p = tid >> 3, k = tid & 7;
+    if (p < n && k < 2 * L) {
+      const int x = x0 + p;
+      const int lt = k >> 1, ax = k & 1;
+      const float base = ax ? ((float)y + 0.5f) / (s_vr[2 * l + 1] * (float)Hl)
+                            : ((float)x + 0.5f) / (s_vr[2 * l] * (float)Wl);
+      ref_points[(((size_t)b * S + s0 + p) * L + lt) * 2 + ax] = base * s_vr[2 * lt + ax];
+    }
+  }
+  {
+    const int npair = E;
+    const int per = 256 / npair > 0 ? 256 / npair : 1;
+    for (int k = tid % npair; k < npair; k += 256) {
+      const int c = 2 * k;
+      const int axis = c >= E, i = axis ? c - E : c;
+      const float dt = dim_t[i];
+      const float2 le = *reinterpret_cast<const float2*>(level_embed + l * 2 * E + c);
+      for (int p = (npair <= 256 ? tid / npair : 0); p < n; p += per) {
+        const size_t s = (size_t)b * S + s0 + p;
+        const float e = (float)(axis ? s_pix[p][2] : s_pix[p][0]), last = (float)(axis ? s_pix[p][3] : s_pix[p][1]);
+        const float v = (e - 0.5f) / (last + eps) * scale;
+        const float a = v / dt;
+        float sn, cs;
+        sincosf(a, &sn, &cs);
+        if constexpr (sizeof(PosT) == 4) {
+          *reinterpret_cast<float2*>(pos_flat + s * (2 * E) + c) = make_float2(sn + le.x, cs + le.y);
+        } else {
+          const unsigned lo = f2bf(bf2f(f2bf(sn)) + le.x), hi = f2bf(bf2f(f2bf(cs)) + le.y);
+          *reinterpret_cast<unsigned*>(pos_flat + s * (2 * E) + c) = lo | (hi << 16);
+        }
+      }
+    }
+  }
+}
+
+
 struct GnLevels {
   const void* x[4];
   const float* conv_bias[4];
@@ -673,7 +860,7 @@
                                  const float* level_embed, const int* level_hw, int num_levels, int batch, int height,
                                  int width, int embed_dim, float scale, float eps, unsigned char* mask_flat,
                                  void* pos_flat, bool pos_bf16, float* valid_ratios, float* ref_points,
-                                 unsigned* mask_bits) {
+                                 unsigned* mask_bits, bool fused = false) {
   if (!pixel_mask || !dim_t || !level_embed || !level_hw || !mask_flat || !pos_flat || !valid_ratios || !ref_points)
     return EGTR_E_ARG;
   if (num_levels < 1 || num_levels > 4 || batch <= 0 || height <= 0 || width <= 0 || embed_dim <= 0)
@@ -693,6 +880,33 @@
     }
   }
   hipStream_t st = static_cast<hipStream_t>(stream);
+  if (fused) {
+    LevelRuns lr;
+    int nb = 0;
+    for (int l = 0; l < 4; ++l) {
+      lr.block0[l] = nb;
+      lr.runs[l] = (ld.W[l] + kGeoRun - 1) / kGeoRun;
+      if (l < num_levels) {
+        if (ld.W[l] > kGeoMaxW) return EGTR_E_UNSUPPORTED;
+        nb += ld.H[l] * lr.runs[l];
+      }
+    }
+    lr.block0[4] = nb;
+    const dim3 fgrid((unsigned)nb, (unsigned)batch);
+#define EGTR_GEO_FUSED(MaskT, PosT)                                                                                      \
+  hipLaunchKernelGGL((level_geometry_fused<MaskT, PosT>), fgrid, dim3(256), 0, st, static_cast<const MaskT*>(pixel_mask), \
+                     dim_t, level_embed, ld, lr, num_levels, S, height, width, embed_dim, scale, eps, mask_flat, mask_bits, \
+                     static_cast<PosT*>(pos_flat), valid_ratios, ref_points)
+    if (mask_elem_size == 8) {
+      if (pos_bf16) EGTR_GEO_FUSED(long long, unsigned short);
+      else EGTR_GEO_FUSED(long long, float);
+    } else {
+      if (pos_bf16) EGTR_GEO_FUSED(unsigned char, unsigned short);
+      else EGTR_GEO_FUSED(unsigned char, float);
+    }
+#undef EGTR_GEO_FUSED
+    return egtr_check_launch();
+  }
   const dim3 grid1((unsigned)((S + 255) / 256), (unsigned)batch);
   if (mask_elem_size == 8)
     hipLaunchKernelGGL(level_mask_resize<long long>, grid1, dim3(256), 0, st, static_cast<const long long*>(pixel_mask),
@@ -730,6 +944,26 @@
   return level_geometry_launch(stream, pixel_mask, mask_elem_size, dim_t, level_embed, level_hw, num_levels, batch, height,
                                width, embed_dim, scale, eps, mask_flat, pos_flat, true, valid_ratios, ref_points,
                                mask_bits);
+}
+
+extern "C" int egtr_level_geometry_fused_f32(egtr_stream_t stream, const void* pixel_mask, int mask_elem_size,
+                                             const float* dim_t, const float* level_embed, const int* level_hw,
+                                             int num_levels, int batch, int height, int width, int embed_dim, float scale,
+                                             float eps, unsigned char* mask_flat, float* pos_flat, float* valid_ratios,
+                                             float* ref_points, unsigned* mask_bits) {
+  return level_geometry_launch(stream, pixel_mask, mask_elem_size, dim_t, level_embed, level_hw, num_levels, batch, height,
+                               width, embed_dim, scale, eps, mask_flat, pos_flat, false, valid_ratios, ref_points,
+                               mask_bits, true);
+}
+
+extern "C" int egtr_level_geometry_fused_bf16(egtr_stream_t stream, const void* pixel_mask, int mask_elem_size,
+                                              const float* dim_t, const float* level_embed, const int* level_hw,
+                                              int num_levels, int batch, int height, int width, int embed_dim, float scale,
+                                              float eps, unsigned char* mask_flat, uint16_t* pos_flat, float* valid_ratios,
+                                              float* ref_points, unsigned* mask_bits) {
+  return level_geometry_launch(stream, pixel_mask, mask_elem_size, dim_t, level_embed, level_hw, num_levels, batch, height,
+                               width, embed_dim, scale, eps, mask_flat, pos_flat, true, valid_ratios, ref_points,
+                               mask_bits, true);
 }
 
 static int groupnorm_flatten_launch(egtr_stream_t stream, int num_levels, const void* const* x,
@@ -791,20 +1025,21 @@
   f[0] = a.x; f[1] = a.y; f[2] = a.z; f[3] = a.w; f[4] = b.x; f[5] = b.y; f[6] = b.z; f[7] = b.w;
 }
 constexpr int kGnTokChunk = 256;
-template <typename T>
+constexpr int kGnTokChunkFused = 64;
+template <typename T, int CHUNK = kGnTokChunk>
 __global__ __launch_bounds__(256) void gn_partial_tokens(GnTokLevels P, int L, int chunks_total, double2* __restrict__ partial) {
   __shared__ double s_red[2][32][9];
   const int b = blockIdx.y;
   int l = 0;
   while (l + 1 < L && (int)blockIdx.x >= P.cchunk0[l + 1]) ++l;
-  const int t_begin = ((int)blockIdx.x - P.cchunk0[l]) * kGnTokChunk, hw = P.hw[l];
+  const int t_begin = ((int)blockIdx.x - P.cchunk0[l]) * CHUNK, hw = P.hw[l];
   const int g = threadIdx.x & 31, ph = threadIdx.x >> 5;
   const T* x = static_cast<const T*>(P.x[l]) + (size_t)b * hw * 256;
   const float4 ba = *reinterpret_cast<const float4*>(P.conv_bias[l] + 8 * g), bb = *reinterpret_cast<const float4*>(P.conv_bias[l] + 8 * g + 4);
   const float cb[8] = {ba.x, ba.y, ba.z, ba.w, bb.x, bb.y, bb.z, bb.w};
   float s1 = 0.f, s2 = 0.f;
 #pragma unroll
-  for (int u0 = 0; u0 < kGnTokChunk / 8; u0 += 8) {
+  for (int u0 = 0; u0 < CHUNK / 8; u0 += 8) {
     float f[8][8];
 #pragma unroll
     for (int u = 0; u < 8; ++u) {
@@ -863,9 +1098,37 @@
 }
 
 template <typename T>
+__device__ __forceinline__ void gn_normalize_store(const GnTokLevels& P, int l, int g, const float (&f)[8], float2 st,
+                                                   T* __restrict__ dst, long long rel) {
+  typedef __bf16 bf16x2 __attribute__((ext_vector_type(2)));
+  const float4 ca = *reinterpret_cast<const float4*>(P.conv_bias[l] + 8 * g), cb = *reinterpret_cast<const float4*>(P.conv_bias[l] + 8 * g + 4);
+  const float4 ga = *reinterpret_cast<const float4*>(P.gamma[l] + 8 * g), gb = *reinterpret_cast<const float4*>(P.gamma[l] + 8 * g + 4);
+  const float4 ea = *reinterpret_cast<const float4*>(P.beta[l] + 8 * g), eb = *reinterpret_cast<const float4*>(P.beta[l] + 8 * g + 4);
+  const float c8[8] = {ca.x, ca.y, ca.z, ca.w, cb.x, cb.y, cb.z, cb.w};
+  const float g8[8] = {ga.x, ga.y, ga.z, ga.w, gb.x, gb.y, gb.z, gb.w};
+  const float e8[8] = {ea.x, ea.y, ea.z, ea.w, eb.x, eb.y, eb.z, eb.w};
+  float o[8];
+#pragma unroll
+  for (int k = 0; k < 8; ++k) o[k] = (f[k] + c8[k] - st.x) * st.y * g8[k] + e8[k];
+  if constexpr (sizeof(T) == 2) {
+    unsigned w[4];
+#pragma unroll
+    for (int k = 0; k < 4; ++k) {
+      bf16x2 pr;
+      pr[0] = (__bf16)o[2 * k];
+      pr[1] = (__bf16)o[2 * k + 1];
+      w[k] = __builtin_bit_cast(unsigned, pr);
+    }
+    reinterpret_cast<uint4*>(dst)[rel] = make_uint4(w[0], w[1], w[2], w[3]);
+  } else {
+    reinterpret_cast<float4*>(dst)[2 * rel] = make_float4(o[0], o[1], o[2], o[3]);
+    reinterpret_cast<float4*>(dst)[2 * rel + 1] = make_float4(o[4], o[5], o[6], o[7]);
+  }
+}
+
+template <typename T>
 __global__ __launch_bounds__(256) void gn_apply_tokens(GnTokLevels P, int L, int S, const float2* __restrict__ stats,
                                                        T* __restrict__ out) {
-  typedef __bf16 bf16x2 __attribute__((ext_vector_type(2)));
   const int b = blockIdx.y, B = gridDim.y;
   const long long i = (long long)blockIdx.x * 256 + threadIdx.x;
   if (i >= (long long)S * 32) return;
@@ -876,36 +1139,72 @@
   const float2 st = stats[((size_t)l * B + b) * 32 + g];
   float f[8];
   load_group8(static_cast<const T*>(P.x[l]) + (size_t)b * P.hw[l] * 256, (size_t)rel, f);
-  const float4 ca = *reinterpret_cast<const float4*>(P.conv_bias[l] + 8 * g), cb = *reinterpret_cast<const float4*>(P.conv_bias[l] + 8 * g + 4);
-  const float4 ga = *reinterpret_cast<const float4*>(P.gamma[l] + 8 * g), gb = *reinterpret_cast<const float4*>(P.gamma[l] + 8 * g + 4);
-  const float4 ea = *reinterpret_cast<const float4*>(P.beta[l] + 8 * g), eb = *reinterpret_cast<const float4*>(P.beta[l] + 8 * g + 4);
-  const float c8[8] = {ca.x, ca.y, ca.z, ca.w, cb.x, cb.y, cb.z, cb.w};
-  const float g8[8] = {ga.x, ga.y, ga.z, ga.w, gb.x, gb.y, gb.z, gb.w};
-  const float e8[8] = {ea.x, ea.y, ea.z, ea.w, eb.x, eb.y, eb.z, eb.w};
-  float o[8];
-#pragma unroll
-  for (int k = 0; k < 8; ++k) o[k] = (f[k] + c8[k] - st.x) * st.y * g8[k] + e8[k];
+  gn_normalize_store(P, l, g, f, st, out + ((size_t)b * S + P.start[l]) * 256, rel);
+}
+
+constexpr int kGnApplyTokens = 32;
+struct GnTokBlocks {
+  int ablock0[5];
+};
+
+template <typename T>
+__global__ __launch_bounds__(256) void gn_apply_tokens_fused(GnTokLevels P, GnTokBlocks A, int L, int S, int chunks_total,
+                                                             float eps, const double2* __restrict__ partial,
+                                                             T* __restrict__ out) {
+  __shared__ double2 s_part[8][32];
+  __shared__ float2 s_stats[32];
+  const int b = blockIdx.y;
+  int l = 0;
+  while (l + 1 < L && (int)blockIdx.x >= A.ablock0[l + 1]) ++l;
+  const int hw = P.hw[l];
+  const long long nrel = (long long)hw * 32;
+  const long long rel0 = (long long)((int)blockIdx.x - A.ablock0[l]) * (kGnApplyTokens * 32) + threadIdx.x;
+  const int g = threadIdx.x & 31, part = threadIdx.x >> 5;
+  const T* x = static_cast<const T*>(P.x[l]) + (size_t)b * hw * 256;
+  constexpr int U = kGnApplyTokens * 32 / 256;
+  float f[U][8];
+#pragma unroll
+  for (int u = 0; u < U; ++u)
+    if (rel0 + 256 * u < nrel) load_group8(x, (size_t)(rel0 + 256 * u), f[u]);
+  double t1 = 0.0, t2 = 0.0;
+  const int c_end = P.cchunk0[l + 1];
+  for (int c0 = P.cchunk0[l] + part; c0 < c_end; c0 += 64) {
+    double2 p[8];
+#pragma unroll
+    for (int u = 0; u < 8; ++u)
+      p[u] = c0 + 8 * u < c_end ? partial[((size_t)b * chunks_total + c0 + 8 * u) * 32 + g] : make_double2(0.0, 0.0);
+#pragma unroll
+    for (int u = 0; u < 8; ++u) {
+      t1 += p[u].x;
+      t2 += p[u].y;
+    }
+  }
+  s_part[part][g] = make_double2(t1, t2);
+  __syncthreads();
+  if (part == 0) {
+    t1 = 0.0;
+    t2 = 0.0;
+#pragma unroll
+    for (int k = 0; k < 8; ++k) {
+      t1 += s_part[k][g].x;
+      t2 += s_part[k][g].y;
+    }
+    const double n = 8.0 * hw, mean = t1 / n;
+    const double var = fmax(t2 / n - mean * mean, 0.0);
+    s_stats[g] = make_float2((float)mean, (float)(1.0 / sqrt(var + (double)eps)));
+  }
+  __syncthreads();
+  const float2 st = s_stats[g];
   T* dst = out + ((size_t)b * S + P.start[l]) * 256;
-  if constexpr (sizeof(T) == 2) {
-    unsigned w[4];
-#pragma unroll
-    for (int k = 0; k < 4; ++k) {
-      bf16x2 pr;
-      pr[0] = (__bf16)o[2 * k];
-      pr[1] = (__bf16)o[2 * k + 1];
-      w[k] = __builtin_bit_cast(unsigned, pr);
-    }
-    reinterpret_cast<uint4*>(dst)[rel] = make_uint4(w[0], w[1], w[2], w[3]);
-  } else {
-    reinterpret_cast<float4*>(dst)[2 * rel] = make_float4(o[0], o[1], o[2], o[3]);
-    reinterpret_cast<float4*>(dst)[2 * rel + 1] = make_float4(o[4], o[5], o[6], o[7]);
-  }
-}
-}
-
-static int gn_tokens_chunks(int num_levels, const int* level_tokens) {
+#pragma unroll
+  for (int u = 0; u < U; ++u)
+    if (rel0 + 256 * u < nrel) gn_normalize_store(P, l, g, f[u], st, dst, rel0 + 256 * u);
+}
+}
+
+static int gn_tokens_chunks(int num_levels, const int* level_tokens, int chunk = kGnTokChunk) {
   int c = 0;
-  for (int l = 0; l < num_levels; ++l) c += (level_tokens[l] + kGnTokChunk - 1) / kGnTokChunk;
+  for (int l = 0; l < num_levels; ++l) c += (level_tokens[l] + chunk - 1) / chunk;
   return c;
 }
 
@@ -914,14 +1213,23 @@
   return (long long)num_levels * batch * 64 + (long long)batch * gn_tokens_chunks(num_levels, level_tokens) * 128;
 }
 
+extern "C" long long egtr_input_proj_groupnorm_tokens_fused_workspace_floats(int num_levels, const int* level_tokens,
+                                                                             int batch) {
+  if (!level_tokens || num_levels < 1 || num_levels > 4 || batch <= 0) return 0;
+  return (long long)batch * gn_tokens_chunks(num_levels, level_tokens, kGnTokChunkFused) * 128;
+}
+
 static int groupnorm_tokens_launch(egtr_stream_t stream, int num_levels, const void* const* x, const float* const* conv_bias,
                                    const float* const* gamma, const float* const* beta, const int* level_tokens, int batch,
-                                   int channels, int num_groups, float eps, float* stats, void* out, bool bf16) {
+                                   int channels, int num_groups, float eps, float* stats, void* out, bool bf16,
+                                   bool fused = false) {
   if (!x || !conv_bias || !gamma || !beta || !level_tokens || !stats || !out) return EGTR_E_ARG;
   if (num_levels < 1 || num_levels > 4 || batch <= 0) return EGTR_E_ARG;
   if (channels != 256 || num_groups != 32) return EGTR_E_UNSUPPORTED;
   GnTokLevels P;
-  int S = 0, cc = 0;
+  GnTokBlocks A;
+  const int chunk = fused ? kGnTokChunkFused : kGnTokChunk;
+  int S = 0, cc = 0, ab = 0;
   for (int l = 0; l < 4; ++l) {
     const int s = l < num_levels ? l : 0;
     if (!x[s] || !conv_bias[s] || !gamma[s] || !beta[s] || level_tokens[s] <= 0) return EGTR_E_ARG;
@@ -934,19 +1242,37 @@
     P.start[l] = S;
     P.chunk0[l] = (long long)S * 32;
     P.cchunk0[l] = cc;
+    A.ablock0[l] = ab;
     if (l < num_levels) {
       S += P.hw[l];
-      cc += (P.hw[l] + kGnTokChunk - 1) / kGnTokChunk;
+      cc += (P.hw[l] + chunk - 1) / chunk;
+      ab += (P.hw[l] + kGnApplyTokens - 1) / kGnApplyTokens;
     }
   }
   P.chunk0[4] = (long long)S * 32;
   P.cchunk0[4] = cc;
+  A.ablock0[4] = ab;
   for (int l = num_levels; l < 4; ++l) {
     P.chunk0[l] = (long long)S * 32;
     P.cchunk0[l] = cc;
+    A.ablock0[l] = ab;
   }
   if ((reinterpret_cast<uintptr_t>(out) | reinterpret_cast<uintptr_t>(stats)) & 15) return EGTR_E_UNSUPPORTED;
   hipStream_t st = static_cast<hipStream_t>(stream);
+  if (fused) {
+    double2* part = reinterpret_cast<double2*>(stats);
+    const dim3 pgrid(cc, batch), fgrid(ab, batch);
+    if (bf16) {
+      hipLaunchKernelGGL((gn_partial_tokens<unsigned short, kGnTokChunkFused>), pgrid, dim3(256), 0, st, P, num_levels, cc, part);
+      hipLaunchKernelGGL(gn_apply_tokens_fused<unsigned short>, fgrid, dim3(256), 0, st, P, A, num_levels, S, cc, eps, part,
+                         static_cast<unsigned short*>(out));
+    } else {
+      hipLaunchKernelGGL((gn_partial_tokens<float, kGnTokChunkFused>), pgrid, dim3(256), 0, st, P, num_levels, cc, part);
+      hipLaunchKernelGGL(gn_apply_tokens_fused<float>, fgrid, dim3(256), 0, st, P, A, num_levels, S, cc, eps, part,
+                         static_cast<float*>(out));
+    }
+    return egtr_check_launch();
+  }
   float2* st2 = reinterpret_cast<float2*>(stats);
   double2* partial = reinterpret_cast<double2*>(stats + (size_t)num_levels * batch * 64);
   const long long chunks = (long long)S * 32;
@@ -978,6 +1304,24 @@
                                                     int channels, int num_groups, float eps, float* stats, float* out) {
   return groupnorm_tokens_launch(stream, num_levels, reinterpret_cast<const void* const*>(x), conv_bias, gamma, beta,
                                  level_tokens, batch, channels, num_groups, eps, stats, out, false);
+}
+
+extern "C" int egtr_input_proj_groupnorm_tokens_fused_bf16(egtr_stream_t stream, int num_levels, const uint16_t* const* x,
+                                                           const float* const* conv_bias, const float* const* gamma,
+                                                           const float* const* beta, const int* level_tokens, int batch,
+                                                           int channels, int num_groups, float eps, float* partials,
+                                                           uint16_t* out) {
+  return groupnorm_tokens_launch(stream, num_levels, reinterpret_cast<const void* const*>(x), conv_bias, gamma, beta,
+                                 level_tokens, batch, channels, num_groups, eps, partials, out, true, true);
+}
+
+extern "C" int egtr_input_proj_groupnorm_tokens_fused_f32(egtr_stream_t stream, int num_levels, const float* const* x,
+                                                          const float* const* conv_bias, const float* const* gamma,
+                                                          const float* const* beta, const int* level_tokens, int batch,
+                                                          int channels, int num_groups, float eps, float* partials,
+                                                          float* out) {
+  return groupnorm_tokens_launch(stream, num_levels, reinterpret_cast<const void* const*>(x), conv_bias, gamma, beta,
+                                 level_tokens, batch, channels, num_groups, eps, partials, out, false, true);
 }
 
 extern "C" int egtr_input_proj_groupnorm_flatten_f32(egtr_stream_t stream, int num_levels, const float* const* x,
diff --git a/egtr_amd/kernels/elementwise.py b/egtr_amd/kernels/elementwise.py
--- a/egtr_amd/kernels/elementwise.py
+++ b/egtr_amd/kernels/elementwise.py
@@ -185,7 +185,7 @@
     return out
 
 
-def input_proj_groupnorm_tokens(token_outputs, input_projs):
+def input_proj_groupnorm_tokens(token_outputs, input_projs, fused=False):
     import ctypes
     lib = _lib.lib()
     L = len(token_outputs)
@@ -206,9 +206,10 @@
     S = sum(toks)
     out = torch.empty(B, S, 256, dtype=dt, device=xs[0].device)
     PA, IA = ctypes.c_void_p * L, ctypes.c_int * L
-    stats = torch.empty(int(lib.egtr_input_proj_groupnorm_tokens_workspace_floats(L, IA(*toks), B)), dtype=torch.float32,
+    stem = "egtr_input_proj_groupnorm_tokens_fused" if fused else "egtr_input_proj_groupnorm_tokens"
+    stats = torch.empty(int(getattr(lib, stem + "_workspace_floats")(L, IA(*toks), B)), dtype=torch.float32,
                         device=xs[0].device)
-    entry = "egtr_input_proj_groupnorm_tokens_bf16" if dt == torch.bfloat16 else "egtr_input_proj_groupnorm_tokens_f32"
+    entry = stem + ("_bf16" if dt == torch.bfloat16 else "_f32")
     _lib.launch(entry, L, PA(*[x.data_ptr() for x in xs]), PA(*[k[0].data_ptr() for k in keep]),
                 PA(*[k[1].data_ptr() for k in keep]), PA(*[k[2].data_ptr() for k in keep]), IA(*toks), B, 256, 32,
                 float(gn0.eps), stats.data_ptr(), out.data_ptr())
@@ -218,7 +219,7 @@
 _DIM_T = {}
 
 
-def level_geometry(pixel_mask, spatial_shapes_list, level_embed, embedding_dim, temperature, scale, eps=1e-6):
+def level_geometry(pixel_mask, spatial_shapes_list, level_embed, embedding_dim, temperature, scale, eps=1e-6, fused=False):
     import ctypes
     dev = pixel_mask.device
     key = (embedding_dim, float(temperature), str(dev))
@@ -245,7 +246,7 @@
     pos = torch.empty(B, S, 2 * embedding_dim, dtype=pos_dtype, device=dev)
     vr = torch.empty(B, L, 2, dtype=torch.float32, device=dev)
     ref = torch.empty(B, S, L, 2, dtype=torch.float32, device=dev)
-    entry = "egtr_level_geometry_bf16" if pos_dtype == torch.bfloat16 else "egtr_level_geometry_f32"
+    entry = ("egtr_level_geometry_fused" if fused else "egtr_level_geometry") + ("_bf16" if pos_dtype == torch.bfloat16 else "_f32")
     _lib.launch(entry, pm.data_ptr(), pm.element_size(), dim_t.data_ptr(), le.data_ptr(), hw, L, B, H, W_, embedding_dim,
                 float(scale), float(eps), mask_u8.data_ptr(), pos.data_ptr(), vr.data_ptr(), ref.data_ptr(), bits.data_ptr())
     return mask_u8.view(torch.bool), pos, vr, ref, bits
diff --git a/egtr_amd/ops.py b/egtr_amd/ops.py
--- a/egtr_amd/ops.py
+++ b/egtr_amd/ops.py
@@ -886,11 +886,40 @@
     return BiasActFunction.apply(x, bias, residual)
 
 
+LEVEL_GEOMETRY_FUSED = True
+GN_TOKENS_FUSED = True
+LEVEL_GEOMETRY_FUSED_MAX_WIDTH = 2048
+
+_level_geometry_launch = level_geometry
+_input_proj_groupnorm_tokens_launch = input_proj_groupnorm_tokens
+
+
+def level_geometry_fused_supported(pixel_mask, spatial_shapes_list):
+    eligible = LEVEL_GEOMETRY_FUSED and pixel_mask.is_cuda and not torch.is_grad_enabled()
+    return _gate("level_geometry_fused", eligible, eligible and max(w for _, w in spatial_shapes_list) <= LEVEL_GEOMETRY_FUSED_MAX_WIDTH,
+                 lambda: f"level widths {[w for _, w in spatial_shapes_list]}: the kernel buffers rows up to "
+                         f"{LEVEL_GEOMETRY_FUSED_MAX_WIDTH} wide")
+
+
+def level_geometry(pixel_mask, spatial_shapes_list, level_embed, embedding_dim, temperature, scale, eps=1e-6):
+    return _level_geometry_launch(pixel_mask, spatial_shapes_list, level_embed, embedding_dim, temperature, scale, eps,
+                                  fused=level_geometry_fused_supported(pixel_mask, spatial_shapes_list))
+
+
+def gn_tokens_fused_supported(token_outputs):
+    return GN_TOKENS_FUSED and token_outputs[0].is_cuda and not torch.is_grad_enabled()
+
+
+def input_proj_groupnorm_tokens(token_outputs, input_projs):
+    return _input_proj_groupnorm_tokens_launch(token_outputs, input_projs, fused=gn_tokens_fused_supported(token_outputs))
+
+
 class LevelGeometryTrainFunction(Function):
 
     @staticmethod
     def forward(ctx, level_embed, pixel_mask, spatial_shapes_list, embedding_dim, temperature, scale):
-        mask, pos, vr, ref, _ = level_geometry(pixel_mask, spatial_shapes_list, level_embed, embedding_dim, temperature, scale)
+        mask, pos, vr, ref, _ = _level_geometry_launch(pixel_mask, spatial_shapes_list, level_embed, embedding_dim, temperature,
+                                                       scale)
         ctx.shapes = (tuple(spatial_shapes_list), pos.shape[0])
         ctx.mark_non_differentiable(mask, vr, ref)
         return pos, mask, vr, ref
diff --git a/include/egtr_hip.h b/include/egtr_hip.h
--- a/include/egtr_hip.h
+++ b/include/egtr_hip.h
@@ -326,6 +326,15 @@
                              int width, int embed_dim, float scale, float eps, unsigned char* mask_flat,
                              uint16_t* pos_flat, float* valid_ratios, float* ref_points, unsigned* mask_bits);
 
+int egtr_level_geometry_fused_f32(egtr_stream_t stream, const void* pixel_mask, int mask_elem_size, const float* dim_t,
+                                  const float* level_embed, const int* level_hw, int num_levels, int batch, int height,
+                                  int width, int embed_dim, float scale, float eps, unsigned char* mask_flat,
+                                  float* pos_flat, float* valid_ratios, float* ref_points, unsigned* mask_bits);
+int egtr_level_geometry_fused_bf16(egtr_stream_t stream, const void* pixel_mask, int mask_elem_size, const float* dim_t,
+                                   const float* level_embed, const int* level_hw, int num_levels, int batch, int height,
+                                   int width, int embed_dim, float scale, float eps, unsigned char* mask_flat,
+                                   uint16_t* pos_flat, float* valid_ratios, float* ref_points, unsigned* mask_bits);
+
 int egtr_input_proj_groupnorm_flatten_f32(egtr_stream_t stream, int num_levels, const float* const* x,
                                           const float* const* conv_bias, const float* const* gamma,
                                           const float* const* beta, const int* level_hw, int batch, int channels,
@@ -344,6 +353,16 @@
                                          const float* const* conv_bias, const float* const* gamma, const float* const* beta,
                                          const int* level_tokens, int batch, int channels, int num_groups, float eps,
                                          float* stats, float* out);
+
+long long egtr_input_proj_groupnorm_tokens_fused_workspace_floats(int num_levels, const int* level_tokens, int batch);
+int egtr_input_proj_groupnorm_tokens_fused_bf16(egtr_stream_t stream, int num_levels, const uint16_t* const* x,
+                                                const float* const* conv_bias, const float* const* gamma,
+                                                const float* const* beta, const int* level_tokens, int batch, int channels,
+                                                int num_groups, float eps, float* partials, uint16_t* out);
+int egtr_input_proj_groupnorm_tokens_fused_f32(egtr_stream_t stream, int num_levels, const float* const* x,
+                                               const float* const* conv_bias, const float* const* gamma,
+                                               const float* const* beta, const int* level_tokens, int batch, int channels,
+                                               int num_groups, float eps, float* partials, float* out);
 
 int egtr_rel_head_forward_save_f32(egtr_stream_t stream, const float* gate_q, const float* gate_k, const float* uq,
                                    const float* uk, const float* b1, const float* w2r, const float* b2r,
```

Result: no change. 391.2 images/sec (median of 6 runs) (+0.4%).
